# jasonkyuyim/se3_diffusion

Measured on AMD Instinct MI355X. Metric: residues/sec IPA fwd+bwd, higher is better.
Workload: dtype f32

## Files before the change

include/fd_hip.h:

```cpp
#ifndef FD_HIP_H_
#define FD_HIP_H_

#ifdef __cplusplus
extern "C" {
#endif

#define FD_ABI_VERSION 2

const char* fd_last_error(void);
int fd_abi_version(void);
const char* fd_backend(void);
const char* fd_build_flags(void);
long fd_launch_count(void);

typedef struct FdGemmDesc {
  const float* A;
  const float* B;
  float* C;
  int M, N, K;
  long a_rs, a_cs;
  long b_rs, b_cs;
  long ldc;
  int batch, bdiv;
  long a_so, a_si, b_so, b_si, c_so, c_si;
// ... 41 lines not shown
int fd_edge_mlp_pack(const float* W1, const float* W2, const float* Wf, long ld, void* image, void* stream);
int fd_edge_mlp_pack_bwd(const float* Wf, const float* W2, const float* W1, long ld, const float* W40, void* image, void* stream);
typedef struct FdEdgeMlpDesc {
  const float* x;
  const void* img;
  const float* p1;
  const float* q1;
  const float* bias2;
  float* save1;
  float* save2;
  const float* pf;
  const float* qf;
  const float* gamma;
  const float* beta;
  const float* rowscale;
  float* y;
  float* mean;
  float* rstd;
  float* out;
  long rows;
  int nres;
  int backward;
  float eps;
  int blocks;
  long ld_pq;
  long ld_pqf;
  float* zb_out;
  const float* zb_bias;
  unsigned* mask1;
  unsigned* mask2;
  const unsigned* gmask1;
  const unsigned* gmask2;
  const float* ln_y;
  const float* ln_mean;
  const float* ln_rstd;
  const float* ln_gamma;
  const float* ln_rowscale;
  float* dy_out;
  float* ln_dgamma;
  float* ln_dbeta;
  const float* dzb;
  unsigned* sched;
  int shape;
} FdEdgeMlpDesc;
#define FD_EDGE_MLP_W8_MIN_ROWS 65536L
#define FD_EDGE_MLP_PAIR_MAX_ROWS 16384L
int fd_edge_mlp(const FdEdgeMlpDesc* desc, void* stream);

#define FD_EDGE_EMBED_IMAGE_BYTES (24 * 12288)
int fd_edge_embed_pack_zb(const float* W40, void* image, void* stream);
int fd_edge_embed_pack(const float* W0, const float* W2, const float* W4, void* image, void* stream);
typedef struct FdEdgeEmbedDesc {
  const long* seq_idx;
  const float* sc_ca;
  const float* idenom;
  const float* dg_lower;
  const float* dg_upper;
  const void* img;
  const float* p;
  const float* q;
  const float* bias2;
  const float* bias3;
  const float* gamma;
  const float* beta;
  const float* rowscale;
  float* h1;
  float* h2;
  float* h3;
  float* mean;
  float* rstd;
  float* out;
  long rows;
  int nres;
  float eps;
  int blocks;
  float* zb_out;
  const float* zb_bias;
  unsigned* mask1;
  unsigned* mask2;
  long ld_pq;
} FdEdgeEmbedDesc;
int fd_edge_embed(const FdEdgeEmbedDesc* desc, void* stream);

#define FD_EDGE_EMBED_BWD_IMAGE_BYTES (16 * 12288)
int fd_edge_embed_bwd_pack(const float* W2, const float* W4, void* image, void* stream);
typedef struct FdEdgeEmbedBwdDesc {
  const float* dy;
  const float* h3;
  const float* mean;
  const float* rstd;
  const float* gamma;
  const float* rowscale;
  const float* h2;
  const float* h1;
  const void* img;
  float* dh3;
  float* dh2;
  float* dh1;
  float* dgamma;
  float* dbeta;
  long rows;
  int blocks;
  const unsigned* gmask2;
  const unsigned* gmask1;
  unsigned* sched;
} FdEdgeEmbedBwdDesc;
int fd_edge_embed_bwd(const FdEdgeEmbedBwdDesc* desc, void* stream);

typedef struct FdLnGemmDesc {
  const float* x;
  long ldx;
  const float* gamma;
  const float* beta;
  const float* ln_rowscale;
  float* ln_out;
  long ld_ln_out;
  const float* W;
  long ldw;
  const float* bias;
  const float* resid;
  long ld_resid;
  float* out;
  long ldo;
  int M, N, K;
  int relu;
  float eps;
  int ln_cols;
} FdLnGemmDesc;
int fd_ln_gemm(const FdLnGemmDesc* desc, void* stream);

#define FD_PAIR_DW_MAX_ITEMS 8
typedef struct FdPairDwItem {
  const float* A;
  long lda;
  const float* A_add;
  long ld_add;
  const float* B;
  long ldb;
  float* C;
  long ldc;
  float* a_colsum;
  int trans;
  int a_bands;
  int b_cols;
} FdPairDwItem;
typedef struct FdPairDwDesc {
  FdPairDwItem item[FD_PAIR_DW_MAX_ITEMS];
  int nitems;
  long rows;
  int blocks;
} FdPairDwDesc;
int fd_pair_dw(const FdPairDwDesc* desc, void* stream);

#define FD_GROUP_DW_MAX_ITEMS 32
typedef struct FdGroupDwItem {
  const float* A;
  const float* B;
  float* C;
  float* a_colsum;
  int lda, ldb, ldc;
  int n_out, k_in;
} FdGroupDwItem;
typedef struct FdGroupDwDesc {
  FdGroupDwItem item[FD_GROUP_DW_MAX_ITEMS];
  int nitems;
  long rows;
  int blocks;
} FdGroupDwDesc;
int fd_group_dw(const FdGroupDwDesc* desc, void* stream);

int fd_seq_attn_fwd(const float* qkv, const float* key_add, float* out, float* A_out, float scale, int B, int N,
                    void* stream);
int fd_seq_attn_bwd(const float* qkv, const float* A, const float* dout, const float* out, float* dqkv, float scale, int B, int N,
                    void* stream);

int fd_node_feats(const long* seq_idx, const float* tscaled, const float* fixed, const float* tfreq,
                  const float* idenom, float* out , int B, int N, void* stream);
int fd_node_feats_ld(const long* seq_idx, const float* tscaled, const float* fixed, const float* tfreq,
                     const float* idenom, float* out , long ld, int B, int N, void* stream);
int fd_edge_feats(const long* seq_idx, const float* tscaled, const float* fixed, const float* sc_ca,
                  const float* tfreq, const float* idenom, const float* dg_lower, const float* dg_upper,
                  float* out , int B, int N, void* stream);

int fd_ipa_points_fwd(const float* proj, const float* quat, const float* trans, float* qp, float* kp, float* vp,
                      float* kp_soa, int n_res, long R, int nheads, int c_hidden, int n_qk, int n_v, void* stream);
int fd_ipa_points_bwd(const float* proj, const float* quat, const float* dqp, const float* dkp, const float* dvp,
                      float* dproj, float* dframe, long R, int nheads, int c_hidden, int n_qk, int n_v,
                      void* stream);
int fd_ipa_softmax_fwd(float* S, const float* zb, const float* qp, const float* kp, const float* head_w,
                       const float* mask, int B, int N, void* stream);
// ... 296 lines not shown
```

se3_diffusion_amd/csrc/fd_edge_embed.hip:

```cpp
#include "fd_common.h"
#include "../../include/fd_hip.h"

namespace {

#include "fd_chain.h"

constexpr int EE_UNITS = 20;
constexpr int EE_ZB_UNITS = 4;
constexpr int EE_ZB = 40;
constexpr int EE_C = 128;
constexpr float kPi = 3.14159265358979323846f;

__global__ __launch_bounds__(256) void edge_embed_pack_kernel(const float* __restrict__ W0, const float* __restrict__ W2,
                                                              const float* __restrict__ W4, char* __restrict__ img) {
  const int gid = (int)(blockIdx.x * blockDim.x + threadIdx.x);
  if (gid >= EE_UNITS * 4 * 64) return;
  const int lane = gid & 63, i = (gid >> 6) & 3, u = gid >> 8;
  const int m = lane & 15, g = lane >> 4;
  const int layer = u < 4 ? 0 : (u < 12 ? 1 : 2);
  const int r = u - (layer == 0 ? 0 : (layer == 1 ? 4 : 12));
  const int n = 64 * (r & 1) + 16 * i + m, k0 = 32 * (r >> 1);
  float x[8];
#pragma unroll
  for (int e = 0; e < 8; ++e) {
    if (layer == 0) {
      const int k = k0 + 8 * g + e;
      x[e] = k < 54 ? W0[n * 120 + 66 + k] : 0.f;
    } else {
      const int k = k0 + 16 * (e >> 2) + 4 * g + (e & 3);
      x[e] = (layer == 1 ? W2 : W4)[n * EE_C + k];
    }
  }
  uint4 s0, s1, s2;
  fd_split8(x, s0, s1, s2);
  char* dst = img + (long)u * EM_UNIT + (i * 3) * EM_PIECE + lane * 16;
  *reinterpret_cast<uint4*>(dst) = s0;
  *reinterpret_cast<uint4*>(dst + EM_PIECE) = s1;
  *reinterpret_cast<uint4*>(dst + 2 * EM_PIECE) = s2;
}

__global__ __launch_bounds__(256) void edge_embed_pack_zb_kernel(const float* __restrict__ W40, char* __restrict__ img) {
  const int gid = (int)(blockIdx.x * blockDim.x + threadIdx.x);
  if (gid >= EE_ZB_UNITS * 4 * 64) return;
  const int lane = gid & 63, i = (gid >> 6) & 3, ks = gid >> 8;
  const int m = lane & 15, g = lane >> 4;
  const int n = 16 * i + m;
  float x[8];
#pragma unroll
  for (int e = 0; e < 8; ++e) {
    const int k = 32 * ks + 16 * (e >> 2) + 4 * g + (e & 3);
    x[e] = n < EE_ZB ? W40[n * EE_C + k] : 0.f;
  }
  uint4 s0, s1, s2;
  fd_split8(x, s0, s1, s2);
  char* dst = img + (long)(EE_UNITS + ks) * EM_UNIT + (i * 3) * EM_PIECE + lane * 16;
  *reinterpret_cast<uint4*>(dst) = s0;
  *reinterpret_cast<uint4*>(dst + EM_PIECE) = s1;
  *reinterpret_cast<uint4*>(dst + 2 * EM_PIECE) = s2;
}

template <bool ZB>
__global__ __launch_bounds__(64 * EM_WAVES, 2) void edge_embed_kernel(FdEdgeEmbedDesc d) {
  constexpr int EE_NSTAGE = (EE_UNITS + (ZB ? EE_ZB_UNITS : 0)) / EM_UPS;
  __shared__ __attribute__((aligned(16))) char lds[2 * EM_STAGE];
  const int tid = (int)threadIdx.x;
  const int lane = tid & 63, wave = tid >> 6;
  const int m = lane & 15, g = lane >> 4;
  const long rows = d.rows;
  const long ld_pq = d.ld_pq > 0 ? d.ld_pq : EE_C;
  const int ntiles = (int)((rows + EM_ROWS - 1) / EM_ROWS);
  const int G = (int)gridDim.x, first = (int)blockIdx.x;
  if (first >= ntiles) return;
  const int nmine = (ntiles - first + G - 1) / G;
  const int total_stages = nmine * EE_NSTAGE;

  const char* __restrict__ img_lane = static_cast<const char*>(d.img) + wave * (EM_STAGE / EM_WAVES) + lane * 16;
  char* const lds_wave = lds + wave * (EM_STAGE / EM_WAVES);
  int issued = 0, consumed = 0;
  auto issue_stage = [&]() {
    const char* src = img_lane + (long)(issued % EE_NSTAGE) * EM_STAGE;
    char* dst = lds_wave + (issued & 1) * EM_STAGE;
    fd::glds16x4(src, dst);
    fd::glds16x2(src + 4096, dst + 4096);
    ++issued;
  };
  auto stage_begin = [&]() -> const char* {
    fd::wait_vmem();
    __syncthreads();
    const char* cur = lds + (consumed & 1) * EM_STAGE + lane * 16;
    ++consumed;
    return cur;
  };
  auto stage_prefetch = [&]() {
    if (issued < total_stages) issue_stage();
  };
  issue_stage();

  float den[8], lo[8], up[8];
#pragma unroll
  for (int e = 0; e < 8; ++e) {
    den[e] = d.idenom[(8 * g + e) & 15];
    const int kb = 8 * g + e;
    lo[e] = kb < 22 ? d.dg_lower[kb] : 3.0e38f;
    up[e] = kb < 22 ? d.dg_upper[kb] : 0.f;
  }

  for (int ti = 0; ti < nmine; ++ti) {
    const long row = ((long)first + (long)ti * G) * EM_ROWS + wave * 16 + m;
    const bool rok = row < rows;
    const long rc = rok ? row : rows - 1;
    const long qi = rc / d.nres;
    const long qj = (qi / d.nres) * d.nres + (rc - qi * d.nres);

    float x0[8], x1[8];
    {
      const float rel = (float)(d.seq_idx[qi] - d.seq_idx[qj]) * kPi;
      const float dx = d.sc_ca[qi * 3 + 0] - d.sc_ca[qj * 3 + 0], dy = d.sc_ca[qi * 3 + 1] - d.sc_ca[qj * 3 + 1],
                  dz = d.sc_ca[qi * 3 + 2] - d.sc_ca[qj * 3 + 2];
      const float dist = sqrtf(dx * dx + dy * dy + dz * dz);
#pragma unroll
      for (int e = 0; e < 8; ++e) {
        float sn, cs;
        sincosf(rel / den[e], &sn, &cs);
        x0[e] = g < 2 ? sn : cs;
        x1[e] = (dist > lo[e] && dist < up[e]) ? 1.f : 0.f;
      }
    }
    uint4 b[3];
    Em16Half H[2];

    f32x4 acc1[8];
#pragma unroll
    for (int nb = 0; nb < 8; ++nb) {
      const float4 pa = *reinterpret_cast<const float4*>(d.p + qi * ld_pq + 16 * nb + 4 * g);
      const float4 qa = *reinterpret_cast<const float4*>(d.q + qj * ld_pq + 16 * nb + 4 * g);
      acc1[nb][0] = pa.x + qa.x; acc1[nb][1] = pa.y + qa.y; acc1[nb][2] = pa.z + qa.z; acc1[nb][3] = pa.w + qa.w;
    }
#pragma clang loop unroll(full)
    for (int sg = 0; sg < 4 / EM_UPS; ++sg) {
      const char* st = stage_begin();
      em16_read_half(H[0], st);
// ... 203 lines not shown
```

se3_diffusion_amd/csrc/fd_edge_embed_bwd.hip:

```cpp
#include "fd_common.h"
#include "../../include/fd_hip.h"

namespace {

#include "fd_chain.h"

constexpr int EB_UNITS = 16;
constexpr int EB_NSTAGE = EB_UNITS / EM_UPS;
constexpr int EB_C = 128;

__global__ __launch_bounds__(256) void edge_embed_bwd_pack_kernel(const float* __restrict__ W2, const float* __restrict__ W4,
                                                                  char* __restrict__ img) {
  const int gid = (int)(blockIdx.x * blockDim.x + threadIdx.x);
  if (gid >= EB_UNITS * 4 * 64) return;
  const int lane = gid & 63, i = (gid >> 6) & 3, u = gid >> 8;
  const int m = lane & 15, g = lane >> 4;
  const int layer = u >> 3, r = u & 7;
  const int n = 64 * (r & 1) + 16 * i + m, k0 = 32 * (r >> 1);
  const float* __restrict__ W = layer == 0 ? W4 : W2;
  float x[8];
#pragma unroll
  for (int e = 0; e < 8; ++e) {
    const int k = k0 + 16 * (e >> 2) + 4 * g + (e & 3);
    x[e] = W[k * EB_C + n];
  }
  uint4 s0, s1, s2;
  fd_split8(x, s0, s1, s2);
  char* dst = img + (long)u * EM_UNIT + (i * 3) * EM_PIECE + lane * 16;
  *reinterpret_cast<uint4*>(dst) = s0;
  *reinterpret_cast<uint4*>(dst + EM_PIECE) = s1;
  *reinterpret_cast<uint4*>(dst + 2 * EM_PIECE) = s2;
}

__global__ __launch_bounds__(64 * EM_WAVES, 2) void edge_embed_bwd_kernel(FdEdgeEmbedBwdDesc d) {
  __shared__ __attribute__((aligned(16))) char lds[2 * EM_STAGE];
  const int tid = (int)threadIdx.x;
  const int lane = tid & 63, wave = tid >> 6;
  const int m = lane & 15, g = lane >> 4;
  const long rows = d.rows;
  const int ntiles = (int)((rows + EM_ROWS - 1) / EM_ROWS);
  const int G = (int)gridDim.x, first = (int)blockIdx.x;
  if (first >= ntiles) return;
  unsigned* const sched = d.sched;
  const bool dyn = sched != nullptr;
  __shared__ int s_tile;
  const int nmine = (ntiles - first + G - 1) / G;
  const int total_stages = dyn ? 0x7fffffff : nmine * EB_NSTAGE;

  const char* __restrict__ img_lane = static_cast<const char*>(d.img) + wave * (EM_STAGE / EM_WAVES) + lane * 16;
  char* const lds_wave = lds + wave * (EM_STAGE / EM_WAVES);
  int issued = 0, consumed = 0;
  auto issue_stage = [&]() {
    const char* src = img_lane + (long)(issued % EB_NSTAGE) * EM_STAGE;
    char* dst = lds_wave + (issued & 1) * EM_STAGE;
    fd::glds16x4(src, dst);
    fd::glds16x2(src + 4096, dst + 4096);
    ++issued;
  };
  auto stage_begin = [&]() -> const char* {
    fd::wait_vmem();
    __syncthreads();
    const char* cur = lds + (consumed & 1) * EM_STAGE + lane * 16;
    ++consumed;
    return cur;
  };
  auto stage_prefetch = [&]() {
    if (issued < total_stages) issue_stage();
  };
  issue_stage();

  f32x4 dgam[8], dbet[8];
#pragma unroll
  for (int nb = 0; nb < 8; ++nb)
#pragma unroll
    for (int e = 0; e < 4; ++e) dgam[nb][e] = dbet[nb][e] = 0.f;

  int tile = first, nxt = 0;
  for (int ti = 0;;) {
    if (dyn && tid == 0) nxt = G + (int)atomicAdd(&sched[0], 1u);
    const long row = (long)tile * EM_ROWS + wave * 16 + m;
    const bool rok = row < rows;
    const long rc = rok ? row : rows - 1;

    const bool packed = d.gmask2 != nullptr;
    unsigned gm2 = 0u, gm1 = 0u;
    if (packed) {
      gm2 = d.gmask2[rc * 4 + g];
      gm1 = d.gmask1[rc * 4 + g];
    }

    f32x4 d3[8];
    {
      const float rs = (d.rowscale != nullptr ? d.rowscale[rc] : 1.f) * (rok ? 1.f : 0.f);
      const float mean = d.mean[rc], rstd = d.rstd[rc];
      float s1 = 0.f, s2 = 0.f;
#pragma unroll
      for (int nb = 0; nb < 8; ++nb) {
        const int col = 16 * nb + 4 * g;
        const float4 dy = *reinterpret_cast<const float4*>(d.dy + rc * EB_C + col);
        const float4 h = *reinterpret_cast<const float4*>(d.h3 + rc * EB_C + col);
        const float4 gm = *reinterpret_cast<const float4*>(d.gamma + col);
        const float dyv[4] = {dy.x, dy.y, dy.z, dy.w}, hv[4] = {h.x, h.y, h.z, h.w}, gv[4] = {gm.x, gm.y, gm.z, gm.w};
#pragma unroll
        for (int e = 0; e < 4; ++e) {
          const float x = (hv[e] - mean) * rstd;
          const float gy = dyv[e] * rs;
          dgam[nb][e] += gy * x;
          dbet[nb][e] += gy;
          const float t = gy * gv[e];
          d3[nb][e] = t;
          s1 += t;
          s2 += t * x;
        }
      }
      s1 += __shfl_xor(s1, 16);
      s1 += __shfl_xor(s1, 32);
      s2 += __shfl_xor(s2, 16);
      s2 += __shfl_xor(s2, 32);
      const float m1 = s1 * (1.0f / 128.0f), m2 = s2 * (1.0f / 128.0f);
#pragma unroll
      for (int nb = 0; nb < 8; ++nb) {
        const float4 h = *reinterpret_cast<const float4*>(d.h3 + rc * EB_C + 16 * nb + 4 * g);
        const float hv[4] = {h.x, h.y, h.z, h.w};
#pragma unroll
        for (int e = 0; e < 4; ++e) d3[nb][e] = rstd * (d3[nb][e] - m1 - (hv[e] - mean) * rstd * m2);
        if (rok)
          *reinterpret_cast<float4*>(d.dh3 + row * EB_C + 16 * nb + 4 * g) =
              make_float4(d3[nb][0], d3[nb][1], d3[nb][2], d3[nb][3]);
      }
    }
    uint4 b[3];
    Em16Half H[2];

    f32x4 a2[8];
#pragma unroll
    for (int nb = 0; nb < 8; ++nb)
#pragma unroll
      for (int e = 0; e < 4; ++e) a2[nb][e] = 0.f;
#pragma clang loop unroll(full)
    for (int sg = 0; sg < 8 / EM_UPS; ++sg) {
      const char* st = stage_begin();
      em16_read_half(H[0], st);
#pragma clang loop unroll(full)
      for (int hh = 0; hh < 2 * EM_UPS; ++hh) {
        const int r = EM_UPS * sg + (hh >> 1), ks = r >> 1, g2 = r & 1, a = 4 * g2 + 2 * (hh & 1);
        EM_PIN_TOP();
        if (hh + 1 < 2 * EM_UPS) em16_read_half(H[(hh + 1) & 1], st + (hh + 1) * (EM_UNIT / 2));
        EM_PIN_MID();
        if (g2 == 0 && (hh & 1) == 0) em16_split2(d3[2 * ks], d3[2 * ks + 1], b[0], b[1], b[2]);
        em16_mma_half(a2[a], a2[a + 1], H[hh & 1], b);
        EM_GROUPS(hh + 1 < 2 * EM_UPS);
        if (hh == 1) stage_prefetch();
      }
    }
#pragma unroll
    for (int nb = 0; nb < 8; ++nb) {
      if (packed) {
#pragma unroll
        for (int e = 0; e < 4; ++e) a2[nb][e] = ((gm2 >> (4 * nb + e)) & 1u) ? a2[nb][e] : 0.f;
      } else {
        const float4 h = *reinterpret_cast<const float4*>(d.h2 + rc * EB_C + 16 * nb + 4 * g);
        a2[nb][0] = h.x > 0.f ? a2[nb][0] : 0.f;
        a2[nb][1] = h.y > 0.f ? a2[nb][1] : 0.f;
        a2[nb][2] = h.z > 0.f ? a2[nb][2] : 0.f;
        a2[nb][3] = h.w > 0.f ? a2[nb][3] : 0.f;
      }
      if (rok)
        *reinterpret_cast<float4*>(d.dh2 + row * EB_C + 16 * nb + 4 * g) = make_float4(a2[nb][0], a2[nb][1], a2[nb][2], a2[nb][3]);
    }

    f32x4 a1[8];
#pragma unroll
    for (int nb = 0; nb < 8; ++nb)
#pragma unroll
      for (int e = 0; e < 4; ++e) a1[nb][e] = 0.f;
#pragma clang loop unroll(full)
    for (int sg = 0; sg < 8 / EM_UPS; ++sg) {
      const char* st = stage_begin();
      em16_read_half(H[0], st);
#pragma clang loop unroll(full)
      for (int hh = 0; hh < 2 * EM_UPS; ++hh) {
        const int r = EM_UPS * sg + (hh >> 1), ks = r >> 1, g2 = r & 1, a = 4 * g2 + 2 * (hh & 1);
        EM_PIN_TOP();
        if (hh + 1 < 2 * EM_UPS) em16_read_half(H[(hh + 1) & 1], st + (hh + 1) * (EM_UNIT / 2));
        EM_PIN_MID();
        if (g2 == 0 && (hh & 1) == 0) em16_split2(a2[2 * ks], a2[2 * ks + 1], b[0], b[1], b[2]);
        em16_mma_half(a1[a], a1[a + 1], H[hh & 1], b);
        EM_GROUPS(hh + 1 < 2 * EM_UPS);
        if (hh == 1) stage_prefetch();
      }
    }
#pragma unroll
    for (int nb = 0; nb < 8; ++nb) {
      float4 o;
      if (packed) {
        o = make_float4(((gm1 >> (4 * nb)) & 1u) ? a1[nb][0] : 0.f, ((gm1 >> (4 * nb + 1)) & 1u) ? a1[nb][1] : 0.f,
                        ((gm1 >> (4 * nb + 2)) & 1u) ? a1[nb][2] : 0.f, ((gm1 >> (4 * nb + 3)) & 1u) ? a1[nb][3] : 0.f);
      } else {
        const float4 h = *reinterpret_cast<const float4*>(d.h1 + rc * EB_C + 16 * nb + 4 * g);
        o = make_float4(h.x > 0.f ? a1[nb][0] : 0.f, h.y > 0.f ? a1[nb][1] : 0.f, h.z > 0.f ? a1[nb][2] : 0.f,
                        h.w > 0.f ? a1[nb][3] : 0.f);
      }
      if (rok) *reinterpret_cast<float4*>(d.dh1 + row * EB_C + 16 * nb + 4 * g) = o;
    }
    if (!dyn) {
      if (++ti >= nmine) break;
      tile = first + ti * G;
    } else {
      if (tid == 0) s_tile = nxt;
      __syncthreads();
      tile = s_tile;
      __syncthreads();
      if (tile >= ntiles) break;
    }
  }
  if (dyn) fd::wait_vmem();

#pragma unroll
  for (int nb = 0; nb < 8; ++nb)
#pragma unroll
    for (int e = 0; e < 4; ++e) {
      float a = dgam[nb][e], c = dbet[nb][e];
#pragma unroll
      for (int o = 1; o < 16; o <<= 1) {
        a += __shfl_xor(a, o);
        c += __shfl_xor(c, o);
      }
      dgam[nb][e] = a;
      dbet[nb][e] = c;
    }
  __syncthreads();
  float* red = reinterpret_cast<float*>(lds);
  if (m == 0) {
#pragma unroll
    for (int nb = 0; nb < 8; ++nb)
#pragma unroll
      for (int e = 0; e < 4; ++e) {
        red[(wave * 2 + 0) * EB_C + 16 * nb + 4 * g + e] = dgam[nb][e];
        red[(wave * 2 + 1) * EB_C + 16 * nb + 4 * g + e] = dbet[nb][e];
      }
  }
  __syncthreads();
  if (tid < 2 * EB_C) {
    const int which = tid >> 7, col = tid & 127;
    float a = 0.f;
#pragma unroll
    for (int w = 0; w < EM_WAVES; ++w) a += red[(w * 2 + which) * EB_C + col];
    float* dst = which == 0 ? d.dgamma : d.dbeta;
    if (dst != nullptr) atomicAdd(dst + col, a);
  }
}

}

extern "C" int fd_edge_embed_bwd_pack(const float* W2, const float* W4, void* img, void* stream) {
  FD_CHECK_ARG(W2 && W4 && img, "fd_edge_embed_bwd_pack: null operand");
  FD_CHECK_ARG(fd_aligned16(img), "fd_edge_embed_bwd_pack: image must be 16-byte aligned");
  hipLaunchKernelGGL(edge_embed_bwd_pack_kernel, dim3(EB_UNITS * 4 * 64 / 256), dim3(256), 0, (hipStream_t)stream, W2, W4,
                     static_cast<char*>(img));
  FD_CHECK_LAUNCH("fd_edge_embed_bwd_pack");
  return FD_OK;
}

extern "C" int fd_edge_embed_bwd(const FdEdgeEmbedBwdDesc* desc, void* stream) {
  FD_CHECK_ARG(desc != nullptr, "fd_edge_embed_bwd: null descriptor");
  const FdEdgeEmbedBwdDesc& d = *desc;
  FD_CHECK_ARG(d.dy && d.h3 && d.mean && d.rstd && d.gamma && d.img && d.dh3 && d.dh2 && d.dh1,
               "fd_edge_embed_bwd: a required operand is null");
  FD_CHECK_ARG((d.h2 && d.h1) || (d.gmask2 && d.gmask1), "fd_edge_embed_bwd: h2 / h1 or their packed sign masks are required");
  FD_CHECK_ARG(d.rows >= 0, "fd_edge_embed_bwd: negative row count");
  const void* ptrs[] = {d.dy, d.h3, d.gamma, d.h2, d.h1, d.img, d.dh3, d.dh2, d.dh1};
  for (const void* p : ptrs) FD_CHECK_ARG(fd_aligned16(p), "fd_edge_embed_bwd: operands must be 16-byte aligned");
  if (d.rows == 0) return FD_OK;
  const long ntiles = (d.rows + EM_ROWS - 1) / EM_ROWS;
  const int blocks = d.blocks > 0 ? d.blocks : 256 * EM_BLOCKS_PER_CU;
  const long grid = ntiles < blocks ? ntiles : blocks;
  FdEdgeEmbedBwdDesc dd = d;
  if (dd.sched != nullptr && ntiles >= 4 * grid) {
    FD_CHECK_ARG(hipMemsetAsync(dd.sched, 0, sizeof(unsigned), (hipStream_t)stream) == hipSuccess,
                 "fd_edge_embed_bwd: zeroing the tile counter failed");
  } else {
    dd.sched = nullptr;
  }
  hipLaunchKernelGGL(edge_embed_bwd_kernel, dim3((unsigned)grid), dim3(64 * EM_WAVES), 0, (hipStream_t)stream, dd);
  FD_CHECK_LAUNCH("fd_edge_embed_bwd");
  return FD_OK;
}
```

se3_diffusion_amd/csrc/fd_edge_mlp.hip:

```cpp
#if defined(EM_PHASE_TIMING) || defined(EM_ABLATE_PQ) || defined(EM_PLAIN_SAVES)
#include "fd_probe.h"
#endif
#include "fd_common.h"
#include "../../include/fd_hip.h"

#ifdef EM_SHAPE_W8
#define EM_LAUNCH fd_edge_mlp_launch_w8
#else
#define EM_LAUNCH fd_edge_mlp_launch_w4
#endif
int fd_edge_mlp_launch_w4(const FdEdgeMlpDesc& d, hipStream_t st);
int fd_edge_mlp_launch_w8(const FdEdgeMlpDesc& d, hipStream_t st);
int fd_edge_mlp_launch_pair(const FdEdgeMlpDesc& d, hipStream_t st);

namespace {

#include "fd_chain.h"

__device__ __forceinline__ float fd_f4(const float4& v, int e) { return e == 0 ? v.x : e == 1 ? v.y : e == 2 ? v.z : v.w; }

constexpr int EM_UNITS = 120;
constexpr int EM_ZB_UNITS = 4;
constexpr int EM_ZB = 40;
constexpr int EM_RING = 2;
constexpr int EM_H = 384, EM_C = 128;
#ifdef EM_PLAIN_SAVES
#define EM_SAVE4(p, a, b, c, e) (*reinterpret_cast<float4*>(p) = make_float4((a), (b), (c), (e)))
#else
#define EM_SAVE4(p, a, b, c, e) fd::store_nt4((p), (a), (b), (c), (e))
#endif

#ifdef EM_PHASE_TIMING
__device__ unsigned long long em_phase[12];
#define EM_TICK_TO(var)                                                \
  {                                                                    \
    __builtin_amdgcn_sched_barrier(0);                                 \
    const long long t_ = (long long)__builtin_amdgcn_s_memtime();      \
    __builtin_amdgcn_sched_barrier(0);                                 \
    var += t_ - tl_;                                                   \
    tl_ = t_;                                                          \
  }
#define EM_BODY_TO(i) { EM_TICK_TO(tb_); em_add(i, tb_); tb_ = 0; }
#else
#define EM_TICK_TO(var)
#define EM_BODY_TO(i)
#endif

#ifndef EM_SHAPE_W8
struct EmMat {
  const float* p;
  long rs, cs;
};

__global__ __launch_bounds__(256) void edge_mlp_pack16_kernel(EmMat A1, EmMat A2, EmMat A4, char* __restrict__ img, int rot) {
  const int gid = (int)(blockIdx.x * blockDim.x + threadIdx.x);
  if (gid >= EM_UNITS * 4 * 64) return;
  const int lane = gid & 63, i = (gid >> 6) & 3, u = gid >> 8;
  const int m = lane & 15, g = lane >> 4;
  EmMat M;
  int n, k0;
  if (u < 96) {
    const int c = u / 32, r = u % 32, hc = (c + rot) % 3;
    if (r < 8) {
      M = A1; n = 128 * hc + 64 * (r & 1) + 16 * i + m; k0 = 32 * (r >> 1);
    } else {
      const int r2 = r - 8;
      M = A2; n = 64 * (r2 % 6) + 16 * i + m; k0 = 128 * hc + 32 * (r2 / 6);
    }
  } else {
    const int v = u - 96;
    M = A4; n = 64 * (v & 1) + 16 * i + m; k0 = 32 * (v >> 1);
  }
  float x[8];
#pragma unroll
  for (int e = 0; e < 8; ++e) {
    const int k = k0 + 16 * (e >> 2) + 4 * g + (e & 3);
    x[e] = M.p[(long)n * M.rs + (long)k * M.cs];
  }
  uint4 s0, s1, s2;
  fd_split8(x, s0, s1, s2);
  char* dst = img + (long)u * EM_UNIT + (i * 3) * EM_PIECE + lane * 16;
  *reinterpret_cast<uint4*>(dst) = s0;
  *reinterpret_cast<uint4*>(dst + EM_PIECE) = s1;
  *reinterpret_cast<uint4*>(dst + 2 * EM_PIECE) = s2;
}

__global__ __launch_bounds__(256) void edge_mlp_pack_zb_kernel(const float* __restrict__ W40, char* __restrict__ img) {
  const int gid = (int)(blockIdx.x * blockDim.x + threadIdx.x);
  if (gid >= EM_ZB_UNITS * 4 * 64) return;
  const int lane = gid & 63, i = (gid >> 6) & 3, ks = gid >> 8;
  const int m = lane & 15, g = lane >> 4;
  const int n = 16 * i + m;
  float x[8];
#pragma unroll
  for (int e = 0; e < 8; ++e) {
    const int k = 32 * ks + 16 * (e >> 2) + 4 * g + (e & 3);
    x[e] = n < EM_ZB ? W40[n * EM_C + k] : 0.f;
  }
  uint4 s0, s1, s2;
  fd_split8(x, s0, s1, s2);
  char* dst = img + (long)(EM_UNITS + ks) * EM_UNIT + (i * 3) * EM_PIECE + lane * 16;
  *reinterpret_cast<uint4*>(dst) = s0;
  *reinterpret_cast<uint4*>(dst + EM_PIECE) = s1;
  *reinterpret_cast<uint4*>(dst + 2 * EM_PIECE) = s2;
}

__global__ __launch_bounds__(256) void edge_mlp_pack_zbw_kernel(const float* __restrict__ W40, char* __restrict__ img) {
  const int gid = (int)(blockIdx.x * blockDim.x + threadIdx.x);
  if (gid >= EM_ZB_UNITS * 4 * 64) return;
  const int lane = gid & 63, i = (gid >> 6) & 3, u = gid >> 8;
  const int m = lane & 15, g = lane >> 4;
  const int n = 64 * (u & 1) + 16 * i + m, k0 = 32 * (u >> 1);
  float x[8];
#pragma unroll
  for (int e = 0; e < 8; ++e) {
    const int k = k0 + 8 * g + e;
    x[e] = k < EM_ZB ? W40[k * EM_C + n] : 0.f;
  }
  uint4 s0, s1, s2;
  fd_split8(x, s0, s1, s2);
  char* dst = img + (long)u * EM_UNIT + (i * 3) * EM_PIECE + lane * 16;
  *reinterpret_cast<uint4*>(dst) = s0;
  *reinterpret_cast<uint4*>(dst + EM_PIECE) = s1;
  *reinterpret_cast<uint4*>(dst + 2 * EM_PIECE) = s2;
}

#endif

template <bool BWD, bool ZB = false, bool TRAIN = false, bool LNB = false, bool ZBW = false>
__global__ __launch_bounds__(64 * EM_WAVES, 2) void edge_mlp16_kernel(FdEdgeMlpDesc d) {
  static_assert(!BWD || (!ZB && TRAIN), "backward: no zb layer, always with the saves");
  static_assert(BWD || (!LNB && !ZBW), "the fused prologue is a backward option");
  constexpr int EM_NSTAGE = (EM_UNITS + (ZB ? EM_ZB_UNITS : 0) + (ZBW ? EM_ZB_UNITS : 0)) / EM_UPS;
  __shared__ __attribute__((aligned(16))) char lds[EM_RING * EM_STAGE];
  __shared__ float lnacc[LNB ? 2 * EM_C : 1];
  const int tid = (int)threadIdx.x;
  const int lane = tid & 63, wave = tid >> 6;
  const int m = lane & 15, g = lane >> 4;
  const long rows = d.rows;
#ifdef EM_PHASE_TIMING
  long long p0_ = 0, p1_ = 0, p2_ = 0, p3_ = 0, p4_ = 0, p5_ = 0, p6_ = 0, p7_ = 0, p8_ = 0, p9_ = 0;
  long long tb_ = 0, tl_ = (long long)__builtin_amdgcn_s_memtime();
  auto em_add = [&](int i, long long v) {
    switch (i) {
      case 0: p0_ += v; break;
      case 2: p2_ += v; break;
      case 3: p3_ += v; break;
      case 4: p4_ += v; break;
      case 5: p5_ += v; break;
      case 6: p6_ += v; break;
      case 7: p7_ += v; break;
      case 8: p8_ += v; break;
      default: p9_ += v; break;
    }
  };
#endif
  const long ld_pq = d.ld_pq > 0 ? d.ld_pq : EM_H, ld_pqf = d.ld_pqf > 0 ? d.ld_pqf : EM_C;
  const int ntiles = (int)((rows + EM_ROWS - 1) / EM_ROWS);
  const int G = (int)gridDim.x, first = (int)blockIdx.x;
  if (first >= ntiles) return;
  unsigned* const sched = d.sched;
  const bool dyn = sched != nullptr;
  __shared__ int s_tile;
  const int nmine = (ntiles - first + G - 1) / G;
  const int total_stages = dyn ? 0x7fffffff : nmine * EM_NSTAGE;

  const char* __restrict__ img_lane = static_cast<const char*>(d.img) + wave * (EM_STAGE / EM_WAVES) + lane * 16;
  char* const lds_wave = lds + wave * (EM_STAGE / EM_WAVES);
  int issued = 0, consumed = 0;
  auto issue_stage = [&]() __attribute__((always_inline)) {
    const char* src = img_lane + (long)(issued % EM_NSTAGE) * EM_STAGE;
    char* dst = lds_wave + (issued % EM_RING) * EM_STAGE;
    if (EM_PPW == 6) {
      fd::glds16x4(src, dst);
      fd::glds16x2(src + 4096, dst + 4096);
    } else {
      fd::glds16x3(src, dst);
    }
    ++issued;
  };
  auto stage_begin = [&]() __attribute__((always_inline)) -> const char* {
    EM_TICK_TO(tb_);
    fd::wait_vmem();
    __syncthreads();
    EM_TICK_TO(p1_);
    const char* cur = lds + (consumed % EM_RING) * EM_STAGE + lane * 16;
    ++consumed;
    return cur;
  };
  auto stage_prefetch = [&]() __attribute__((always_inline)) {
    if (issued < total_stages) issue_stage();
  };
  issue_stage();
  if (LNB) {
    if (tid < 2 * EM_C) lnacc[tid] = 0.f;
    __syncthreads();
  }

  int tile = first, nxt = 0;
  for (int ti = 0;;) {
    if (dyn && tid == 0) nxt = G + (int)atomicAdd(&sched[0], 1u);
    const long row = (long)tile * EM_ROWS + wave * 16 + m;
    const bool rok = row < rows;
    const long rc = rok ? row : rows - 1;
    const long qi = rc / d.nres;
    const long qj = (qi / d.nres) * d.nres + (rc - qi * d.nres);

    f32x4 X[BWD ? 8 : 1], Xk[2][2];
    auto load_xk = [&](int buf, int ks) __attribute__((always_inline)) {
#pragma unroll
      for (int i = 0; i < 2; ++i) {
        const float4 v = *reinterpret_cast<const float4*>(d.x + rc * EM_C + 16 * (2 * ks + i) + 4 * g);
        Xk[buf][i][0] = v.x; Xk[buf][i][1] = v.y; Xk[buf][i][2] = v.z; Xk[buf][i][3] = v.w;
      }
    };
    if (BWD) {
#pragma unroll
      for (int nb = 0; nb < 8; ++nb) {
        float4 v = make_float4(0.f, 0.f, 0.f, 0.f);
        if (!LNB || d.x != nullptr) v = *reinterpret_cast<const float4*>(d.x + rc * EM_C + 16 * nb + 4 * g);
        X[nb][0] = v.x; X[nb][1] = v.y; X[nb][2] = v.z; X[nb][3] = v.w;
      }
    } else {
      load_xk(0, 0);
    }
    if (LNB) {
      if (ZBW) {
        float kz[2][8];
        {
          const float* zp = d.dzb + rc * EM_ZB + 8 * g;
          const float4 v = *reinterpret_cast<const float4*>(zp);
          const float4 w = *reinterpret_cast<const float4*>(zp + 4);
          kz[0][0] = v.x; kz[0][1] = v.y; kz[0][2] = v.z; kz[0][3] = v.w;
          kz[0][4] = w.x; kz[0][5] = w.y; kz[0][6] = w.z; kz[0][7] = w.w;
          float4 v1 = make_float4(0.f, 0.f, 0.f, 0.f), w1 = v1;
          if (g == 0) {
            v1 = *reinterpret_cast<const float4*>(d.dzb + rc * EM_ZB + 32);
            w1 = *reinterpret_cast<const float4*>(d.dzb + rc * EM_ZB + 36);
          }
          kz[1][0] = v1.x; kz[1][1] = v1.y; kz[1][2] = v1.z; kz[1][3] = v1.w;
          kz[1][4] = w1.x; kz[1][5] = w1.y; kz[1][6] = w1.z; kz[1][7] = w1.w;
        }
        uint4 bz[3];
        Em16Half Hz[2];
#pragma clang loop unroll(full)
        for (int sg = 0; sg < EM_ZB_UNITS / EM_UPS; ++sg) {
          const char* st = stage_begin();
          em16_read_half(Hz[0], st);
#pragma clang loop unroll(full)
          for (int hh = 0; hh < 2 * EM_UPS; ++hh) {
            const int r = EM_UPS * sg + (hh >> 1), g2 = r & 1, a = 4 * g2 + 2 * (hh & 1);
            EM_PIN_TOP();
            if (hh + 1 < 2 * EM_UPS) em16_read_half(Hz[(hh + 1) & 1], st + (hh + 1) * (EM_UNIT / 2));
            if (g2 == 0 && (hh & 1) == 0) fd_split8(kz[r >> 1], bz[0], bz[1], bz[2]);
            em16_mma_half(X[a], X[a + 1], Hz[hh & 1], bz);
            EM_GROUPS(hh + 1 < 2 * EM_UPS);
            if (hh == 1) stage_prefetch();
          }
        }
      }
      {
        const float rs = (d.ln_rowscale != nullptr ? d.ln_rowscale[rc] : 1.f) * (rok ? 1.f : 0.f);
        const float mean = d.ln_mean[rc], rstd = d.ln_rstd[rc];
        float s1 = 0.f, s2 = 0.f;
#pragma unroll
        for (int nb = 0; nb < 8; ++nb) {
          const int col = 16 * nb + 4 * g;
          const float4 yv = *reinterpret_cast<const float4*>(d.ln_y + rc * EM_C + col);
          const float4 gm = *reinterpret_cast<const float4*>(d.ln_gamma + col);
          const float hv[4] = {yv.x, yv.y, yv.z, yv.w}, gv[4] = {gm.x, gm.y, gm.z, gm.w};
          float cg[4], cb[4];
#pragma unroll
          for (int e = 0; e < 4; ++e) {
            const float xh = (hv[e] - mean) * rstd;
            const float gy = X[nb][e] * rs;
            cg[e] = fd::row16_sum(gy * xh);
            cb[e] = fd::row16_sum(gy);
            const float t = gy * gv[e];
            X[nb][e] = t;
            s1 += t;
            s2 += t * xh;
          }
          if (m == 0) {
#pragma unroll
// ... 243 lines not shown
          if (col < EM_ZB && d.zb_bias != nullptr) a = *reinterpret_cast<const float4*>(d.zb_bias + col);
          acc4[nb][0] = a.x; acc4[nb][1] = a.y; acc4[nb][2] = a.z; acc4[nb][3] = a.w;
        }
#pragma clang loop unroll(full)
        for (int sg = 0; sg < EM_ZB_UNITS / EM_UPS; ++sg) {
          const char* st = stage_begin();
          em16_read_half(H[0], st);
#pragma clang loop unroll(full)
          for (int hh = 0; hh < 2 * EM_UPS; ++hh) {
            const int ks = EM_UPS * sg + (hh >> 1), a = 2 * (hh & 1);
            EM_PIN_TOP();
            if (hh + 1 < 2 * EM_UPS) em16_read_half(H[(hh + 1) & 1], st + (hh + 1) * (EM_UNIT / 2));
            if ((hh & 1) == 0) em16_split2(acc3[2 * ks], acc3[2 * ks + 1], b[0], b[1], b[2]);
            em16_mma_half(acc4[a], acc4[a + 1], H[hh & 1], b);
            EM_GROUPS(hh + 1 < 2 * EM_UPS);
            if (hh == 1) stage_prefetch();
          }
        }
#pragma unroll
        for (int nb = 0; nb < 3; ++nb) {
          const int col = 16 * nb + 4 * g;
          if (rok && col < EM_ZB)
            *reinterpret_cast<float4*>(d.zb_out + row * EM_ZB + col) = make_float4(acc4[nb][0], acc4[nb][1], acc4[nb][2], acc4[nb][3]);
        }
      }
    } else {
#pragma unroll
      for (int nb = 0; nb < 8; ++nb)
        if (rok)
          *reinterpret_cast<float4*>(d.out + row * EM_C + 16 * nb + 4 * g) =
              make_float4(acc3[nb][0], acc3[nb][1], acc3[nb][2], acc3[nb][3]);
    }
    EM_BODY_TO(BWD ? 7 : 8);
    if (!dyn) {
      if (++ti >= nmine) break;
      tile = first + ti * G;
    } else {
      if (tid == 0) s_tile = nxt;
      __syncthreads();
      tile = s_tile;
      __syncthreads();
      if (tile >= ntiles) break;
    }
  }
#ifdef EM_PHASE_TIMING
  if (lane == 0) {
    const long long pv[10] = {p0_, p1_, p2_, p3_, p4_, p5_, p6_, p7_, p8_, p9_};
#pragma unroll
    for (int i = 0; i < 10; ++i)
      __hip_atomic_fetch_add(&em_phase[i], (unsigned long long)pv[i], __ATOMIC_RELAXED, __HIP_MEMORY_SCOPE_AGENT);
  }
  if (tid == 0) __hip_atomic_fetch_add(&em_phase[10], 1ull, __ATOMIC_RELAXED, __HIP_MEMORY_SCOPE_AGENT);
#endif
  if (dyn) fd::wait_vmem();
  if (LNB) {
    __syncthreads();
    if (tid < EM_C) {
      if (d.ln_dgamma != nullptr) atomicAdd(d.ln_dgamma + tid, lnacc[tid]);
    } else if (tid < 2 * EM_C) {
      if (d.ln_dbeta != nullptr) atomicAdd(d.ln_dbeta + (tid - EM_C), lnacc[tid]);
    }
  }
}

}

#ifdef EM_PHASE_TIMING
extern "C" int fd_edge_mlp_phases(unsigned long long* host12, int reset) {
  if (host12 != nullptr && hipMemcpyFromSymbol(host12, HIP_SYMBOL(em_phase), sizeof(em_phase)) != hipSuccess) return -1;
  if (reset) {
    unsigned long long z[12] = {0};
    if (hipMemcpyToSymbol(HIP_SYMBOL(em_phase), z, sizeof(z)) != hipSuccess) return -1;
  }
  return 0;
}
#endif

int EM_LAUNCH(const FdEdgeMlpDesc& d, hipStream_t st) {
  const long ntiles = (d.rows + EM_ROWS - 1) / EM_ROWS;
  const int blocks = d.blocks > 0 ? d.blocks : 256 * EM_BLOCKS_PER_CU;
  const int grid = (int)(ntiles < blocks ? ntiles : blocks);
  const dim3 g3(grid), b3(64 * EM_WAVES);
  FdEdgeMlpDesc dd = d;
  if (dd.sched != nullptr && ntiles >= 4L * grid) {
    FD_CHECK_ARG(hipMemsetAsync(dd.sched, 0, sizeof(unsigned), st) == hipSuccess, "fd_edge_mlp: zeroing the tile counter failed");
  } else {
    dd.sched = nullptr;
  }
  const bool zbv = d.zb_out != nullptr, train = d.save1 != nullptr;
#define EM_GO(...) hipLaunchKernelGGL(HIP_KERNEL_NAME(edge_mlp16_kernel<__VA_ARGS__>), g3, b3, 0, st, dd)
  if (d.backward) {
    if (d.ln_y != nullptr && d.dzb != nullptr) EM_GO(true, false, true, true, true);
    else if (d.ln_y != nullptr) EM_GO(true, false, true, true, false);
    else EM_GO(true, false, true, false, false);
  } else if (zbv) {
    if (train) EM_GO(false, true, true); else EM_GO(false, true, false);
  } else {
    if (train) EM_GO(false, false, true); else EM_GO(false, false, false);
  }
#undef EM_GO
  FD_CHECK_LAUNCH("fd_edge_mlp");
  return FD_OK;
}

#ifndef EM_SHAPE_W8
extern "C" int fd_edge_mlp_pack(const float* W1, const float* W2, const float* Wf, long ld, void* img, void* stream) {
  FD_CHECK_ARG(W1 && W2 && Wf && img, "fd_edge_mlp_pack: null operand");
  FD_CHECK_ARG(fd_aligned16(img), "fd_edge_mlp_pack: image must be 16-byte aligned");
  EmMat m1{W1, ld, 1}, m2{W2, ld, 1}, m4{Wf, ld, 1};
  hipLaunchKernelGGL(edge_mlp_pack16_kernel, dim3(EM_UNITS * 4 * 64 / 256), dim3(256), 0, (hipStream_t)stream, m1, m2, m4,
                     static_cast<char*>(img), 0);
  FD_CHECK_LAUNCH("fd_edge_mlp_pack");
  return FD_OK;
}

extern "C" int fd_edge_mlp_pack_bwd(const float* Wf, const float* W2, const float* W1, long ld, const float* W40, void* img,
                                    void* stream) {
  FD_CHECK_ARG(Wf && W2 && W1 && img, "fd_edge_mlp_pack_bwd: null operand");
  FD_CHECK_ARG(fd_aligned16(img), "fd_edge_mlp_pack_bwd: image must be 16-byte aligned");
  char* base = static_cast<char*>(img);
  if (W40 != nullptr) {
    hipLaunchKernelGGL(edge_mlp_pack_zbw_kernel, dim3(EM_ZB_UNITS * 4 * 64 / 256), dim3(256), 0, (hipStream_t)stream, W40, base);
    base += (long)EM_ZB_UNITS * EM_UNIT;
  }
  EmMat m1{Wf, 1, ld}, m2{W2, 1, ld}, m4{W1, 1, ld};
  hipLaunchKernelGGL(edge_mlp_pack16_kernel, dim3(EM_UNITS * 4 * 64 / 256), dim3(256), 0, (hipStream_t)stream, m1, m2, m4, base, 1);
  FD_CHECK_LAUNCH("fd_edge_mlp_pack_bwd");
  return FD_OK;
}

extern "C" int fd_edge_mlp_pack_zb(const float* W40, void* img, void* stream) {
  FD_CHECK_ARG(W40 && img, "fd_edge_mlp_pack_zb: null operand");
  FD_CHECK_ARG(fd_aligned16(img), "fd_edge_mlp_pack_zb: image must be 16-byte aligned");
  hipLaunchKernelGGL(edge_mlp_pack_zb_kernel, dim3(EM_ZB_UNITS * 4 * 64 / 256), dim3(256), 0, (hipStream_t)stream, W40,
                     static_cast<char*>(img));
  FD_CHECK_LAUNCH("fd_edge_mlp_pack_zb");
  return FD_OK;
}

extern "C" int fd_edge_mlp(const FdEdgeMlpDesc* desc, void* stream) {
  FD_CHECK_ARG(desc != nullptr, "fd_edge_mlp: null descriptor");
  const FdEdgeMlpDesc& d = *desc;
  FD_CHECK_ARG(d.img && d.out && (d.x || (d.backward && d.ln_y && d.dzb)), "fd_edge_mlp: x / img / out are required");
  FD_CHECK_ARG(d.ln_y == nullptr || (d.backward && d.ln_mean && d.ln_rstd && d.ln_gamma),
               "fd_edge_mlp: the fused LayerNorm backward (ln_y) is a backward option and needs ln_mean / ln_rstd / ln_gamma");
  FD_CHECK_ARG(d.dzb == nullptr || d.ln_y != nullptr, "fd_edge_mlp: dzb needs the fused LayerNorm-backward prologue (ln_y)");
  FD_CHECK_ARG(d.nres > 0 && d.rows >= 0, "fd_edge_mlp: bad extents");
  if (d.backward) {
    FD_CHECK_ARG(d.gmask1 && d.gmask2 && d.save1 && d.save2,
                 "fd_edge_mlp(backward): the packed sign masks of h2 (gmask1) and h1 (gmask2) and the outputs d2 (save1) / d1 (save2) "
                 "are required");
    FD_CHECK_ARG(!d.mask1 && !d.mask2 && !d.zb_out, "fd_edge_mlp(backward): mask1 / mask2 / zb_out are forward outputs");
  } else {
    FD_CHECK_ARG(d.p1 && d.q1 && d.bias2 && d.pf && d.qf && d.gamma && d.beta,
                 "fd_edge_mlp(forward): p1 / q1 / bias2 / pf / qf / gamma / beta are required");
    const int nsave = (d.save1 != nullptr) + (d.save2 != nullptr) + (d.mask1 != nullptr) + (d.mask2 != nullptr);
    FD_CHECK_ARG(nsave == 0 || nsave == 4,
                 "fd_edge_mlp(forward): the training outputs save1 (h1), save2 (h2 + [z | 0 | 0]), mask1, mask2 come together");
    FD_CHECK_ARG(nsave == 4 || (!d.y && !d.mean && !d.rstd), "fd_edge_mlp(forward): y / mean / rstd are training outputs (with the saves)");
    FD_CHECK_ARG(!d.gmask1 && !d.gmask2, "fd_edge_mlp(forward): gmask1 / gmask2 are backward inputs");
  }
  const void* ptrs[] = {d.x, d.img, d.out, d.p1, d.q1, d.bias2, d.save1, d.save2, d.pf, d.qf,
                        d.gamma, d.beta, d.y, d.ln_y, d.ln_gamma, d.dy_out, d.dzb};
  for (const void* p : ptrs) FD_CHECK_ARG(fd_aligned16(p), "fd_edge_mlp: operands must be 16-byte aligned");
  if (d.rows == 0) return FD_OK;
  FD_CHECK_ARG(d.zb_out == nullptr || (fd_aligned16(d.zb_out) && fd_aligned16(d.zb_bias)),
               "fd_edge_mlp: zb_out / zb_bias must be 16-byte aligned (the image must carry the fd_edge_mlp_pack_zb units)");
  FD_CHECK_ARG(d.shape == 0 || d.shape == 2 || d.shape == 4 || d.shape == 8,
               "fd_edge_mlp: shape is 0 (by size), 2 (two waves per 16 rows: inference forward), 4 or 8 (waves per block)");
  const bool pair_ok = !d.backward && d.save1 == nullptr;
  FD_CHECK_ARG(d.shape != 2 || pair_ok, "fd_edge_mlp: shape 2 is an inference forward (no backward, no training saves)");
// ... 8 lines not shown
```

se3_diffusion_amd/csrc/fd_gemm_w.h:

```cpp
#ifdef GW_RING
#include "fd_probe.h"
#endif
#ifdef GW_ABL
#include "fd_probe.h"
#else
#define GW_ABL 0
#endif
constexpr int W_BK = 16;
typedef fd::u32x4 w_u32x4;
constexpr int W_TR_PST = W_BK * 64 + 64;

template <int BM, int BN, bool B_KC>
struct WCfg {
  static constexpr int TM = BM / 64, TN = BN / 64;
  static constexpr int A_BYTES = BM * 64;
  static constexpr int B_PLANE = B_KC ? BN * 32 : (BN / 32) * W_TR_PST;
  static constexpr int B_BYTES = 3 * B_PLANE;
  static constexpr int STAGE = A_BYTES + B_BYTES;
#ifdef GW_RING
  static constexpr int RING = GW_RING;
#else
  static constexpr int RING = 3;
#endif
  static constexpr int LDS = RING * STAGE;
// ... 78 lines not shown
#pragma unroll
    for (int j = 0; j < TN; ++j)
#pragma unroll
      for (int r = 0; r < 16; ++r) acc[i][j][r] = 0.f;

  const int sa = (l31 >> 2) & 3;
  const int fa_row = (wm * TM * 32 + l31) * 64;
  const int fa_p0 = fa_row + (((2 * h) ^ sa) * 16), fa_p1 = fa_row + (((2 * h + 1) ^ sa) * 16);
  const int fb_off = A_BYTES + (B_KC ? (wn * TN * 32 + l31) * 32 + ((h ^ ((l31 >> 3) & 1)) * 16)
                                     : (wn * TN) * W_TR_PST + (8 * h + ((lane & 15) >> 2)) * 64 + ((lane >> 4) & 1) * 32 + (lane & 3) * 8);
  auto step = [&](const char* st) __attribute__((always_inline)) {
    uint4 fa[TM][3], fb[TN][3];
    float4 xa[TM][2];
    if (!(GW_ABL & 32)) {
#pragma unroll
      for (int i = 0; i < TM; ++i) {
        xa[i][0] = *reinterpret_cast<const float4*>(st + fa_p0 + i * 32 * 64);
        xa[i][1] = *reinterpret_cast<const float4*>(st + fa_p1 + i * 32 * 64);
      }
#pragma unroll
      for (int pl = 0; pl < 3; ++pl)
#pragma unroll
        for (int j = 0; j < TN; ++j) {
          if (B_KC) {
            fb[j][pl] = *reinterpret_cast<const uint4*>(st + fb_off + pl * B_PLANE + j * 32 * 32);
          } else {
            const char* q = st + fb_off + pl * B_PLANE + j * W_TR_PST;
            const uint2 lo = fd::lds_read_tr16(q), hi = fd::lds_read_tr16(q + 256);
            fb[j][pl] = make_uint4(lo.x, lo.y, hi.x, hi.y);
          }
        }
    }
#pragma unroll
    for (int i = 0; i < TM; ++i) {
      uint2 a0, a1, a2, b0, b1, b2;
      if (GW_ABL & 4) {
        a0 = make_uint2(__float_as_uint(xa[i][0].x), __float_as_uint(xa[i][0].y)); a1 = a0; a2 = a0;
        b0 = make_uint2(__float_as_uint(xa[i][1].x), __float_as_uint(xa[i][1].y)); b1 = b0; b2 = b0;
      } else {
        fd_split4(xa[i][0], a0, a1, a2);
        fd_split4(xa[i][1], b0, b1, b2);
      }
      fa[i][0] = make_uint4(a0.x, a0.y, b0.x, b0.y);
      fa[i][1] = make_uint4(a1.x, a1.y, b1.x, b1.y);
      fa[i][2] = make_uint4(a2.x, a2.y, b2.x, b2.y);
    }
    if (GW_ABL & 8) {
      acc[0][0][0] += __uint_as_float(fa[0][0].x ^ fb[0][0].x ^ fa[TM - 1][2].w ^ fb[TN - 1][2].w);
      return;
    }
    fd_mma6<TRANS, TM, TN>(acc, fa, fb);
  };

  constexpr int RING = Cfg::RING;
  int wslot = 0, rslot = 0;
#pragma unroll
  for (int u = 0; u < RING - 1; ++u) {
    copy(lds + wslot * STAGE);
    wslot = wslot + 1 == RING ? 0 : wslot + 1;
  }
  fd::wait_vmem_keep<(RING - 2) * NPW>();
  __syncthreads();
#pragma unroll 1
  for (int s = 0; s < nk; ++s) {
    copy(lds + wslot * STAGE);
    wslot = wslot + 1 == RING ? 0 : wslot + 1;
    step(lds + rslot * STAGE);
    rslot = rslot + 1 == RING ? 0 : rslot + 1;
    fd::wait_vmem_keep<(RING - 2) * NPW>();
    __syncthreads();
  }
  fd::wait_vmem();

  float* __restrict__ C = d.C;
  if ((GW_ABL & 16) && acc[0][0][0] != 12345.678f) return;
  if (TRANS)
    store_tile_t<TM, TN>(d, C, acc, m0 + wm * TM * 32, n0 + wn * TN * 32, h, l31, g.epi_vec != 0);
  else
    store_tile<TM, TN>(d, C, acc, m0 + wm * TM * 32, n0 + wn * TN * 32, h, l31, g.ksplit > 1);
}

__global__ __launch_bounds__(256) void split_planes_kernel(const float* __restrict__ x, long n8, long n,
                                                           unsigned short* __restrict__ planes) {
  for (long i = (long)blockIdx.x * blockDim.x + threadIdx.x; i < n8; i += (long)gridDim.x * blockDim.x) {
    const float4 a = *reinterpret_cast<const float4*>(x + 8 * i), b = *reinterpret_cast<const float4*>(x + 8 * i + 4);
    uint2 a0, a1, a2, b0, b1, b2;
    fd_split4(a, a0, a1, a2);
    fd_split4(b, b0, b1, b2);
    *reinterpret_cast<uint4*>(planes + 8 * i) = make_uint4(a0.x, a0.y, b0.x, b0.y);
    *reinterpret_cast<uint4*>(planes + n + 8 * i) = make_uint4(a1.x, a1.y, b1.x, b1.y);
    *reinterpret_cast<uint4*>(planes + 2 * n + 8 * i) = make_uint4(a2.x, a2.y, b2.x, b2.y);
  }
}

bool w_ok(const FdGemmDesc& d) {
  if (d.b_planes == nullptr || d.a_cs != 1 || (d.K % W_BK) != 0 || d.batch > 1 || d.a_rowsum != nullptr || d.M < 1) return false;
  auto al4 = [](long x) { return (x & 3) == 0; };
  auto al8 = [](long x) { return (x & 7) == 0; };
  if (!(fd_aligned16(d.A) && al4(d.a_rs) && fd_aligned16(d.b_planes) && al8(d.b_plane_stride))) return false;
  if (d.b_rs == 1) return al8(d.b_cs);
  return d.b_cs == 1 && al8(d.b_rs) && al8(d.N) && d.N >= 8;
}

template <int BM, int BN>
int launch_w(const FdGemmDesc& d, hipStream_t stream) {
  GemmArgs g{};
  g.d = d;
  g.nblk_m = fd_cdiv(d.M, BM);
  g.nblk_n = fd_cdiv(d.N, BN);
  g.ksplit = d.ksplit > 1 ? d.ksplit : 1;
  const int nkt_all = d.K / W_BK;
  if (g.ksplit > nkt_all) g.ksplit = nkt_all > 0 ? nkt_all : 1;
  g.mtiles = 1;
  g.epi_vec = epilogue_vectorisable(d, g.ksplit);
  const bool b_kc = (d.b_rs == 1);
  static const int raster_env = getenv("FD_GEMM_W_RASTER") ? atoi(getenv("FD_GEMM_W_RASTER")) : -1;
  g.raster = raster_env >= 0 ? raster_env : ((long)d.N * 6 > (long)d.M * 4 ? 1 : 0);
  dim3 grid(g.nblk_m * g.nblk_n, 1, g.ksplit), block(256, 1, 1);
  if (g.ksplit > 1) {
    if (b_kc) hipLaunchKernelGGL(HIP_KERNEL_NAME(gemm_w_kernel<BM, BN, true, false>), grid, block, 0, stream, g);
    else hipLaunchKernelGGL(HIP_KERNEL_NAME(gemm_w_kernel<BM, BN, false, false>), grid, block, 0, stream, g);
  } else {
    if (b_kc) hipLaunchKernelGGL(HIP_KERNEL_NAME(gemm_w_kernel<BM, BN, true, true>), grid, block, 0, stream, g);
    else hipLaunchKernelGGL(HIP_KERNEL_NAME(gemm_w_kernel<BM, BN, false, true>), grid, block, 0, stream, g);
  }
  FD_CHECK_LAUNCH("fd_gemm(pre-split weights)");
  return FD_OK;
}
```

se3_diffusion_amd/csrc/fd_split.h:

```cpp
#pragma once

__device__ __forceinline__ void fd_split_residual(float& u, float& v, unsigned t) {
  u -= fd::bf16lo_f32(t);
  v -= fd::bf16hi_f32(t);
}

__device__ __forceinline__ void fd_split4(float4 v, uint2& s0, uint2& s1, uint2& s2) {
  const unsigned h0 = fd::pack_bf16(v.x, v.y), h1 = fd::pack_bf16(v.z, v.w);
  fd_split_residual(v.x, v.y, h0);
  fd_split_residual(v.z, v.w, h1);
  const unsigned m0 = fd::pack_bf16(v.x, v.y), m1 = fd::pack_bf16(v.z, v.w);
  fd_split_residual(v.x, v.y, m0);
  fd_split_residual(v.z, v.w, m1);
  s0 = make_uint2(h0, h1);
  s1 = make_uint2(m0, m1);
  s2 = make_uint2(fd::pack_bf16(v.x, v.y), fd::pack_bf16(v.z, v.w));
}

__device__ __forceinline__ void fd_split8(const float (&x)[8], uint4& s0, uint4& s1, uint4& s2) {
  unsigned t0[4], t1[4], t2[4];
#pragma unroll
  for (int j = 0; j < 4; ++j) {
    float u = x[2 * j], v = x[2 * j + 1];
    t0[j] = fd::pack_bf16(u, v);
    fd_split_residual(u, v, t0[j]);
    t1[j] = fd::pack_bf16(u, v);
    fd_split_residual(u, v, t1[j]);
    t2[j] = fd::pack_bf16(u, v);
  }
  s0 = make_uint4(t0[0], t0[1], t0[2], t0[3]);
  s1 = make_uint4(t1[0], t1[1], t1[2], t1[3]);
  s2 = make_uint4(t2[0], t2[1], t2[2], t2[3]);
}

constexpr int FD_PA[6] = {2, 1, 0, 1, 0, 0};
constexpr int FD_PB[6] = {0, 1, 2, 0, 1, 0};

template <bool TRANS, int TM, int TN>
__device__ __forceinline__ void fd_mma6(f32x16 (&acc)[TM][TN], const uint4 (&fa)[TM][3], const uint4 (&fb)[TN][3]) {
#pragma unroll
  for (int p = 0; p < 6; ++p)
#pragma unroll
    for (int i = 0; i < TM; ++i)
#pragma unroll
      for (int j = 0; j < TN; ++j)
        acc[i][j] = TRANS ? fd::mfma_32x32x16_bf16(fb[j][FD_PB[p]], fa[i][FD_PA[p]], acc[i][j])
                          : fd::mfma_32x32x16_bf16(fa[i][FD_PA[p]], fb[j][FD_PB[p]], acc[i][j]);
}
```

se3_diffusion_amd/hip.py:

```python
from __future__ import annotations

import ctypes
import os
from ctypes import POINTER, Structure, c_char_p, c_double, c_float, c_int, c_long, c_void_p

import torch

_HERE = os.path.dirname(os.path.abspath(__file__))
LIB_PATH = os.path.join(_HERE, "lib", "libfd_hip.so")


_RAW_STREAM = getattr(torch._C, "_cuda_getCurrentRawStream", None)


class FdError(RuntimeError):
    pass


class FdGemmDesc(Structure):
    _fields_ = [
        ("A", c_void_p), ("B", c_void_p), ("C", c_void_p),
        ("M", c_int), ("N", c_int), ("K", c_int),
        ("a_rs", c_long), ("a_cs", c_long),
        ("b_rs", c_long), ("b_cs", c_long),
# ... 4 lines not shown
        ("alpha", c_float), ("beta", c_int),
        ("bias", c_void_p),
        ("pair_p", c_void_p), ("pair_q", c_void_p), ("ld_pair", c_long), ("nres", c_int),
        ("resid", c_void_p), ("ld_resid", c_long),
        ("gate", c_void_p), ("ld_gate", c_long),
        ("rowscale", c_void_p),
        ("relu", c_int), ("tile", c_int), ("ksplit", c_int), ("mtiles", c_int),
        ("a_rowsum", c_void_p),
        ("b_planes", c_void_p), ("b_plane_stride", c_long),
    ]


class FdHeadConst(Structure):
    _fields_ = [
        ("atoms", c_float * 15), ("Rd", c_float * 9), ("td", c_float * 3),
        ("coord_scale", c_float),
        ("exp_max_sigma", c_double), ("exp_min_sigma", c_double),
        ("min_b", c_float), ("max_b", c_float),
        ("L", c_int),
        ("score_norms", c_void_p), ("omega_grid", c_void_p), ("n_omega", c_int),
    ]


class FdLossDesc(Structure):
    _fields_ = [
        ("B", c_int), ("N", c_int),
        ("res_mask", c_void_p), ("fixed_mask", c_void_p), ("t", c_void_p),
        ("gt_trans_score", c_void_p), ("gt_rot_score", c_void_p),
        ("trans_score_scaling", c_void_p), ("rot_score_scaling", c_void_p),
        ("gt_rigids", c_void_p), ("gt_atom37", c_void_p),
        ("rot_score", c_void_p), ("trans_score", c_void_p), ("rigids", c_void_p), ("atom37", c_void_p),
        ("coordinate_scaling", c_float), ("trans_x0_threshold", c_float), ("trans_loss_weight", c_float),
        ("rot_loss_weight", c_float), ("rot_loss_t_threshold", c_float),
        ("bb_atom_loss_weight", c_float), ("bb_atom_loss_t_filter", c_float), ("aux_loss_weight", c_float),
        ("dist_mat_loss_weight", c_float), ("dist_mat_loss_t_filter", c_float),
        ("d_rot_score", c_void_p), ("d_trans_score", c_void_p), ("d_rigids", c_void_p), ("d_atom37", c_void_p),
        ("terms", c_void_p), ("loss", c_void_p), ("scratch", c_void_p),
        ("joint_rot_loss", c_int),
    ]


class FdEdgeMlpDesc(Structure):
    __slots__ = ()
    _fields_ = [
        ("x", c_void_p), ("img", c_void_p), ("p1", c_void_p), ("q1", c_void_p), ("bias2", c_void_p),
        ("save1", c_void_p), ("save2", c_void_p),
        ("pf", c_void_p), ("qf", c_void_p), ("gamma", c_void_p), ("beta", c_void_p), ("rowscale", c_void_p),
        ("y", c_void_p), ("mean", c_void_p), ("rstd", c_void_p), ("out", c_void_p),
        ("rows", c_long), ("nres", c_int), ("backward", c_int), ("eps", c_float), ("blocks", c_int),
        ("ld_pq", c_long), ("ld_pqf", c_long), ("zb_out", c_void_p), ("zb_bias", c_void_p),
        ("mask1", c_void_p), ("mask2", c_void_p), ("gmask1", c_void_p), ("gmask2", c_void_p),
        ("ln_y", c_void_p), ("ln_mean", c_void_p), ("ln_rstd", c_void_p), ("ln_gamma", c_void_p), ("ln_rowscale", c_void_p),
        ("dy_out", c_void_p), ("ln_dgamma", c_void_p), ("ln_dbeta", c_void_p), ("dzb", c_void_p), ("sched", c_void_p),
        ("shape", c_int),
    ]


EDGE_MLP_W8_MIN_ROWS = 65536
EDGE_MLP_PAIR_MAX_ROWS = 16384
EDGE_MLP_IMAGE_BYTES = 124 * 12288


class FdEdgeEmbedDesc(Structure):
    __slots__ = ()
    _fields_ = [
        ("seq_idx", c_void_p), ("sc_ca", c_void_p), ("idenom", c_void_p), ("dg_lower", c_void_p), ("dg_upper", c_void_p),
        ("img", c_void_p), ("p", c_void_p), ("q", c_void_p), ("bias2", c_void_p), ("bias3", c_void_p),
        ("gamma", c_void_p), ("beta", c_void_p), ("rowscale", c_void_p),
        ("h1", c_void_p), ("h2", c_void_p), ("h3", c_void_p), ("mean", c_void_p), ("rstd", c_void_p), ("out", c_void_p),
        ("rows", c_long), ("nres", c_int), ("eps", c_float), ("blocks", c_int), ("zb_out", c_void_p), ("zb_bias", c_void_p),
        ("mask1", c_void_p), ("mask2", c_void_p), ("ld_pq", c_long),
    ]


EDGE_EMBED_IMAGE_BYTES = 24 * 12288


class FdEdgeEmbedBwdDesc(Structure):
    __slots__ = ()
    _fields_ = [
        ("dy", c_void_p), ("h3", c_void_p), ("mean", c_void_p), ("rstd", c_void_p), ("gamma", c_void_p), ("rowscale", c_void_p),
        ("h2", c_void_p), ("h1", c_void_p), ("img", c_void_p), ("dh3", c_void_p), ("dh2", c_void_p), ("dh1", c_void_p),
        ("dgamma", c_void_p), ("dbeta", c_void_p), ("rows", c_long), ("blocks", c_int), ("gmask2", c_void_p), ("gmask1", c_void_p),
        ("sched", c_void_p),
    ]


EDGE_EMBED_BWD_IMAGE_BYTES = 16 * 12288

class FdLnGemmDesc(Structure):
    __slots__ = ()
    _fields_ = [
        ("x", c_void_p), ("ldx", c_long), ("gamma", c_void_p), ("beta", c_void_p), ("ln_rowscale", c_void_p),
        ("ln_out", c_void_p), ("ld_ln_out", c_long), ("W", c_void_p), ("ldw", c_long), ("bias", c_void_p),
        ("resid", c_void_p), ("ld_resid", c_long), ("out", c_void_p), ("ldo", c_long),
        ("M", c_int), ("N", c_int), ("K", c_int), ("relu", c_int), ("eps", c_float), ("ln_cols", c_int),
    ]


PAIR_DW_MAX_ITEMS = 8


class FdPairDwItem(Structure):
    __slots__ = ()
    _fields_ = [
        ("A", c_void_p), ("lda", c_long), ("A_add", c_void_p), ("ld_add", c_long), ("B", c_void_p), ("ldb", c_long),
        ("C", c_void_p), ("ldc", c_long), ("a_colsum", c_void_p), ("trans", c_int), ("a_bands", c_int), ("b_cols", c_int),
    ]


class FdPairDwDesc(Structure):
    _fields_ = [("item", FdPairDwItem * PAIR_DW_MAX_ITEMS), ("nitems", c_int), ("rows", c_long), ("blocks", c_int)]


GROUP_DW_MAX_ITEMS = 32


class FdGroupDwItem(Structure):
    __slots__ = ()
    _fields_ = [("A", c_void_p), ("B", c_void_p), ("C", c_void_p), ("a_colsum", c_void_p),
                ("lda", c_int), ("ldb", c_int), ("ldc", c_int), ("n_out", c_int), ("k_in", c_int)]


class FdGroupDwDesc(Structure):
    _fields_ = [("item", FdGroupDwItem * GROUP_DW_MAX_ITEMS), ("nitems", c_int), ("rows", c_long), ("blocks", c_int)]


OPT_WS_DOUBLES = 3 * 4096
OPT_STATE_BYTES = 72


class FdOptState(Structure):
    __slots__ = ()
    _fields_ = [
        ("step", c_long), ("skipped", c_long), ("clipped", c_long), ("nonfinite", c_long),
        ("grad_norm", c_double), ("clip_coef", c_double), ("max_abs", c_double),
        ("bc1", c_float), ("rsqrt_bc2", c_float), ("coef", c_float), ("apply", c_int),
    ]


assert ctypes.sizeof(FdOptState) == OPT_STATE_BYTES


ABI_VERSION = 2


def _ptr(t, off=0):
    if t is None:
        return None
    if isinstance(t, tuple):
        t, off = t
    return t.data_ptr() + t.element_size() * int(off)


def fill_ptrs(desc, **fields):
    tens = []
    for name, t in fields.items():
        if t is None:
            continue
        if type(t) is tuple:
            off = t[1]
            t = t[0]
            setattr(desc, name, t.data_ptr() + t.element_size() * int(off))
        else:
            setattr(desc, name, t.data_ptr())
        tens.append(t)
    return tens


_SIGS = {
    "fd_gemm": "Ss",
    "fd_gemm_plan": "S",
    "fd_split_planes": "plps",
    "fd_gemm_set_exact_f32": "i",
    "fd_gemm_set_persistent_blocks": "i",
    "fd_edge_mlp_pack": "ppplps",
    "fd_edge_mlp": "Ss",
    "fd_edge_mlp_pack_zb": "pps",
    "fd_edge_mlp_pack_bwd": "ppplpps",
    "fd_edge_embed_pack": "pppps",
    "fd_edge_embed": "Ss",
    "fd_edge_embed_pack_zb": "pps",
    "fd_edge_embed_bwd_pack": "ppps",
    "fd_edge_embed_bwd": "Ss",
    "fd_ln_gemm": "Ss",
    "fd_pair_dw": "Ss",
    "fd_group_dw": "Ss",
    "fd_layernorm_fwd": "plpppplpplifs",
    "fd_layernorm_bwd": "plplpppppl" + "ipplis",
    "fd_colsum_acc": "pllips",
    "fd_pair_reduce_acc": "piiippls",
    "fd_axpby": "ppffls",
    "fd_rowscale": "plppllis",
    "fd_add2d": "plpllifs",
    "fd_node_feats": "ppppppiis",
    "fd_node_feats_ld": "ppppppliis",
    "fd_edge_feats": "pppppppppiis",
    "fd_ipa_points_fwd": "pppppppiliiiis",
    "fd_ipa_points_bwd": "pppppppliiiis",
    "fd_ipa_softmax_fwd": "ppppppiis",
    "fd_ipa_attn_fwd": "ppppppppiis",
    "fd_ipa_flash_fwd": "ppppppppppp" + "iiis",
    "fd_ipa_flash_fwd_split": "ppppppppppp" + "iiii" + "ps",
    "fd_ipa_flash_bwd": "pppppppppppp" + "pppppp" + "iis",
    "fd_ipa_flash_bwd_keys": "pppppppp" + "ppp" + "iiis",
    "fd_ipa_opt_bwd_dot": "ppppppp" + "ls",
    "fd_seq_attn_fwd": "ppppfiis",
    "fd_seq_attn_bwd": "pppppfiis",
    "fd_ipa_attn_bwd": "pppppppppppppiis",
    "fd_ipa_softmax_bwd": "ppppppppppiis",
    "fd_ipa_kpts_bwd": "pppppiis",
    "fd_ipa_dz_acc": "ppplis",
    "fd_ipa_opt_fwd": "ppppls",
    "fd_ipa_opt_bwd": "pppppls",
    "fd_ipa_opair_fwd": "pppiis",
    "fd_ipa_opair_bwd": "pppppiis",
    "fd_row_softmax_fwd": "pplii" + "s",
    "fd_row_softmax_bwd": "pplis",
    "fd_split_rigids": "pfpfppplis",
    "fd_bb_update_fwd": "plipppppppp" + "ls",
    "fd_bb_update_bwd": "pppppppppp" + "ls",
    "fd_heads_fwd": "pppp" + "pl" + "ppp" + "pi" + "S" + "ppppppp" + "iis",
    "fd_heads_bwd": "ppppp" + "ppp" + "pi" + "S" + "ppppp" + "ppp" + "iis",
    "fd_backbone_atoms": "ppSppls",
    "fd_igso3_tables": "ppiiippps",
    "fd_sample_ref": "pppppidpls",
    "fd_forward_marginal": "ppppppipdddipppp" + "ls",
    "fd_forward_marginal_batch": "ppppppippdipppp" + "iis",
    "fd_se3_reverse_step": "ppppppiiddpdddiiips",
    "fd_se3_reverse_step_f32": "ppppppiiddpdddiiips",
    "fd_se3_reverse_step_net": "ppppppiiddpdddiiips",
    "fd_sample_advance": "ppppilpipps",
    "fd_sample_record": "ppppp" + "S" + "piili" + "pppp" + "s",
    "fd_dsm_loss": "Ss",
    "fd_adam_step": "pppplffffffs",
    "fd_adam_step_ema": "ppppplfffffffs",
    "fd_grad_stats": "plpps",
    "fd_adam_step_guarded": "pppplddddd" + "i" + "pp" + "s",
    "fd_adam_step_guarded_ema": "ppppplddddd" + "i" + "pp" + "di" + "s",
    "fd_backbone_metrics": "plpiips",
    "fd_aligned_rmsd": "plplpppiipps",
    "fd_tm_search": "plplppp" + "iiiii" + "ppp" + "s",
    "fd_tm_align": "pliplipppp" + "iiii" + "pppp" + "s",
    "fd_dssp_hbonds": "plppiipps",
    "fd_dssp_assign": "plipppiipps",
    "fd_violations": "plppiippppps",
    "fd_cluster_linkage": "pllp" + "iiii" + "ppps",
    "fd_cluster_cut": "pppllp" + "iii" + "d" + "ppps",
    "fd_chain_windows": "pppips",
    "fd_chain_batch": "pppppp" + "ii" + "S" + "ppppp" + "s",
    "fd_mpnn_graph": "pppp" + "li" + "ppp" + "s",
    "fd_mpnn_encoder": "ppp" + "li" + "pp" + "ppppp" + "s",
    "fd_mpnn_decode": "pp" + "ilii" + "pppp" + "pppppp" + "fi" + "pppp" + "s",
    "fd_pdb_count": "plpp" + "ii" + "pp" + "s",
    "fd_pdb_format": "plppp" + "iil" + "pl" + "s",
    "fd_pdb_read_summary": "plpi" + "i" + "p" + "s",
    "fd_pdb_read_count": "plpi" + "ii" + "ppp" + "s",
    "fd_pdb_read_fill": "plpi" + "ii" + "ppp" + "ll" + "pppppp" + "pppp" + "s",
    "fd_cif_read_lines": "plpi" + "p" + "s",
    "fd_cif_read_marks": "plpi" + "pp" + "s",
    "fd_cif_read_header": "plpi" + "ii" + "pppp" + "s",
    "fd_cif_read_summary": "plpi" + "i" + "ppp" + "s",
    "fd_cif_read_count": "plpi" + "ii" + "ppp" + "s",
    "fd_cif_read_fill": "plpi" + "ii" + "ppp" + "ll" + "pppppp" + "pppp" + "s",
    "fd_seq_align": "ppi" + "pipi" + "p" + "iii" + "p" + "s",
    "fd_seq_greedy": "pli" + "p" + "pppp" + "s",
}
# ... 149 lines not shown
```

se3_diffusion_amd/network.py:

```python
from __future__ import annotations

import math

import torch

from . import hip, ops
from .ops import empty, zeros, mv, lib
from .options import opts

H, C, PQ, PV, CZ4 = 8, 256, 8, 12, 32
CS, CZ = 256, 128
LDP = 6816
LDF = 2688
ZB = 40
TD, TH, THD = 320, 4, 80


def check_conf(conf):
    ipa = conf.ipa
    want = dict(c_s=256, c_z=128, c_hidden=256, c_skip=64, no_heads=8, no_qk_points=8, no_v_points=12,
                seq_tfmr_num_heads=4)
    for k, v in want.items():
        if getattr(ipa, k) != v:
            raise NotImplementedError(
# ... 60 lines not shown
    seq = feats["seq_idx"]
    R, Pn = B * N, B * N * N
    pre = "embedding_layer.edge_embedder"
    padded = cache is not None and not save and opts.embed_first_padded and fused_embed()
    NFL = 72 if padded else 65
    nf = empty((R, NFL), dev)
    if padded:
        lib().call("fd_node_feats_ld", seq, tscaled, fixed, tfreq, idenom, nf, NFL, B, N)
        if "embed_first" not in cache:
            Wn, W0e = P["embedding_layer.node_embedder.0.weight"], P[f"{pre}.0.weight"]
            Wn72 = torch.zeros((CS, NFL), device=Wn.device); Wn72[:, :65] = Wn
            Wpq = torch.zeros((2 * CZ, NFL), device=Wn.device); Wpq[:CZ, :33] = W0e[:, :33]; Wpq[CZ:, :33] = W0e[:, 33:66]
            bpq = torch.cat([P[f"{pre}.0.bias"], torch.zeros_like(P[f"{pre}.0.bias"])]).contiguous()
            cache["embed_first"] = (Wn72, Wpq, bpq)
        Wn72, Wpq, bpq = cache["embed_first"]
        node, sv_n = mlp3_ln_fwd(P, "embedding_layer.node_embedder", mv(nf), R, NFL, CS, mask, W0=Wn72)
    else:
        lib().call("fd_node_feats", seq, tscaled, fixed, tfreq, idenom, nf, B, N)
        node, sv_n = mlp3_ln_fwd(P, "embedding_layer.node_embedder", mv(nf), R, 65, CS, mask)
    emask = pair_mask(mask, B, N) if cache is None else cache.setdefault("emask", None)
    if emask is None:
        emask = cache["emask"] = pair_mask(mask, B, N)
    if not fused_embed():
        ef = empty((Pn, 120), dev)
        lib().call("fd_edge_feats", seq, tscaled, fixed, feats["sc_ca_t"], tfreq, idenom, lower, upper, ef, B, N)
        edge, sv_e = mlp3_ln_fwd(P, pre, mv(ef), Pn, 120, CZ, emask)
        return node, edge, dict(node=sv_n, edge=sv_e, emask=emask), None
    W0 = P[f"{pre}.0.weight"]
    ld_pq = 0
    if padded:
        pq = empty((R, 2 * CZ), dev)
        ops.linear(mv(nf), mv(Wpq), bpq, mv(pq), R, 2 * CZ, NFL)
        p_, q_, ld_pq = pq, pq[:, CZ:], 2 * CZ
    else:
        p_ = empty((R, CZ), dev); q_ = empty((R, CZ), dev)
        ops.linear((nf, 0, 65), (W0, 0, 120), P[f"{pre}.0.bias"], mv(p_), R, CZ, 33)
        ops.linear((nf, 0, 65), (W0, 33, 120), None, mv(q_), R, CZ, 33)
    use_zb = (opts.zb_from_edge and zb_next is not None and zb_next[0].is_contiguous() and zb_next[0].data_ptr() % 16 == 0
              and zb_next[1].data_ptr() % 16 == 0)
    key = ("ee_img", pre, use_zb)
    if cache is not None and key in cache:
        img = cache[key]
    else:
        img = ops.edge_embed_pack(W0, P[f"{pre}.2.weight"], P[f"{pre}.4.weight"], W40=zb_next[0] if use_zb else None)
        if cache is not None:
            cache[key] = img
    edge = empty((Pn, CZ), dev)
    kw = {}
    zb = None
    if use_zb:
        zb = empty((Pn, ZB), dev)
        kw.update(zb_out=zb, zb_bias=zb_next[1])
    if save:
        h1 = empty((Pn, CZ), dev); h2 = empty((Pn, CZ), dev); h3 = empty((Pn, CZ), dev)
        mean = empty((Pn,), dev); rstd = empty((Pn,), dev)
        kw.update(h1=h1, h2=h2, h3=h3, mean=mean, rstd=rstd)
        if opts.packed_gates:
            mh1 = empty((Pn, 4), dev, torch.int32); mh2 = empty((Pn, 4), dev, torch.int32)
            kw.update(mask1=mh1, mask2=mh2)
    ops.edge_embed(seq, feats["sc_ca_t"], idenom, lower, upper, img, p_, q_, P[f"{pre}.2.bias"], P[f"{pre}.4.bias"],
                   P[f"{pre}.5.weight"], P[f"{pre}.5.bias"], edge, Pn, N, rowscale=emask, ld_pq=ld_pq, **kw)
    sv_e = None
    if save:
        sv_e = dict(x=None, h1=h1, h2=h2, h3=h3, mean=mean, rstd=rstd, rowscale=emask, M=Pn, K0=120, C=CZ,
                    mh1=kw.get("mask1"), mh2=kw.get("mask2"),
                    regen=(seq, tscaled, fixed, feats["sc_ca_t"], B, N))
    return node, edge, dict(node=sv_n, edge=sv_e, emask=emask), zb


def embed_regen_early(sv, G):
    se = sv["edge"]
    if G is None or se is None or se.get("x") is not None or "regen" not in se:
        return
    seq, tscaled, fixed, sc, B, N = se["regen"]
    Pn = B * N * N
    if not ops.side_active(sc, Pn):
        return
    tfreq, idenom, lower, upper = ops.feature_tables(sc.device)
    ef = empty((Pn, 120), sc)
    ops.side(lambda: lib().call("fd_edge_feats", seq, tscaled, fixed, sc, tfreq, idenom, lower, upper, ef, B, N), (ef,), Pn)
    se["x_early"] = ef


def embed_bwd(P, G, sv, dnode, dedge):
    mlp3_ln_bwd(P, G, "embedding_layer.node_embedder", sv["node"], dnode)
    se = sv["edge"]
    if se.get("x_early") is not None:
        se = dict(se, x=mv(se.pop("x_early")))
    if se.get("x") is None:
        seq, tscaled, fixed, sc, B, N = se["regen"]
        tfreq, idenom, lower, upper = ops.feature_tables(dedge.device)
        ef = empty((B * N * N, 120), dedge)
        lib().call("fd_edge_feats", seq, tscaled, fixed, sc, tfreq, idenom, lower, upper, ef, B, N)
        se = dict(se, x=mv(ef))
    pre = "embedding_layer.edge_embedder"
    if (opts.fused_embed_bwd and fused_embed() and G is not None and se.get("regen") is not None
            and all(f"{pre}.{l}.{t}" in G for l in (0, 2, 4) for t in ("weight", "bias"))):
        M = se["M"]
        dh3 = empty((M, CZ), dedge); dh2 = empty((M, CZ), dedge); dh1 = empty((M, CZ), dedge)
        img = ops.edge_embed_bwd_pack(P[f"{pre}.2.weight"], P[f"{pre}.4.weight"])
        ops.edge_embed_bwd(dedge, se["h3"], se["mean"], se["rstd"], P[f"{pre}.5.weight"], se["rowscale"], se["h2"], se["h1"], img,
                           dh3, dh2, dh1, G[f"{pre}.5.weight"], G[f"{pre}.5.bias"], M, gmask2=se.get("mh2"), gmask1=se.get("mh1"))
        x = se["x"]
        items = [(mv(dh3), mv(se["h2"]), mv(G[f"{pre}.4.weight"]), G[f"{pre}.4.bias"], CZ, CZ),
                 (mv(dh2), mv(se["h1"]), mv(G[f"{pre}.2.weight"]), G[f"{pre}.2.bias"], CZ, CZ),
                 (mv(dh1), x, mv(G[f"{pre}.0.weight"]), G[f"{pre}.0.bias"], CZ, se["K0"])]
        ops.side(lambda: ops.group_dw(items, M), (dh3, dh2, dh1, se["h2"], se["h1"], x[0]), M)
        return
    mlp3_ln_bwd(P, G, pre, se, dedge)


def pair_mask(mask, B, N):
    em = empty((B * N * N,), mask)
    src = mask.reshape(B, 1, N).expand(B, N, N).contiguous()
    lib().call("fd_rowscale", src, N, mask.reshape(-1), em, N, B * N, N)
    return em


def _adjacent_view(a, b, shape, *more):
    ts = (a, b) + more
    for x, y in zip(ts[:-1], ts[1:]):
        if not (x.is_contiguous() and y.is_contiguous() and x.dtype == y.dtype and x.device == y.device
                and x.untyped_storage().data_ptr() == y.untyped_storage().data_ptr()
                and x.storage_offset() + x.numel() == y.storage_offset()):
            return None
    if a.data_ptr() % 16 != 0:
        return None
    strides, st = [], 1
    for d in reversed(shape):
        strides.append(st)
        st *= d
    return a.detach().as_strided(shape, tuple(reversed(strides)))


_PROJ = ("linear_q", "linear_kv", "linear_q_points", "linear_kv_points")


def _proj_views(P, pre):
    if not opts.proj_merge:
        return None
    try:
        W = _adjacent_view(*(P[f"{pre}.{n}.weight"] for n in _PROJ[:2]), (LDP, CS), *(P[f"{pre}.{n}.weight"] for n in _PROJ[2:]))
        b = _adjacent_view(*(P[f"{pre}.{n}.bias"] for n in _PROJ[:2]), (LDP,), *(P[f"{pre}.{n}.bias"] for n in _PROJ[2:]))
    except KeyError:
        return None
    return None if W is None or b is None else (W, b)


def _joined(a, b, shape):
    v = _adjacent_view(a, b, shape)
    return v if v is not None else torch.cat([a, b], 0).contiguous()


def ipa_w40(P, pre, cache=None):
    if cache is not None and ("W40", pre) in cache:
        return cache[("W40", pre)]
    W40 = _joined(P[f"{pre}.linear_b.weight"], P[f"{pre}.down_z.weight"], (ZB, CZ))
    b40 = _joined(P[f"{pre}.linear_b.bias"], P[f"{pre}.down_z.bias"], (ZB,))
    if cache is not None:
        cache[("W40", pre)] = (W40, b40)
    return W40, b40


def ipa_fwd(P, pre, s, z, quat, trans, mask, B, N, cache=None, zb=None, out_view=None, save=True):
    dev = z
    R, Pn = B * N, B * N * N
    proj = empty((R, LDP), dev)
    if cache is not None:
        if ("Wproj", pre) not in cache:
            cache[("Wproj", pre)] = (torch.cat([P[f"{pre}.{n}.weight"] for n in _PROJ], 0).contiguous(),
                                     torch.cat([P[f"{pre}.{n}.bias"] for n in _PROJ], 0).contiguous())
        Wp, bp = cache[("Wproj", pre)]
        ops.linear(s, mv(Wp), bp, mv(proj), R, LDP, CS)
    elif _proj_views(P, pre) is not None:
        Wp, bp = _proj_views(P, pre)
        ops.linear(s, mv(Wp), bp, mv(proj), R, LDP, CS)
    else:
        ops.linear(s, mv(P[f"{pre}.linear_q.weight"]), P[f"{pre}.linear_q.bias"], (proj, 0, LDP), R, H * C, CS)
        ops.linear(s, mv(P[f"{pre}.linear_kv.weight"]), P[f"{pre}.linear_kv.bias"], (proj, 2048, LDP), R, 2 * H * C, CS)
        ops.linear(s, mv(P[f"{pre}.linear_q_points.weight"]), P[f"{pre}.linear_q_points.bias"], (proj, 6144, LDP), R, 192, CS)
        ops.linear(s, mv(P[f"{pre}.linear_kv_points.weight"]), P[f"{pre}.linear_kv_points.bias"], (proj, 6336, LDP), R, 480, CS)
    qp = empty((R, H, PQ * 3), dev); kp = empty((R, H, PQ * 3), dev); vp = empty((R, H, PV * 3), dev)
    train = bool(save)
    flash = (opts.flash_ipa and B * ((N + 15) // 16) >= opts.flash_ipa_min_tiles and N <= 1024
             and (lib().is_device or opts.flash_ipa_min_tiles <= 0))
# ... 291 lines not shown
```

se3_diffusion_amd/ops.py:

```python
from __future__ import annotations

import math
import threading

import torch

from . import hip
from .options import opts

F32 = torch.float32


def lib():
    return hip.get_lib()


def empty(shape, like, dtype=F32):
    return torch.empty(shape, device=like.device, dtype=dtype)


def zeros(shape, like, dtype=F32):
    a = _ARENA["buf"]
    if a is not None and dtype == F32 and a.device == like.device:
        n = 1
        for d in shape:
            n *= int(d)
        lo = _ARENA["used"]
        hi = lo + (n + 63) // 64 * 64
        if hi <= a.numel():
            _ARENA["used"] = hi
            return a[lo:lo + n].view(shape)
    return torch.zeros(shape, device=like.device, dtype=dtype)


_ARENA = {"buf": None, "used": 0}


class zero_arena:
    def __init__(self, numel, like):
        self.numel, self.like = int(numel), like

    def __enter__(self):
        self.prev = dict(_ARENA)
        _ARENA["buf"] = torch.zeros(self.numel, device=self.like.device, dtype=F32) if self.numel > 0 else None
        _ARENA["used"] = 0
        return self

    def __exit__(self, *exc):
        _ARENA.update(self.prev)
        return False


def mv(t, off=0, ld=None):
    return (t, off, ld if ld is not None else t.shape[-1])


_PLANES = None


def weight_planes(P):
    global _PLANES
    _PLANES = None
    if not opts.weight_planes or lib().exact_f32:
        return None
    ts = list(P.values())
    st = ts[0].untyped_storage()
    base, nbytes = st.data_ptr(), st.nbytes()
    if base % 16 or nbytes % 32 or any(t.dtype != F32 or t.untyped_storage().data_ptr() != base for t in ts):
        return None
    n = nbytes // 4
    flat = torch.empty(0, dtype=F32, device=ts[0].device).set_(st, 0, (n,), (1,))
    planes = torch.empty((3, n), dtype=torch.int16, device=ts[0].device)
    lib().call("fd_split_planes", flat, n, planes)
    _PLANES = (base, nbytes, planes)
    return _PLANES


def set_weight_planes(ps):
    global _PLANES
    was, _PLANES = _PLANES, ps
    return was


def _planes_of(wt, wo):
    ps = _PLANES
    if ps is None:
        return None
    a = wt.data_ptr() + 4 * wo
    if not (ps[0] <= a < ps[0] + ps[1]):
        return None
    return (ps[2].data_ptr() + (a - ps[0]) // 2, ps[1] // 4)


def linear(x, W, b, out, M, N, K, *, relu=False, resid=None, rowscale=None, pair=None, beta=False,
           gate=None, alpha=1.0, tile=0):
    xt, xo, xl = x
    wt, wo, wl = W
    ot, oo, ol = out
    kw = {}
    bp = _planes_of(wt, wo)
    if bp is not None:
        kw["b_planes"] = bp
    if resid is not None:
        kw.update(resid=(resid[0], resid[1]), ld_resid=resid[2])
    if gate is not None:
        kw.update(gate=(gate[0], gate[1]), ld_gate=gate[2])
    lib().gemm(xt, wt, ot, M, N, K, (xl, 1), (1, wl), ol, a_off=xo, b_off=wo, c_off=oo, bias=b,
               relu=relu, rowscale=rowscale, pair=pair, beta=beta, alpha=alpha, tile=tile, **kw)


def linear_dx(dy, W, dx, M, N, K, *, beta=False, gate=None, rowscale=None, alpha=1.0, resid=None):
    dt, do, dl = dy
    wt, wo, wl = W
    xt, xo, xl = dx
    kw = {}
    if gate is not None:
        kw.update(gate=(gate[0], gate[1]), ld_gate=gate[2])
    if resid is not None:
        kw.update(resid=(resid[0], resid[1]), ld_resid=resid[2])
    bp = _planes_of(wt, wo)
    if beta and not kw and rowscale is None and N >= 1024 and opts.dx_splitk and not lib().exact_f32:
        lib().gemm(dt, wt, xt, M, K, N, (dl, 1), (wl, 1), xl, a_off=do, b_off=wo, c_off=xo, alpha=alpha,
                   ksplit=min(8, N // 512), b_planes=bp)
        return
    lib().gemm(dt, wt, xt, M, K, N, (dl, 1), (wl, 1), xl, a_off=do, b_off=wo, c_off=xo, beta=beta,
               rowscale=rowscale, alpha=alpha, b_planes=bp, **kw)


_SIDE = {"streams": {}, "pending": [], "used": False}


def _new_side_stream(device):
    return torch.cuda.Stream(device=device, priority=int(opts.side_stream_priority))


def side(fn, tensors, rows):
    t = tensors[0]
    if not (opts.grad_stream and t.is_cuda and rows <= opts.grad_stream_max_rows):
        fn()
        return
    key = t.device.index
    st = _SIDE["streams"].get(key)
    if st is None:
        st = _SIDE["streams"][key] = _new_side_stream(t.device)
    st.wait_stream(torch.cuda.current_stream())
    with torch.cuda.stream(st):
        fn()
    _SIDE["pending"].extend(tensors)
    _SIDE["used"] = True


def side_active(t, rows):
    return bool(opts.grad_stream and t.is_cuda and rows <= opts.grad_stream_max_rows)


def grad_stream(device):
    if not (opts.grad_stream and device.type == "cuda"):
        return None
    st = _SIDE["streams"].get(device.index)
    if st is None:
        st = _SIDE["streams"][device.index] = _new_side_stream(device)
    st.wait_stream(torch.cuda.current_stream())
# ... 77 lines not shown
    q["items"], q["tensors"], q["rows"] = [], [], None


def queue_dw_ok(dy, x, dW, M, N, K):
    if not opts.grouped_node_dw or M > GROUP_DW_MAX_ROWS or M < 1 or lib().exact_f32:
        return False
    dt, do, dl = dy
    xt, xo, xl = x
    wt, wo, wl = dW
    if (N % 4) or (K % 4) or (dl % 4) or (xl % 4) or (dt.data_ptr() + 4 * do) % 16 or (xt.data_ptr() + 4 * xo) % 16:
        return False
    return not (wl < K or dl < N or xl < K)


def flush_dw(blocks=0):
    q = _DWQ
    if not q["items"]:
        return
    items, tens, rows = q["items"], q["tensors"], q["rows"]
    q["items"], q["tensors"], q["rows"] = [], [], None
    side(lambda: group_dw(items, rows, blocks), tens, rows)


def add_view(dst, src, rows, cols, alpha=1.0):
    dt, do, dl = dst
    st, so, sl = src
    lib().call("fd_add2d", (dt, do), dl, (st, so), sl, rows, cols, alpha)


def bias_grad(dy, db, M, N):
    dt, do, dl = dy
    lib().call("fd_colsum_acc", (dt, do), dl, M, N, db)


def layernorm(x, gamma, beta, y, rows, C, *, rowscale=None, save=None):
    xt, xo, xl = x
    yt, yo, yl = y
    mean, rstd = save if save is not None else (None, None)
    lib().call("fd_layernorm_fwd", (xt, xo), xl, gamma, beta, rowscale, (yt, yo), yl, mean, rstd, rows, C, 1e-5)


def layernorm_bwd(dy, x, gamma, mean, rstd, dx, rows, C, *, rowscale=None, dgamma=None, dbeta=None, accum=False):
    dt, do, dl = dy
    xt, xo, xl = x
    gt, go, gl = dx
    lib().call("fd_layernorm_bwd", (dt, do), dl, (xt, xo), xl, gamma, rowscale, mean, rstd, (gt, go), gl,
               int(accum), dgamma, dbeta, rows, C)


def ln_linear_ok(x, W, M, N, K):
    return bool(opts.ln_fold and M <= 1024 and K % 8 == 0 and K <= 320 and x[1] % 4 == 0 and W[1] == 0 and x[2] % 4 == 0
                and W[2] % 4 == 0)


def ln_linear(x, gamma, beta, W, b, out, M, N, K, *, relu=False, resid=None, ln_rowscale=None, ln_out=None, ln_cols=0):
    d = hip.FdLnGemmDesc()
    tens = hip.fill_ptrs(d, x=x, gamma=gamma, beta=beta, ln_rowscale=ln_rowscale, ln_out=ln_out, W=W, bias=b, resid=resid, out=out)
    d.ldx, d.ldw, d.ldo = x[2], W[2], out[2]
    if ln_out is not None:
        d.ld_ln_out = ln_out[2]
    if resid is not None:
        d.ld_resid = resid[2]
    d.M, d.N, d.K, d.relu, d.eps, d.ln_cols = int(M), int(N), int(K), int(bool(relu)), 1e-5, int(ln_cols)
    lib().launch("fd_ln_gemm", d, tens)


_TABLES = {}


def feature_tables(device, index_embed_size=32, num_bins=22, min_bin=1e-5, max_bin=20.0):
    key = (str(device), index_embed_size, num_bins, min_bin, max_bin)
    if key not in _TABLES:
        half = index_embed_size // 2
        tfreq = torch.exp(torch.arange(half, dtype=torch.float32) * -(math.log(10000) / (half - 1)))
        k = torch.arange(half)
        idenom = (2056 ** (2 * k[None] / index_embed_size))[0].to(torch.float32)
        lower = torch.linspace(min_bin, max_bin, num_bins)
        upper = torch.cat([lower[1:], lower.new_tensor([1e8])])
        _TABLES[key] = tuple(t.contiguous().to(device) for t in (tfreq, idenom, lower, upper))
    return _TABLES[key]


def edge_mlp_pack(W1, W2, Wf, backward=False, out=None, W40=None):
    img = out if out is not None else torch.empty(hip.EDGE_MLP_IMAGE_BYTES, dtype=torch.uint8, device=W1.device)
    assert W40 is None or (W40.is_contiguous() and tuple(W40.shape) == (40, 128))
    assert W1.stride(-1) == 1 and W2.stride(-1) == 1 and Wf.stride(-1) == 1 and W1.stride(0) == W2.stride(0) == Wf.stride(0)
    ld = W1.stride(0)
    if not backward:
        lib().call("fd_edge_mlp_pack", W1, W2, Wf, ld, img)
        if W40 is not None:
            lib().call("fd_edge_mlp_pack_zb", W40, img)
    else:
        lib().call("fd_edge_mlp_pack_bwd", Wf, W2, W1, ld, W40, img)
    return img


def edge_mlp_pack_bwd(Wf, W2, W1, W40=None, out=None):
    return edge_mlp_pack(W1, W2, Wf, backward=True, out=out, W40=W40)


_SCHED = {}
_SCHED_LOCK = threading.Lock()
STATS = {"edge_dynamic_launches": 0, "ipa_flash_fwd": 0, "ipa_sequence_fwd": 0, "ipa_flash_bwd": 0, "ipa_sequence_bwd": 0,
         "ipa_flash_bwd_keys": 0, "ipa_keys_gemms": 0}


_SCHED_WORDS = 256


def edge_sched_init(device):
    with _SCHED_LOCK:
        pool = _SCHED.get(("pool", device))
        if pool is None:
            if device.type == "cuda" and torch.cuda.is_current_stream_capturing():
                raise RuntimeError("ops.edge_sched_init must run before hipGraph capture starts (sampler.sample calls it)")
            pool = _SCHED[("pool", device)] = (torch.zeros(_SCHED_WORDS, dtype=torch.int32, device=device), {})
    return pool


def _edge_sched(like, stream):
    buf, slots = edge_sched_init(like.device)
    with _SCHED_LOCK:
        key = int(stream or 0)
        slot = slots.get(key)
        if slot is None:
            if len(slots) >= _SCHED_WORDS // 4:
                raise RuntimeError(f"ops._edge_sched: more than {_SCHED_WORDS // 4} streams have used the dynamic tile hand-out on "
                                   f"{like.device}; raise ops._SCHED_WORDS")
            slot = slots[key] = len(slots)
        STATS["edge_dynamic_launches"] += 1
    return buf.data_ptr() + 16 * slot


EDGE_MLP_MACS_PER_ROW = 128 * 384 + 384 * 384 + 384 * 128


def edge_mlp(x, img, out, rows, nres, *, backward=False, blocks=0, ld_pq=0, ld_pqf=0, **ptrs):
    d = hip.FdEdgeMlpDesc()
    tens = hip.fill_ptrs(d, x=x, img=img, out=out, **ptrs)
    d.rows, d.nres, d.backward, d.eps, d.blocks = int(rows), int(nres), int(bool(backward)), 1e-5, int(blocks or opts.edge_blocks)
    d.ld_pq, d.ld_pqf = int(ld_pq), int(ld_pqf)
    d.shape = int(opts.edge_shape)
    infer_fwd = not backward and ptrs.get("save1") is None
    if d.shape == 2 and not infer_fwd:
        d.shape = 0
    if d.shape == 0 and infer_fwd and not opts.edge_pair and rows <= hip.EDGE_MLP_PAIR_MAX_ROWS:
        d.shape = 4
    L = lib()
    w8 = d.shape == 8 or (d.shape == 0 and rows >= hip.EDGE_MLP_W8_MIN_ROWS)
    if opts.edge_dynamic_tiles and rows >= 4 * (128 if w8 else 64) * (d.blocks or (256 if w8 else 512)):
        d.sched = _edge_sched(out, L._stream(tens))
    L.launch("fd_edge_mlp", d, tens,
             (7, True, True, 2.0 * int(rows) * (EDGE_MLP_MACS_PER_ROW + (5120 if ptrs.get("zb_out") is not None else 0)),
              (int(rows), 128, 384, 1, int(bool(backward)), 0, 0, 1)) if L.profiling else None)


def edge_embed_pack(W0, W2, W4, out=None, W40=None):
    img = out if out is not None else torch.empty(hip.EDGE_EMBED_IMAGE_BYTES, dtype=torch.uint8, device=W0.device)
    lib().call("fd_edge_embed_pack", W0, W2, W4, img)
    if W40 is not None:
        assert W40.is_contiguous() and tuple(W40.shape) == (40, 128)
        lib().call("fd_edge_embed_pack_zb", W40, img)
    return img


def edge_embed(seq_idx, sc_ca, idenom, dg_lower, dg_upper, img, p, q, bias2, bias3, gamma, beta, out, rows, nres, *,
               blocks=0, ld_pq=0, **ptrs):
    d = hip.FdEdgeEmbedDesc()
    tens = hip.fill_ptrs(d, seq_idx=seq_idx, sc_ca=sc_ca, idenom=idenom, dg_lower=dg_lower, dg_upper=dg_upper, img=img, p=p, q=q,
                         bias2=bias2, bias3=bias3, gamma=gamma, beta=beta, out=out, **ptrs)
    d.rows, d.nres, d.eps, d.blocks = int(rows), int(nres), 1e-5, int(blocks)
    d.ld_pq = int(ld_pq)
    L = lib()
    L.launch("fd_edge_embed", d, tens,
             (8, True, True, 2.0 * int(rows) * 310 * 128, (int(rows), 128, 128, 1, 0, 0, 0, 1)) if L.profiling else None)


def edge_embed_bwd_pack(W2, W4, out=None):
    img = out if out is not None else torch.empty(hip.EDGE_EMBED_BWD_IMAGE_BYTES, dtype=torch.uint8, device=W2.device)
    lib().call("fd_edge_embed_bwd_pack", W2, W4, img)
    return img


def edge_embed_bwd(dy, h3, mean, rstd, gamma, rowscale, h2, h1, img, dh3, dh2, dh1, dgamma, dbeta, rows, blocks=0, gmask2=None,
                   gmask1=None):
    d = hip.FdEdgeEmbedBwdDesc()
    tens = hip.fill_ptrs(d, dy=dy, h3=h3, mean=mean, rstd=rstd, gamma=gamma, rowscale=rowscale, h2=h2, h1=h1, img=img, dh3=dh3, dh2=dh2,
                         dh1=dh1, dgamma=dgamma, dbeta=dbeta, gmask2=gmask2, gmask1=gmask1)
    d.rows, d.blocks = int(rows), int(blocks)
    L = lib()
    if opts.edge_dynamic_tiles and rows >= 4 * 64 * (d.blocks or 512):
        d.sched = _edge_sched(dh3, L._stream(tens))
    L.launch("fd_edge_embed_bwd", d, tens)


def pair_dw(items, rows, blocks=0):
    d = hip.FdPairDwDesc()
    tens = []
    assert 1 <= len(items) <= hip.PAIR_DW_MAX_ITEMS
    for t, it in enumerate(items):
        e = d.item[t]
        add = it.get("A_add")
        tens += hip.fill_ptrs(e, A=it["A"], B=it["B"], C=it["C"], A_add=add, a_colsum=it.get("colsum"))
        e.lda, e.ldb, e.ldc, e.ld_add = int(it["A"][2]), int(it["B"][2]), int(it["C"][2]), 0 if add is None else int(add[2])
        e.trans = int(bool(it.get("trans", False)))
        e.a_bands = int(it.get("a_bands", 3))
        e.b_cols = int(it.get("b_cols", 0))
    d.nitems, d.rows, d.blocks = len(items), int(rows), int(blocks)
    L = lib()
    profile = None
    if L.profiling:
        flops = sum(2.0 * int(rows) * 128 * int(it.get("a_bands", 3)) * (int(it.get("b_cols", 0)) or 128) for it in items)
        profile = (9, False, False, flops, (384, 128 * len(items), int(rows), 1, 0, 0, 0, 1))
    L.launch("fd_pair_dw", d, tens, profile)
```

se3_diffusion_amd/optim.py:

```python
from __future__ import annotations

import contextlib

import torch
import torch.distributed as dist

from . import hip

_ALIGN = 64


class FlatAdam:
    def __init__(self, params, lr=1e-4, betas=(0.9, 0.999), eps=1e-8, adjacent=None, max_grad_norm=None,
                 skip_nonfinite=False, ema_decay=None, ema_warmup=True):
        self.params = [p for p in params if p.requires_grad]
        assert self.params, "no trainable parameters"
        assert all(p.dtype == torch.float32 for p in self.params), "fp32 parameters only"
        self.lr, self.betas, self.eps = float(lr), (float(betas[0]), float(betas[1])), float(eps)
        dev = self.params[0].device
        group_of = {}
        for grp in (adjacent or ()):
            grp = [p for p in grp if p.requires_grad]
            assert all(p.numel() % 4 == 0 for p in grp[:-1]), "grouped parameters must keep their successors 16-byte aligned"
            for p in grp:
                group_of[id(p)] = grp
        placed, off = {}, 0
        for p in self.params:
            if id(p) in placed:
                continue
            for q in group_of.get(id(p), [p]):
                if id(q) in placed:
                    continue
                placed[id(q)] = off
                off += q.numel()
            off = (off + _ALIGN - 1) // _ALIGN * _ALIGN
        self.offsets = [placed[id(p)] for p in self.params]
        self.numel = off
        self.flat_p = torch.zeros(off, device=dev)
        self.flat_g = torch.zeros(off, device=dev)
        self.exp_avg = torch.zeros(off, device=dev)
        self.exp_avg_sq = torch.zeros(off, device=dev)
        for p, o in zip(self.params, self.offsets):
            view = self.flat_p[o:o + p.numel()].view_as(p)
            view.copy_(p.data)
            p.data = view
            p.grad = self.flat_g[o:o + p.numel()].view_as(p)
        self.max_grad_norm = None if max_grad_norm is None else float(max_grad_norm)
        self.skip_nonfinite = bool(skip_nonfinite)
        self.guarded = self.max_grad_norm is not None or self.skip_nonfinite
        self._max_norm_arg()
        self._t = 0
        self._ws = self._opt_state = self._stats = None
        if self.guarded:
            self._ws = torch.empty(hip.OPT_WS_DOUBLES, dtype=torch.float64, device=dev)
            self._opt_state = torch.zeros(hip.OPT_STATE_BYTES // 8, dtype=torch.int64, device=dev)
        self._dirty = False
        self.ema_decay = None if ema_decay is None else float(ema_decay)
        self.ema_warmup = bool(ema_warmup)
        self.ema = None
        self._ema_live = False
        if self.ema_decay is not None:
            self._ema_decay_arg()
            self.ema = self.flat_p.clone()

    @property
    def t(self):
        if self.guarded:
            raise AttributeError("a guarded FlatAdam counts its steps on the device: applied_steps() / set_applied_steps()")
        return self._t

    @t.setter
    def t(self, value):
        if self.guarded:
            raise AttributeError("a guarded FlatAdam counts its steps on the device: applied_steps() / set_applied_steps()")
        self._t = int(value)

    def _max_norm_arg(self):
        if self.max_grad_norm is None:
            return 0.0
        if not self.max_grad_norm > 0.0:
            raise ValueError(f"max_grad_norm must be positive or None (no clipping), not {self.max_grad_norm!r}")
        return self.max_grad_norm

    def _ema_decay_arg(self):
        if not 0.0 < self.ema_decay < 1.0:
            raise ValueError(f"ema_decay must lie strictly between 0 and 1 (or be None: no average), not {self.ema_decay!r}")
        return self.ema_decay

    def rebind(self):
        bp, bg = self.flat_p.data_ptr(), self.flat_g.data_ptr()
        for p, o in zip(self.params, self.offsets):
            g = p.grad
            if p.data_ptr() == bp + 4 * o and g is not None and g.data_ptr() == bg + 4 * o:
                continue
            n = p.numel()
            if p.data.data_ptr() != self.flat_p.data_ptr() + 4 * o:
                view = self.flat_p[o:o + n].view_as(p)
                view.copy_(p.data)
                p.data = view
            if p.grad is None:
                view = self.flat_g[o:o + n].view_as(p)
                if self._dirty:
                    view.zero_()
                p.grad = view
            elif p.grad.data_ptr() != self.flat_g.data_ptr() + 4 * o:
                view = self.flat_g[o:o + n].view_as(p)
                if self._dirty:
                    view.copy_(p.grad.to(view.dtype))
                else:
                    view.add_(p.grad.to(view.dtype))
                p.grad = view

    def zero_grad(self, set_to_none=False):
        self.flat_g.zero_()
        for p in self.params:
            if p.grad is not None and not (self.flat_g.data_ptr() <= p.grad.data_ptr() < self.flat_g.data_ptr() + 4 * self.numel):
                p.grad = None
        self._dirty = False
        self.rebind()

    zero = zero_grad

    def all_reduce_mean(self):
        self.rebind()
        if dist.is_initialized() and dist.get_world_size() > 1:
            dist.all_reduce(self.flat_g, op=dist.ReduceOp.SUM)
            self.flat_g.div_(dist.get_world_size())
        self._dirty = True

    def step(self):
        if self._ema_live:
            raise RuntimeError("step() inside ema_weights(): the parameters are the average there, not the training weights")
        self.rebind()
        b1, b2 = self.betas
        if self.guarded:
            if self.ema is None:
                hip.get_lib().call("fd_adam_step_guarded", self.flat_p, self.flat_g, self.exp_avg, self.exp_avg_sq, self.numel,
                                   self.lr, b1, b2, self.eps, self._max_norm_arg(), int(self.skip_nonfinite), self._ws,
                                   self._opt_state)
            else:
                hip.get_lib().call("fd_adam_step_guarded_ema", self.flat_p, self.flat_g, self.exp_avg, self.exp_avg_sq, self.ema,
                                   self.numel, self.lr, b1, b2, self.eps, self._max_norm_arg(), int(self.skip_nonfinite),
                                   self._ws, self._opt_state, self._ema_decay_arg(), int(self.ema_warmup))
            self._dirty = True
            return
        if self.ema is None:
            self._t += 1
            hip.get_lib().call("fd_adam_step", self.flat_p, self.flat_g, self.exp_avg, self.exp_avg_sq, self.numel,
                               self.lr, b1, b2, self.eps, 1.0 - b1 ** self._t, 1.0 - b2 ** self._t)
        else:
            d = self._ema_decay_arg()
            self._t += 1
            if self.ema_warmup:
                d = min(d, (1.0 + self._t) / (10.0 + self._t))
            hip.get_lib().call("fd_adam_step_ema", self.flat_p, self.flat_g, self.exp_avg, self.exp_avg_sq, self.ema, self.numel,
                               self.lr, b1, b2, self.eps, 1.0 - b1 ** self._t, 1.0 - b2 ** self._t, 1.0 - d)
        self._dirty = True

    def _need_ema(self):
        if self.ema is None:
            raise RuntimeError("this FlatAdam keeps no moving average (ema_decay=None)")

    def _exchange_ema(self):
        tmp = self.flat_p.clone()
        self.flat_p.copy_(self.ema)
        self.ema.copy_(tmp)

    def reset_ema(self):
        self._need_ema()
        if self._ema_live:
            raise RuntimeError("reset_ema() inside ema_weights()")
        self.rebind()
        self.ema.copy_(self.flat_p)

    @contextlib.contextmanager
    def ema_weights(self):
        self._need_ema()
        if self._ema_live:
            raise RuntimeError("ema_weights() does not nest")
        self.rebind()
        self._exchange_ema()
        self._ema_live = True
        try:
            yield self
        finally:
            self._exchange_ema()
            self._ema_live = False

    def _ema_slices(self, model):
        self.rebind()
        at = {self.flat_p.data_ptr() + 4 * o: (o, p.numel()) for p, o in zip(self.params, self.offsets)}
        out = []
        for k, t in model.state_dict().items():
            hit = at.get(t.data_ptr()) if t.dtype == torch.float32 and t.device == self.flat_p.device else None
            if hit is not None and hit[1] == t.numel():
                out.append((k, self.ema[hit[0]:hit[0] + hit[1]].view(t.shape)))
        return out

    def ema_state_dict(self, model):
        self._need_ema()
        if self._ema_live:
            raise RuntimeError("ema_state_dict() inside ema_weights(): model.state_dict() is the average there")
        sd = model.state_dict()
        for k, view in self._ema_slices(model):
            sd[k] = view.clone()
        return sd

    def load_ema_state_dict(self, model, sd):
        self._need_ema()
        if self._ema_live:
            raise RuntimeError("load_ema_state_dict() inside ema_weights()")
        slices = self._ema_slices(model)
        for k, view in slices:
            if k not in sd:
                raise KeyError(f"load_ema_state_dict: missing key {k!r}")
            if tuple(sd[k].shape) != tuple(view.shape):
# ... 60 lines not shown
```

se3_diffusion_amd/options.py:

```python
from __future__ import annotations

import contextlib
import dataclasses
import os


def _flag(name, default):
    return os.environ.get(name, "1" if default else "0") not in ("", "0")


def _int(name, default):
    return int(os.environ.get(name, str(default)))


def _opt(env, default):
    return dataclasses.field(default=default, metadata={"env": env})


@dataclasses.dataclass
class Options:
    grad_stream: bool = _opt("FD_GRAD_STREAM", True)
    grad_stream_max_rows: int = _opt("FD_GRAD_STREAM_ROWS", 1 << 40)
    side_stream_priority: int = _opt("FD_SIDE_PRIORITY", 0)
    fused_edge: bool = _opt("FD_EDGE_FUSED", True)
    fused_embed: bool = _opt("FD_EMBED_FUSED", True)
    fused_embed_bwd: bool = _opt("FD_EMBED_BWD_FUSED", True)
    grouped_pair_dw: bool = _opt("FD_PAIR_DW", True)
    pair_dw_blocks: int = _opt("FD_PAIR_DW_BLOCKS", 160)
    edge_blocks: int = _opt("FD_EDGE_BLOCKS", 0)
    edge_shape: int = _opt("FD_EDGE_SHAPE", 0)
    edge_pair: bool = _opt("FD_EDGE_PAIR", True)
    edge_dynamic_tiles: bool = _opt("FD_EDGE_DYN_TILES", True)
    packed_gates: bool = _opt("FD_PACKED_GATES", True)
    fused_ln_bwd: bool = _opt("FD_EDGE_LN_BWD", True)
    zb_from_edge: bool = _opt("FD_ZB_FUSED", True)
    fold_node_terms: bool = _opt("FD_FOLD_NODE_TERMS", True)
    fused_ipa_attn: bool = _opt("FD_IPA_ATTN_FUSED", True)
    flash_ipa: bool = _opt("FD_IPA_FLASH", True)
    flash_ipa_min_tiles: int = _opt("FD_IPA_FLASH_MIN_TILES", 80)
    flash_ipa_bwd: bool = _opt("FD_IPA_FLASH_BWD", True)
    flash_ipa_keys: bool = _opt("FD_IPA_FLASH_KEYS", True)
    flash_ipa_keys_max_n: int = _opt("FD_IPA_FLASH_KEYS_MAX_N", 384)
    flash_ipa_bwd_min_tiles: int = _opt("FD_IPA_FLASH_BWD_MIN_TILES", 128)
    flash_ipa_split_min_n: int = _opt("FD_IPA_FLASH_SPLIT_MIN_N", 384)
    flash_ipa_splits: int = _opt("FD_IPA_FLASH_SPLITS", 4)
    flash_ipa_hpb: int = _opt("FD_IPA_FLASH_HPB", 0)
    proj_merge: bool = _opt("FD_PROJ_MERGE", True)
    fused_seq_attn: bool = _opt("FD_SEQ_ATTN_FUSED", True)
    seq_attn_min_rows: int = _opt("FD_SEQ_ATTN_MIN_ROWS", 1024)
    fused_seq_attn_bwd: bool = _opt("FD_SEQ_ATTN_BWD_FUSED", True)
    grouped_node_dw: bool = _opt("FD_NODE_DW", True)
    defer_node_dw: bool = _opt("FD_DEFER_NODE_DW", True)
    node_dw_blocks: int = _opt("FD_NODE_DW_BLOCKS", 0)
    weight_planes: bool = _opt("FD_WEIGHT_PLANES", True)
    ln_fold: bool = _opt("FD_LN_FOLD", True)
    sampler_device_steps: bool = _opt("FD_SAMPLER_DEVICE_STEPS", True)
    embed_first_padded: bool = _opt("FD_EMBED_FIRST_PADDED", True)
    merge_skip_embed: bool = _opt("FD_MERGE_SKIP", True)
    zero_arena: bool = _opt("FD_ZERO_ARENA", True)
    dx_splitk: bool = _opt("FD_DX_SPLITK", True)

    @classmethod
    def from_env(cls):
        return cls(**{f.name: (_flag if isinstance(f.default, bool) else _int)(f.metadata["env"], f.default)
                      for f in dataclasses.fields(cls)})


opts = Options.from_env()


@contextlib.contextmanager
def override(**kw):
    was = {}
    for k, v in kw.items():
        if not hasattr(opts, k):
            raise AttributeError(f"unknown option {k!r}")
        was[k] = getattr(opts, k)
        setattr(opts, k, v)
    try:
        yield opts
    finally:
        for k, v in was.items():
            setattr(opts, k, v)
```

se3_diffusion_amd/trunk.py:

```python
from __future__ import annotations

import math

import numpy as np
import torch

from . import hip, ops
from .trace import rng
from . import network as nw
from .network import CS, CZ, TD, H, _lin_grads
from .ops import empty, zeros, mv, lib
from .options import opts

EH = 384
CE = 128


def bb_update_fwd(P, b, n3, dmask, quat, trans, R):
    pre = f"score_model.trunk.bb_update_{b}.linear"
    dev = n3
    upd = empty((R, 6), dev); q2 = empty((R, 4), dev); t2 = empty((R, 3), dev)
    lib().call("fd_bb_update_fwd", n3, CS, CS, dmask, P[f"{pre}.weight"], P[f"{pre}.bias"], quat, trans, upd, q2, t2, R)
    return q2, t2, dict(n3=n3, dmask=dmask, quat=quat, upd=upd, R=R)

# ... 278 lines not shown


def sigma_grid(device, min_sigma=0.1, max_sigma=1.5, num_sigma=1000):
    key = (str(device), min_sigma, max_sigma, num_sigma)
    if key not in _SG:
        t = np.linspace(0.0, 1.0, num_sigma)
        g = np.log(t * np.exp(max_sigma) + (1 - t) * np.exp(min_sigma))
        _SG[key] = torch.tensor(g, dtype=torch.float64, device=device)
    return _SG[key]


def heads_fwd(P, node, quat, trans, feats, B, N, dconf, sc_ca_out=None):
    tp = "score_model.torsion_pred"
    dev = node
    R = B * N
    h1 = empty((R, CS), dev); h2 = empty((R, CS), dev); u = empty((R, 2), dev)
    ops.linear(mv(node), mv(P[f"{tp}.linear_1.weight"]), P[f"{tp}.linear_1.bias"], mv(h1), R, CS, CS, relu=True)
    ops.linear(mv(h1), mv(P[f"{tp}.linear_2.weight"]), P[f"{tp}.linear_2.bias"], mv(h2), R, CS, CS, resid=mv(node))
    ops.linear(mv(h2), mv(P[f"{tp}.linear_final.weight"]), P[f"{tp}.linear_final.bias"], mv(u), R, 2, CS)
    hc, sg = head_tables(dconf, dev.device)
    rot = empty((B, N, 3), dev, torch.float64); ts = empty((B, N, 3), dev); rig = empty((B, N, 7), dev)
    psi = empty((B, N, 2), dev); a37 = empty((B, N, 37, 3), dev); a14 = empty((B, N, 14, 3), dev)
    gt = feats["torsion_angles_sin_cos"]
    tt = feats["t"].float().contiguous()
    lib().call("fd_heads_fwd", feats["rigids_t"], quat, trans, u, (gt, 4), 14, feats["fixed_mask"], feats["res_mask"],
               tt, sg, sg.numel(), hc, rot, ts, rig, psi, a37, a14, sc_ca_out, B, N)
    out = dict(psi=psi, rot_score=rot, trans_score=ts, rigids=rig, atom37=a37, atom14=a14)
    return out, dict(node=node, h1=h1, h2=h2, u=u, quat=quat, trans=trans, psi=psi, t=tt, hc=hc, sg=sg, B=B, N=N)


def heads_bwd(P, G, sv, feats, d_out, dnode):
    tp = "score_model.torsion_pred"
    B, N = sv["B"], sv["N"]
    R = B * N
    dev = sv["node"]
    dq = empty((R, 4), dev); dt = empty((R, 3), dev); du = empty((R, 2), dev)

    def g(k, dtype=torch.float32):
        v = d_out.get(k)
        return None if v is None else v.to(dtype).contiguous()

    lib().call("fd_heads_bwd", feats["rigids_t"], sv["quat"], sv["trans"], sv["u"], sv["psi"], feats["fixed_mask"],
               feats["res_mask"], sv["t"], sv["sg"], sv["sg"].numel(), sv["hc"], g("rot_score", torch.float64),
               g("trans_score"), g("rigids"), g("psi"), g("atom37"), dq, dt, du, B, N)
    _lin_grads(G, f"{tp}.linear_final.weight", f"{tp}.linear_final.bias", mv(du), mv(sv["h2"]), R, 2, CS)
    dh2 = empty((R, CS), dev)
    ops.linear_dx(mv(du), mv(P[f"{tp}.linear_final.weight"]), mv(dh2), R, 2, CS)
    ops.add_view(mv(dnode), mv(dh2), R, CS)
    _lin_grads(G, f"{tp}.linear_2.weight", f"{tp}.linear_2.bias", mv(dh2), mv(sv["h1"]), R, CS, CS)
    dh1 = empty((R, CS), dev)
    ops.linear_dx(mv(dh2), mv(P[f"{tp}.linear_2.weight"]), mv(dh1), R, CS, CS, gate=mv(sv["h1"]))
    _lin_grads(G, f"{tp}.linear_1.weight", f"{tp}.linear_1.bias", mv(dh1), mv(sv["node"]), R, CS, CS)
    ops.linear_dx(mv(dh1), mv(P[f"{tp}.linear_1.weight"]), mv(dnode), R, CS, CS, beta=True)
    return dq, dt


def _prep_feats(feats):
    f = {}
    f["res_mask"] = feats["res_mask"].to(torch.float32).contiguous()
    f["fixed_mask"] = feats["fixed_mask"].to(torch.float32).contiguous()
    f["seq_idx"] = feats["seq_idx"].to(torch.int64).contiguous()
    f["t"] = feats["t"].contiguous()
    f["sc_ca_t"] = feats["sc_ca_t"].to(torch.float32).contiguous()
    f["rigids_t"] = feats["rigids_t"].to(torch.float32).contiguous()
    f["torsion_angles_sin_cos"] = feats["torsion_angles_sin_cos"].to(torch.float32).contiguous()
    return f


def _cached(cache, key, fn):
    if cache is None:
        return fn()
    if key not in cache:
        cache[key] = fn()
    return cache[key]


def _tfmr_layers(P, b):
    n = 0
    while f"score_model.trunk.seq_tfmr_{b}.layers.{n}.linear1.weight" in P:
        n += 1
    return n


def forward(P, feats, num_blocks, dconf=(0.1, 0.1, 20.0, 0.1, 1.5, 1000), tfmr_bool_mask=False, save=True, cache=None,
            sc_ca_out=None):
    if save:
        cache = None
    planes = ops.weight_planes(P) if save else None
    if not save:
        ops.set_weight_planes(None)
    f = _prep_feats(feats)
    B, N = f["res_mask"].shape
    R = B * N
    L = lib()
    mask = f["res_mask"]
    dev = mask
    if not (mask.is_cuda and torch.cuda.is_current_stream_capturing()):
        ops.edge_sched_init(mask.device)
    if cache is not None:
        sig = (B, N, mask.data_ptr(), f["fixed_mask"].data_ptr(), bool(tfmr_bool_mask))
        if cache.get("_sig") != sig:
            cache.clear()
            cache["_sig"] = sig
    rig = f["rigids_t"]
    quat = empty((R, 4), dev); trans = empty((R, 3), dev)
    t32 = f["t"].dtype == torch.float32
    tsc = empty((B,), dev) if t32 else None
    L.call("fd_split_rigids", rig, float(dconf[0]), f["t"] if t32 else None, 10000.0, quat, trans, tsc, R, B)
    f["tscaled"] = tsc if t32 else (f["t"] * 10000).float().contiguous()
    with rng("embed.fwd"):
        node0, z, sv_embed, zb = nw.embed_fwd(P, f, B, N, cache, save=save,
                                              zb_next=nw.ipa_w40(P, "score_model.trunk.ipa_0", cache) if num_blocks > 0 else None)
    emask = sv_embed["emask"]

    def _dmask():
        dm = empty((B, N), dev)
        L.call("fd_rowscale", (1 - f["fixed_mask"]).contiguous(), 1, mask.reshape(-1), dm, 1, R, 1)
        return dm
    dmask = _cached(cache, "dmask", _dmask)
    init_node = node0
    node = node0
    if tfmr_bool_mask:
        key_add = _cached(cache, "key_add", lambda: torch.where(mask > 0, torch.zeros_like(mask),
                                                                 torch.full_like(mask, float("-inf"))))
    else:
        key_add = (1 - mask).contiguous()
    stages = []
    cat_all = None
    if (cache is not None and not save and num_blocks > 1 and opts.merge_skip_embed
            and all(_tfmr_layers(P, b) >= 1 for b in range(num_blocks))
            and ops.ln_linear_ok((node, 0, TD), (node, 0, TD), R, 3 * TD, TD)):
        tp = "score_model.trunk"
        if "skip_all" not in cache:
            Wp = torch.zeros((num_blocks * TD, CS), device=mask.device)
            bp = torch.zeros((num_blocks * TD,), device=mask.device)
            for b in range(num_blocks):
                Wp[b * TD + CS:(b + 1) * TD] = P[f"{tp}.skip_embed_{b}.weight"]
                bp[b * TD + CS:(b + 1) * TD] = P[f"{tp}.skip_embed_{b}.bias"]
            cache["skip_all"] = (Wp, bp)
        Wp, bp = cache["skip_all"]
        cat_all = empty((R, num_blocks * TD), dev)
        ops.linear(mv(init_node), mv(Wp), bp, mv(cat_all), R, num_blocks * TD, CS)
    for b in range(num_blocks):
        pre = f"score_model.trunk.ipa_{b}"
        nl = _tfmr_layers(P, b)
        fold1 = (not save) and nl >= 1 and node.is_cuda == z.is_cuda and ops.ln_linear_ok((node, 0, TD), (node, 0, TD), R, 3 * TD, TD)
        fold6 = fold1 and b < num_blocks - 1 and et_folds_node_terms(cache, save)
        cat = ((cat_all, b * TD, num_blocks * TD) if cat_all is not None else (empty((R, TD), dev), 0, TD)) if fold1 else None
        if fold1 and cat_all is None:
            tp = "score_model.trunk"
            ops.linear(mv(init_node), mv(P[f"{tp}.skip_embed_{b}.weight"]), P[f"{tp}.skip_embed_{b}.bias"],
                       (cat[0], cat[1] + CS, cat[2]), R, 64, CS)
        with rng(f"ipa_{b}.fwd"):
            x1, sv_ipa = nw.ipa_fwd(P, pre, mv(node), z, quat, trans, mask.view(-1), B, N, cache, zb=zb,
                                    out_view=cat if fold1 else None, save=save)
        with rng(f"seq_tfmr_{b}.fwd"):
            pend_ln = None
            if fold1:
                tp = "score_model.trunk"
                u = u0 = empty((R, TD), dev)
                pend_ln = (cat, P[f"{tp}.ipa_ln_{b}.weight"], P[f"{tp}.ipa_ln_{b}.bias"], None, CS, u0)
                sv_ln = None
            else:
                u, sv_ln = nw.ln_skip_fwd(P, b, x1, init_node, R)
                u0 = u
            sv_t = []
            for l in range(nl):
                u, s_, pend_ln = nw.tfmr_layer_fwd(P, f"score_model.trunk.seq_tfmr_{b}.layers.{l}", u, key_add, B, N, save=save,
                                                   out_rowscale=mask.view(-1) if (tfmr_bool_mask and l == nl - 1) else None,
                                                   x_ln=pend_ln, defer_out_ln=not save)
                sv_t.append(s_)
# ... 9 lines not shown
                with rng(f"node_transition_{b}.fwd"):
                    q2, t2, sv_bb = bb_update_fwd(P, b, n3, dmask.view(-1), quat, trans, R)
                z, sv_et, zb = edge_transition_pair(P, b, terms, n3, z, emask, B, N, save=save, cache=cache,
                                                    zb_next=nw.ipa_w40(P, f"score_model.trunk.ipa_{b + 1}", cache))
        else:
            with rng(f"node_transition_{b}.fwd"):
                q2, t2, sv_bb = bb_update_fwd(P, b, n3, dmask.view(-1), quat, trans, R)
            if b < num_blocks - 1:
                with rng(f"edge_transition_{b}.fwd"):
                    z, sv_et, zb = edge_transition_fwd(P, b, n3, z, emask, B, N, save=save, cache=cache,
                                                       zb_next=nw.ipa_w40(P, f"score_model.trunk.ipa_{b + 1}", cache))
        stages.append(dict(ipa=sv_ipa, ln=sv_ln, tfmr=sv_t, pn=sv_pn, bb=sv_bb, et=sv_et))
        node, quat, trans = n3, q2, t2
        if not save:
            stages[-1] = None
    with rng("heads.fwd"):
        sc_out = sc_ca_out if not save else None
        assert sc_out is None or (sc_out.is_contiguous() and sc_out.dtype == torch.float32 and tuple(sc_out.shape) == (B, N, 3))
        out, sv_h = heads_fwd(P, node, quat, trans, f, B, N, dconf, sc_ca_out=sc_out)
    if not save:
        return out, None
    return out, dict(feats=f, embed=sv_embed, stages=stages, heads=sv_h, B=B, N=N, num_blocks=num_blocks,
                     bool_mask=tfmr_bool_mask, mask=mask, dmask=dmask, planes=planes)


def backward(P, G, sv, d_out, on_done=None):
    notify = on_done if on_done is not None else (lambda tag: None)
    hooked = on_done is not None
    B, N, nb = sv["B"], sv["N"], sv["num_blocks"]
    R, Pn = B * N, B * N * N
    f = sv["feats"]
    dev = sv["mask"]
    if sv["bool_mask"]:
        raise NotImplementedError("backward is defined for the training-mode (additive) transformer mask")
    ops.reset_dw_queue()
    ops.set_weight_planes(sv.get("planes"))
    try:
        with ops.zero_arena(R * (nb * 2048 + 1024) + 65536 if opts.zero_arena else 0, dev):
            _backward(P, G, sv, d_out, notify, hooked)
    except BaseException:
        ops.reset_dw_queue()
        raise
    finally:
        ops.set_weight_planes(None)


def _backward(P, G, sv, d_out, notify, hooked=False):
    B, N, nb = sv["B"], sv["N"], sv["num_blocks"]
    R, Pn = B * N, B * N * N
    f = sv["feats"]
    dev = sv["mask"]
    dnode = zeros((R, CS), dev)
    nw.embed_regen_early(sv["embed"], G)
    with rng("heads.bwd"):
        dq, dt = heads_bwd(P, G, sv["heads"], f, d_out, dnode)
    ops.flush_dw()
    notify("heads")
    dinit = zeros((R, CS), dev)
    dz = None
    defer_dw = bool(opts.defer_node_dw and not hooked)
    pend = None
    for b in reversed(range(nb)):
        st = sv["stages"][b]
        dn3 = dnode
        dz_in = None
        if st["et"] is not None:
            dz_in = empty((Pn, CZ), dev)
            with rng(f"edge_transition_{b}.bwd"):
                edge_transition_bwd(P, G, b, st["et"], dz, dz_in, dn3, dzb_next=pend, flush_behind_launch=defer_dw)
            pend = None
        dframe = zeros((R, 12), dev)
        with rng(f"node_transition_{b}.bwd"):
            dq_in, dt_in = bb_update_bwd(P, G, b, st["bb"], dq, dt, None, dn3)
            du0 = zeros((R, TD), dev)
            du2 = nw.post_node_bwd(P, G, b, st["pn"], dn3, du0)
        with rng(f"seq_tfmr_{b}.bwd"):
            du = du2
            for l in reversed(range(len(st["tfmr"]))):
                du = nw.tfmr_layer_bwd(P, G, f"score_model.trunk.seq_tfmr_{b}.layers.{l}", st["tfmr"][l], du)
            ops.add_view(mv(du0), mv(du), R, TD)
            dx1 = empty((R, CS), dev)
            nw.ln_skip_bwd(P, G, b, st["ln"], du0, dx1, dinit)
        ds = zeros((R, CS), dev)
        defer = b > 0 and fused_edge() and opts.fused_ln_bwd and sv["stages"][b - 1]["et"] is not None
        dz_acc = dz_in is not None
        if dz_in is None and not defer:
            dz_in = empty((Pn, CZ), dev)
        with rng(f"ipa_{b}.bwd"):
            pend = nw.ipa_bwd(P, G, f"score_model.trunk.ipa_{b}", st["ipa"], dx1, mv(ds), dz_in, dframe, dz_accumulate=dz_acc,
                              defer_dz=defer)
        _frame_grad_fold(st["bb"]["quat"], dframe, dq_in, dt_in, R)
        dq, dt, dnode, dz = dq_in, dt_in, ds, dz_in
        if not (defer_dw and b > 0 and sv["stages"][b - 1]["et"] is not None):
            ops.flush_dw()
        notify(b)
    ops.add_view(mv(dnode), mv(dinit), R, CS)
    with rng("embed.bwd"):
        nw.embed_bwd(P, G, sv["embed"], dnode, dz)
    ops.flush_dw()
    notify("embed")
    ops.join_grad_stream()


def _frame_grad_fold(quat, dframe, dq, dt, R):
    dev = quat
    z4 = zeros((R, 4), dev); z3 = zeros((R, 3), dev); z6 = zeros((R, 6), dev); zm = zeros((R,), dev)
    dq2 = empty((R, 4), dev); dt2 = empty((R, 3), dev); j1 = empty((R, 6), dev); j2 = empty((R, 6), dev)
    lib().call("fd_bb_update_bwd", z4, z3, dframe, zm, z6, quat, dq2, dt2, j1, j2, R)
    ops.add_view(mv(dq), mv(dq2), R, 4)
    ops.add_view(mv(dt), mv(dt2), R, 3)
```

Baseline: 180,900.

## Fuse first IPA pair-bias backward into edge-embed backward and cache packed weight images

Extends the edge-embed backward kernel with a ZBW variant that streams W40^T units and folds the block-0 IPA pair-bias gradient (dzb) into the dy accumulator through extra MFMA stages. This removes a separate dz GEMM and its round trip through memory. Weight-packing kernels move into a shared header, and a batched fd_weight_images path caches the packed images in an arena, invalidated when the optimizer changes the weights. The dynamic tile counter now resets itself atomically, which removes the per-launch memset.

```diff
diff --git a/include/fd_hip.h b/include/fd_hip.h
--- a/include/fd_hip.h
+++ b/include/fd_hip.h
@@ -147,8 +147,9 @@
 } FdEdgeEmbedDesc;
 int fd_edge_embed(const FdEdgeEmbedDesc* desc, void* stream);
 
-#define FD_EDGE_EMBED_BWD_IMAGE_BYTES (16 * 12288)
+#define FD_EDGE_EMBED_BWD_IMAGE_BYTES (20 * 12288)
 int fd_edge_embed_bwd_pack(const float* W2, const float* W4, void* image, void* stream);
+int fd_edge_embed_bwd_pack_zbw(const float* W40, void* image, void* stream);
 typedef struct FdEdgeEmbedBwdDesc {
   const float* dy;
   const float* h3;
@@ -169,8 +170,29 @@
   const unsigned* gmask2;
   const unsigned* gmask1;
   unsigned* sched;
+  const float* dzb;
+  const void* img_zbw;
 } FdEdgeEmbedBwdDesc;
 int fd_edge_embed_bwd(const FdEdgeEmbedBwdDesc* desc, void* stream);
+
+#define FD_WEIGHT_IMAGES_MAX_ITEMS 32
+enum {
+  FD_WI_PLANES = 0, FD_WI_EDGE_MLP_FWD = 1, FD_WI_EDGE_MLP_BWD = 2, FD_WI_ZB = 3, FD_WI_ZBW = 4, FD_WI_EDGE_EMBED = 5,
+  FD_WI_EDGE_EMBED_BWD = 6
+};
+typedef struct FdWeightImageItem {
+  int kind;
+  const float* w0;
+  const float* w1;
+  const float* w2;
+  void* dst;
+  long n;
+} FdWeightImageItem;
+typedef struct FdWeightImagesDesc {
+  FdWeightImageItem item[FD_WEIGHT_IMAGES_MAX_ITEMS];
+  int nitems;
+} FdWeightImagesDesc;
+int fd_weight_images(const FdWeightImagesDesc* desc, void* stream);
 
 typedef struct FdLnGemmDesc {
   const float* x;
diff --git a/se3_diffusion_amd/csrc/fd_edge_embed.hip b/se3_diffusion_amd/csrc/fd_edge_embed.hip
--- a/se3_diffusion_amd/csrc/fd_edge_embed.hip
+++ b/se3_diffusion_amd/csrc/fd_edge_embed.hip
@@ -11,52 +11,17 @@
 constexpr int EE_C = 128;
 constexpr float kPi = 3.14159265358979323846f;
 
+#include "fd_pack.h"
+
 __global__ __launch_bounds__(256) void edge_embed_pack_kernel(const float* __restrict__ W0, const float* __restrict__ W2,
                                                               const float* __restrict__ W4, char* __restrict__ img) {
   const int gid = (int)(blockIdx.x * blockDim.x + threadIdx.x);
-  if (gid >= EE_UNITS * 4 * 64) return;
-  const int lane = gid & 63, i = (gid >> 6) & 3, u = gid >> 8;
-  const int m = lane & 15, g = lane >> 4;
-  const int layer = u < 4 ? 0 : (u < 12 ? 1 : 2);
-  const int r = u - (layer == 0 ? 0 : (layer == 1 ? 4 : 12));
-  const int n = 64 * (r & 1) + 16 * i + m, k0 = 32 * (r >> 1);
-  float x[8];
-#pragma unroll
-  for (int e = 0; e < 8; ++e) {
-    if (layer == 0) {
-      const int k = k0 + 8 * g + e;
-      x[e] = k < 54 ? W0[n * 120 + 66 + k] : 0.f;
-    } else {
-      const int k = k0 + 16 * (e >> 2) + 4 * g + (e & 3);
-      x[e] = (layer == 1 ? W2 : W4)[n * EE_C + k];
-    }
-  }
-  uint4 s0, s1, s2;
-  fd_split8(x, s0, s1, s2);
-  char* dst = img + (long)u * EM_UNIT + (i * 3) * EM_PIECE + lane * 16;
-  *reinterpret_cast<uint4*>(dst) = s0;
-  *reinterpret_cast<uint4*>(dst + EM_PIECE) = s1;
-  *reinterpret_cast<uint4*>(dst + 2 * EM_PIECE) = s2;
+  if (gid < EE_UNITS * PK_FRAGS) pk_edge_embed(gid, W0, W2, W4, img);
 }
 
 __global__ __launch_bounds__(256) void edge_embed_pack_zb_kernel(const float* __restrict__ W40, char* __restrict__ img) {
   const int gid = (int)(blockIdx.x * blockDim.x + threadIdx.x);
-  if (gid >= EE_ZB_UNITS * 4 * 64) return;
-  const int lane = gid & 63, i = (gid >> 6) & 3, ks = gid >> 8;
-  const int m = lane & 15, g = lane >> 4;
-  const int n = 16 * i + m;
-  float x[8];
-#pragma unroll
-  for (int e = 0; e < 8; ++e) {
-    const int k = 32 * ks + 16 * (e >> 2) + 4 * g + (e & 3);
-    x[e] = n < EE_ZB ? W40[n * EE_C + k] : 0.f;
-  }
-  uint4 s0, s1, s2;
-  fd_split8(x, s0, s1, s2);
-  char* dst = img + (long)(EE_UNITS + ks) * EM_UNIT + (i * 3) * EM_PIECE + lane * 16;
-  *reinterpret_cast<uint4*>(dst) = s0;
-  *reinterpret_cast<uint4*>(dst + EM_PIECE) = s1;
-  *reinterpret_cast<uint4*>(dst + 2 * EM_PIECE) = s2;
+  if (gid < EE_ZB_UNITS * PK_FRAGS) pk_zb(gid, W40, img + (long)EE_UNITS * EM_UNIT);
 }
 
 template <bool ZB>
diff --git a/se3_diffusion_amd/csrc/fd_edge_embed_bwd.hip b/se3_diffusion_amd/csrc/fd_edge_embed_bwd.hip
--- a/se3_diffusion_amd/csrc/fd_edge_embed_bwd.hip
+++ b/se3_diffusion_amd/csrc/fd_edge_embed_bwd.hip
@@ -5,34 +5,27 @@
 
 #include "fd_chain.h"
 
+#include "fd_pack.h"
+
 constexpr int EB_UNITS = 16;
-constexpr int EB_NSTAGE = EB_UNITS / EM_UPS;
-constexpr int EB_C = 128;
+constexpr int EB_ZBW_UNITS = 4;
+constexpr int EB_C = 128, EB_ZB = 40;
+static_assert(EB_UNITS == PK_EB_UNITS && EB_ZBW_UNITS == PK_ZB_UNITS && EB_ZB == PK_ZB, "fd_pack.h packs what this kernel streams");
 
 __global__ __launch_bounds__(256) void edge_embed_bwd_pack_kernel(const float* __restrict__ W2, const float* __restrict__ W4,
                                                                   char* __restrict__ img) {
   const int gid = (int)(blockIdx.x * blockDim.x + threadIdx.x);
-  if (gid >= EB_UNITS * 4 * 64) return;
-  const int lane = gid & 63, i = (gid >> 6) & 3, u = gid >> 8;
-  const int m = lane & 15, g = lane >> 4;
-  const int layer = u >> 3, r = u & 7;
-  const int n = 64 * (r & 1) + 16 * i + m, k0 = 32 * (r >> 1);
-  const float* __restrict__ W = layer == 0 ? W4 : W2;
-  float x[8];
-#pragma unroll
-  for (int e = 0; e < 8; ++e) {
-    const int k = k0 + 16 * (e >> 2) + 4 * g + (e & 3);
-    x[e] = W[k * EB_C + n];
-  }
-  uint4 s0, s1, s2;
-  fd_split8(x, s0, s1, s2);
-  char* dst = img + (long)u * EM_UNIT + (i * 3) * EM_PIECE + lane * 16;
-  *reinterpret_cast<uint4*>(dst) = s0;
-  *reinterpret_cast<uint4*>(dst + EM_PIECE) = s1;
-  *reinterpret_cast<uint4*>(dst + 2 * EM_PIECE) = s2;
-}
-
+  if (gid < EB_UNITS * PK_FRAGS) pk_edge_embed_bwd(gid, W2, W4, img);
+}
+
+__global__ __launch_bounds__(256) void edge_embed_bwd_pack_zbw_kernel(const float* __restrict__ W40, char* __restrict__ img) {
+  const int gid = (int)(blockIdx.x * blockDim.x + threadIdx.x);
+  if (gid < EB_ZBW_UNITS * PK_FRAGS) pk_zbw(gid, W40, img + (long)EB_UNITS * EM_UNIT);
+}
+
+template <bool ZBW>
 __global__ __launch_bounds__(64 * EM_WAVES, 2) void edge_embed_bwd_kernel(FdEdgeEmbedBwdDesc d) {
+  constexpr int EB_ZSTAGE = ZBW ? EB_ZBW_UNITS / EM_UPS : 0, EB_NSTAGE = EB_UNITS / EM_UPS + EB_ZSTAGE;
   __shared__ __attribute__((aligned(16))) char lds[2 * EM_STAGE];
   const int tid = (int)threadIdx.x;
   const int lane = tid & 63, wave = tid >> 6;
@@ -48,10 +41,12 @@
   const int total_stages = dyn ? 0x7fffffff : nmine * EB_NSTAGE;
 
   const char* __restrict__ img_lane = static_cast<const char*>(d.img) + wave * (EM_STAGE / EM_WAVES) + lane * 16;
+  const char* __restrict__ zbw_lane = static_cast<const char*>(d.img_zbw) + wave * (EM_STAGE / EM_WAVES) + lane * 16;
   char* const lds_wave = lds + wave * (EM_STAGE / EM_WAVES);
   int issued = 0, consumed = 0;
   auto issue_stage = [&]() {
-    const char* src = img_lane + (long)(issued % EB_NSTAGE) * EM_STAGE;
+    const int s = issued % EB_NSTAGE;
+    const char* src = ZBW && s < EB_ZSTAGE ? zbw_lane + (long)s * EM_STAGE : img_lane + (long)(s - EB_ZSTAGE) * EM_STAGE;
     char* dst = lds_wave + (issued & 1) * EM_STAGE;
     fd::glds16x4(src, dst);
     fd::glds16x2(src + 4096, dst + 4096);
@@ -77,7 +72,11 @@
 
   int tile = first, nxt = 0;
   for (int ti = 0;;) {
-    if (dyn && tid == 0) nxt = G + (int)atomicAdd(&sched[0], 1u);
+    if (dyn && tid == 0) {
+      const unsigned ticket = atomicAdd(&sched[0], 1u);
+      if (ticket + 1u == (unsigned)ntiles) atomicAdd(&sched[0], 0u - (unsigned)ntiles);
+      nxt = G + (int)ticket;
+    }
     const long row = (long)tile * EM_ROWS + wave * 16 + m;
     const bool rok = row < rows;
     const long rc = rok ? row : rows - 1;
@@ -90,6 +89,46 @@
     }
 
     f32x4 d3[8];
+#pragma unroll
+    for (int nb = 0; nb < 8; ++nb) {
+      float4 v = make_float4(0.f, 0.f, 0.f, 0.f);
+      if (!ZBW || d.dy != nullptr) v = *reinterpret_cast<const float4*>(d.dy + rc * EB_C + 16 * nb + 4 * g);
+      d3[nb][0] = v.x; d3[nb][1] = v.y; d3[nb][2] = v.z; d3[nb][3] = v.w;
+    }
+    if (ZBW) {
+      float kz[2][8];
+      {
+        const float* zp = d.dzb + rc * EB_ZB + 8 * g;
+        const float4 v = *reinterpret_cast<const float4*>(zp);
+        const float4 w = *reinterpret_cast<const float4*>(zp + 4);
+        kz[0][0] = v.x; kz[0][1] = v.y; kz[0][2] = v.z; kz[0][3] = v.w;
+        kz[0][4] = w.x; kz[0][5] = w.y; kz[0][6] = w.z; kz[0][7] = w.w;
+        float4 v1 = make_float4(0.f, 0.f, 0.f, 0.f), w1 = v1;
+        if (g == 0) {
+          v1 = *reinterpret_cast<const float4*>(d.dzb + rc * EB_ZB + 32);
+          w1 = *reinterpret_cast<const float4*>(d.dzb + rc * EB_ZB + 36);
+        }
+        kz[1][0] = v1.x; kz[1][1] = v1.y; kz[1][2] = v1.z; kz[1][3] = v1.w;
+        kz[1][4] = w1.x; kz[1][5] = w1.y; kz[1][6] = w1.z; kz[1][7] = w1.w;
+      }
+      uint4 bz[3];
+      Em16Half Hz[2];
+#pragma clang loop unroll(full)
+      for (int sg = 0; sg < EB_ZBW_UNITS / EM_UPS; ++sg) {
+        const char* st = stage_begin();
+        em16_read_half(Hz[0], st);
+#pragma clang loop unroll(full)
+        for (int hh = 0; hh < 2 * EM_UPS; ++hh) {
+          const int r = EM_UPS * sg + (hh >> 1), g2 = r & 1, a = 4 * g2 + 2 * (hh & 1);
+          EM_PIN_TOP();
+          if (hh + 1 < 2 * EM_UPS) em16_read_half(Hz[(hh + 1) & 1], st + (hh + 1) * (EM_UNIT / 2));
+          if (g2 == 0 && (hh & 1) == 0) fd_split8(kz[r >> 1], bz[0], bz[1], bz[2]);
+          em16_mma_half(d3[a], d3[a + 1], Hz[hh & 1], bz);
+          EM_GROUPS(hh + 1 < 2 * EM_UPS);
+          if (hh == 1) stage_prefetch();
+        }
+      }
+    }
     {
       const float rs = (d.rowscale != nullptr ? d.rowscale[rc] : 1.f) * (rok ? 1.f : 0.f);
       const float mean = d.mean[rc], rstd = d.rstd[rc];
@@ -97,14 +136,13 @@
 #pragma unroll
       for (int nb = 0; nb < 8; ++nb) {
         const int col = 16 * nb + 4 * g;
-        const float4 dy = *reinterpret_cast<const float4*>(d.dy + rc * EB_C + col);
         const float4 h = *reinterpret_cast<const float4*>(d.h3 + rc * EB_C + col);
         const float4 gm = *reinterpret_cast<const float4*>(d.gamma + col);
-        const float dyv[4] = {dy.x, dy.y, dy.z, dy.w}, hv[4] = {h.x, h.y, h.z, h.w}, gv[4] = {gm.x, gm.y, gm.z, gm.w};
+        const float hv[4] = {h.x, h.y, h.z, h.w}, gv[4] = {gm.x, gm.y, gm.z, gm.w};
 #pragma unroll
         for (int e = 0; e < 4; ++e) {
           const float x = (hv[e] - mean) * rstd;
-          const float gy = dyv[e] * rs;
+          const float gy = d3[nb][e] * rs;
           dgam[nb][e] += gy * x;
           dbet[nb][e] += gy;
           const float t = gy * gv[e];
@@ -262,27 +300,36 @@
   return FD_OK;
 }
 
+extern "C" int fd_edge_embed_bwd_pack_zbw(const float* W40, void* img, void* stream) {
+  FD_CHECK_ARG(W40 && img, "fd_edge_embed_bwd_pack_zbw: null operand");
+  FD_CHECK_ARG(fd_aligned16(img), "fd_edge_embed_bwd_pack_zbw: image must be 16-byte aligned");
+  hipLaunchKernelGGL(edge_embed_bwd_pack_zbw_kernel, dim3(EB_ZBW_UNITS * 4 * 64 / 256), dim3(256), 0, (hipStream_t)stream, W40,
+                     static_cast<char*>(img));
+  FD_CHECK_LAUNCH("fd_edge_embed_bwd_pack_zbw");
+  return FD_OK;
+}
+
 extern "C" int fd_edge_embed_bwd(const FdEdgeEmbedBwdDesc* desc, void* stream) {
   FD_CHECK_ARG(desc != nullptr, "fd_edge_embed_bwd: null descriptor");
   const FdEdgeEmbedBwdDesc& d = *desc;
-  FD_CHECK_ARG(d.dy && d.h3 && d.mean && d.rstd && d.gamma && d.img && d.dh3 && d.dh2 && d.dh1,
+  FD_CHECK_ARG((d.dy || d.dzb) && d.h3 && d.mean && d.rstd && d.gamma && d.img && d.dh3 && d.dh2 && d.dh1,
                "fd_edge_embed_bwd: a required operand is null");
+  FD_CHECK_ARG((d.dzb != nullptr) == (d.img_zbw != nullptr),
+               "fd_edge_embed_bwd: dzb and img_zbw (the W40^T units of fd_edge_embed_bwd_pack_zbw) come together");
   FD_CHECK_ARG((d.h2 && d.h1) || (d.gmask2 && d.gmask1), "fd_edge_embed_bwd: h2 / h1 or their packed sign masks are required");
   FD_CHECK_ARG(d.rows >= 0, "fd_edge_embed_bwd: negative row count");
-  const void* ptrs[] = {d.dy, d.h3, d.gamma, d.h2, d.h1, d.img, d.dh3, d.dh2, d.dh1};
+  const void* ptrs[] = {d.dy, d.h3, d.gamma, d.h2, d.h1, d.img, d.dh3, d.dh2, d.dh1, d.dzb, d.img_zbw};
   for (const void* p : ptrs) FD_CHECK_ARG(fd_aligned16(p), "fd_edge_embed_bwd: operands must be 16-byte aligned");
   if (d.rows == 0) return FD_OK;
   const long ntiles = (d.rows + EM_ROWS - 1) / EM_ROWS;
   const int blocks = d.blocks > 0 ? d.blocks : 256 * EM_BLOCKS_PER_CU;
   const long grid = ntiles < blocks ? ntiles : blocks;
   FdEdgeEmbedBwdDesc dd = d;
-  if (dd.sched != nullptr && ntiles >= 4 * grid) {
-    FD_CHECK_ARG(hipMemsetAsync(dd.sched, 0, sizeof(unsigned), (hipStream_t)stream) == hipSuccess,
-                 "fd_edge_embed_bwd: zeroing the tile counter failed");
-  } else {
-    dd.sched = nullptr;
-  }
-  hipLaunchKernelGGL(edge_embed_bwd_kernel, dim3((unsigned)grid), dim3(64 * EM_WAVES), 0, (hipStream_t)stream, dd);
+  if (!(dd.sched != nullptr && ntiles >= 4 * grid)) dd.sched = nullptr;
+  if (dd.dzb != nullptr)
+    hipLaunchKernelGGL(edge_embed_bwd_kernel<true>, dim3((unsigned)grid), dim3(64 * EM_WAVES), 0, (hipStream_t)stream, dd);
+  else
+    hipLaunchKernelGGL(edge_embed_bwd_kernel<false>, dim3((unsigned)grid), dim3(64 * EM_WAVES), 0, (hipStream_t)stream, dd);
   FD_CHECK_LAUNCH("fd_edge_embed_bwd");
   return FD_OK;
 }
diff --git a/se3_diffusion_amd/csrc/fd_edge_mlp.hip b/se3_diffusion_amd/csrc/fd_edge_mlp.hip
--- a/se3_diffusion_amd/csrc/fd_edge_mlp.hip
+++ b/se3_diffusion_amd/csrc/fd_edge_mlp.hip
@@ -47,82 +47,21 @@
 #endif
 
 #ifndef EM_SHAPE_W8
-struct EmMat {
-  const float* p;
-  long rs, cs;
-};
+#include "fd_pack.h"
 
 __global__ __launch_bounds__(256) void edge_mlp_pack16_kernel(EmMat A1, EmMat A2, EmMat A4, char* __restrict__ img, int rot) {
   const int gid = (int)(blockIdx.x * blockDim.x + threadIdx.x);
-  if (gid >= EM_UNITS * 4 * 64) return;
-  const int lane = gid & 63, i = (gid >> 6) & 3, u = gid >> 8;
-  const int m = lane & 15, g = lane >> 4;
-  EmMat M;
-  int n, k0;
-  if (u < 96) {
-    const int c = u / 32, r = u % 32, hc = (c + rot) % 3;
-    if (r < 8) {
-      M = A1; n = 128 * hc + 64 * (r & 1) + 16 * i + m; k0 = 32 * (r >> 1);
-    } else {
-      const int r2 = r - 8;
-      M = A2; n = 64 * (r2 % 6) + 16 * i + m; k0 = 128 * hc + 32 * (r2 / 6);
-    }
-  } else {
-    const int v = u - 96;
-    M = A4; n = 64 * (v & 1) + 16 * i + m; k0 = 32 * (v >> 1);
-  }
-  float x[8];
-#pragma unroll
-  for (int e = 0; e < 8; ++e) {
-    const int k = k0 + 16 * (e >> 2) + 4 * g + (e & 3);
-    x[e] = M.p[(long)n * M.rs + (long)k * M.cs];
-  }
-  uint4 s0, s1, s2;
-  fd_split8(x, s0, s1, s2);
-  char* dst = img + (long)u * EM_UNIT + (i * 3) * EM_PIECE + lane * 16;
-  *reinterpret_cast<uint4*>(dst) = s0;
-  *reinterpret_cast<uint4*>(dst + EM_PIECE) = s1;
-  *reinterpret_cast<uint4*>(dst + 2 * EM_PIECE) = s2;
+  if (gid < EM_UNITS * PK_FRAGS) pk_edge_mlp(gid, A1, A2, A4, img, rot);
 }
 
 __global__ __launch_bounds__(256) void edge_mlp_pack_zb_kernel(const float* __restrict__ W40, char* __restrict__ img) {
   const int gid = (int)(blockIdx.x * blockDim.x + threadIdx.x);
-  if (gid >= EM_ZB_UNITS * 4 * 64) return;
-  const int lane = gid & 63, i = (gid >> 6) & 3, ks = gid >> 8;
-  const int m = lane & 15, g = lane >> 4;
-  const int n = 16 * i + m;
-  float x[8];
-#pragma unroll
-  for (int e = 0; e < 8; ++e) {
-    const int k = 32 * ks + 16 * (e >> 2) + 4 * g + (e & 3);
-    x[e] = n < EM_ZB ? W40[n * EM_C + k] : 0.f;
-  }
-  uint4 s0, s1, s2;
-  fd_split8(x, s0, s1, s2);
-  char* dst = img + (long)(EM_UNITS + ks) * EM_UNIT + (i * 3) * EM_PIECE + lane * 16;
-  *reinterpret_cast<uint4*>(dst) = s0;
-  *reinterpret_cast<uint4*>(dst + EM_PIECE) = s1;
-  *reinterpret_cast<uint4*>(dst + 2 * EM_PIECE) = s2;
+  if (gid < EM_ZB_UNITS * PK_FRAGS) pk_zb(gid, W40, img + (long)EM_UNITS * EM_UNIT);
 }
 
 __global__ __launch_bounds__(256) void edge_mlp_pack_zbw_kernel(const float* __restrict__ W40, char* __restrict__ img) {
   const int gid = (int)(blockIdx.x * blockDim.x + threadIdx.x);
-  if (gid >= EM_ZB_UNITS * 4 * 64) return;
-  const int lane = gid & 63, i = (gid >> 6) & 3, u = gid >> 8;
-  const int m = lane & 15, g = lane >> 4;
-  const int n = 64 * (u & 1) + 16 * i + m, k0 = 32 * (u >> 1);
-  float x[8];
-#pragma unroll
-  for (int e = 0; e < 8; ++e) {
-    const int k = k0 + 8 * g + e;
-    x[e] = k < EM_ZB ? W40[k * EM_C + n] : 0.f;
-  }
-  uint4 s0, s1, s2;
-  fd_split8(x, s0, s1, s2);
-  char* dst = img + (long)u * EM_UNIT + (i * 3) * EM_PIECE + lane * 16;
-  *reinterpret_cast<uint4*>(dst) = s0;
-  *reinterpret_cast<uint4*>(dst + EM_PIECE) = s1;
-  *reinterpret_cast<uint4*>(dst + 2 * EM_PIECE) = s2;
+  if (gid < EM_ZB_UNITS * PK_FRAGS) pk_zbw(gid, W40, img);
 }
 
 #endif
@@ -199,7 +138,11 @@
 
   int tile = first, nxt = 0;
   for (int ti = 0;;) {
-    if (dyn && tid == 0) nxt = G + (int)atomicAdd(&sched[0], 1u);
+    if (dyn && tid == 0) {
+      const unsigned ticket = atomicAdd(&sched[0], 1u);
+      if (ticket + 1u == (unsigned)ntiles) atomicAdd(&sched[0], 0u - (unsigned)ntiles);
+      nxt = G + (int)ticket;
+    }
     const long row = (long)tile * EM_ROWS + wave * 16 + m;
     const bool rok = row < rows;
     const long rc = rok ? row : rows - 1;
@@ -609,11 +552,7 @@
   const int grid = (int)(ntiles < blocks ? ntiles : blocks);
   const dim3 g3(grid), b3(64 * EM_WAVES);
   FdEdgeMlpDesc dd = d;
-  if (dd.sched != nullptr && ntiles >= 4L * grid) {
-    FD_CHECK_ARG(hipMemsetAsync(dd.sched, 0, sizeof(unsigned), st) == hipSuccess, "fd_edge_mlp: zeroing the tile counter failed");
-  } else {
-    dd.sched = nullptr;
-  }
+  if (!(dd.sched != nullptr && ntiles >= 4L * grid)) dd.sched = nullptr;
   const bool zbv = d.zb_out != nullptr, train = d.save1 != nullptr;
 #define EM_GO(...) hipLaunchKernelGGL(HIP_KERNEL_NAME(edge_mlp16_kernel<__VA_ARGS__>), g3, b3, 0, st, dd)
   if (d.backward) {
diff --git a/se3_diffusion_amd/csrc/fd_gemm_w.h b/se3_diffusion_amd/csrc/fd_gemm_w.h
--- a/se3_diffusion_amd/csrc/fd_gemm_w.h
+++ b/se3_diffusion_amd/csrc/fd_gemm_w.h
@@ -184,15 +184,8 @@
 
 __global__ __launch_bounds__(256) void split_planes_kernel(const float* __restrict__ x, long n8, long n,
                                                            unsigned short* __restrict__ planes) {
-  for (long i = (long)blockIdx.x * blockDim.x + threadIdx.x; i < n8; i += (long)gridDim.x * blockDim.x) {
-    const float4 a = *reinterpret_cast<const float4*>(x + 8 * i), b = *reinterpret_cast<const float4*>(x + 8 * i + 4);
-    uint2 a0, a1, a2, b0, b1, b2;
-    fd_split4(a, a0, a1, a2);
-    fd_split4(b, b0, b1, b2);
-    *reinterpret_cast<uint4*>(planes + 8 * i) = make_uint4(a0.x, a0.y, b0.x, b0.y);
-    *reinterpret_cast<uint4*>(planes + n + 8 * i) = make_uint4(a1.x, a1.y, b1.x, b1.y);
-    *reinterpret_cast<uint4*>(planes + 2 * n + 8 * i) = make_uint4(a2.x, a2.y, b2.x, b2.y);
-  }
+  for (long i = (long)blockIdx.x * blockDim.x + threadIdx.x; i < n8; i += (long)gridDim.x * blockDim.x)
+    fd_split_planes8(x, n, planes, i);
 }
 
 bool w_ok(const FdGemmDesc& d) {
diff --git a/se3_diffusion_amd/csrc/fd_pack.h b/se3_diffusion_amd/csrc/fd_pack.h
--- /dev/null
+++ b/se3_diffusion_amd/csrc/fd_pack.h
@@ -0,0 +1,112 @@
+#pragma once
+
+constexpr int PK_C = 128;
+constexpr int PK_ZB = 40;
+constexpr int PK_ZB_UNITS = 4;
+constexpr int PK_FRAGS = 4 * 64;
+
+struct EmMat {
+  const float* p;
+  long rs, cs;
+};
+
+__device__ __forceinline__ void pk_store(const float (&x)[8], char* __restrict__ units, int u, int i, int lane) {
+  uint4 s0, s1, s2;
+  fd_split8(x, s0, s1, s2);
+  char* dst = units + (long)u * EM_UNIT + (i * 3) * EM_PIECE + lane * 16;
+  *reinterpret_cast<uint4*>(dst) = s0;
+  *reinterpret_cast<uint4*>(dst + EM_PIECE) = s1;
+  *reinterpret_cast<uint4*>(dst + 2 * EM_PIECE) = s2;
+}
+
+constexpr int PK_EM_UNITS = 120;
+__device__ __forceinline__ void pk_edge_mlp(int gid, EmMat A1, EmMat A2, EmMat A4, char* __restrict__ img, int rot) {
+  const int lane = gid & 63, i = (gid >> 6) & 3, u = gid >> 8;
+  const int m = lane & 15, g = lane >> 4;
+  EmMat M;
+  int n, k0;
+  if (u < 96) {
+    const int c = u / 32, r = u % 32, hc = (c + rot) % 3;
+    if (r < 8) {
+      M = A1; n = 128 * hc + 64 * (r & 1) + 16 * i + m; k0 = 32 * (r >> 1);
+    } else {
+      const int r2 = r - 8;
+      M = A2; n = 64 * (r2 % 6) + 16 * i + m; k0 = 128 * hc + 32 * (r2 / 6);
+    }
+  } else {
+    const int v = u - 96;
+    M = A4; n = 64 * (v & 1) + 16 * i + m; k0 = 32 * (v >> 1);
+  }
+  float x[8];
+#pragma unroll
+  for (int e = 0; e < 8; ++e) {
+    const int k = k0 + 16 * (e >> 2) + 4 * g + (e & 3);
+    x[e] = M.p[(long)n * M.rs + (long)k * M.cs];
+  }
+  pk_store(x, img, u, i, lane);
+}
+
+__device__ __forceinline__ void pk_zb(int gid, const float* __restrict__ W40, char* __restrict__ units) {
+  const int lane = gid & 63, i = (gid >> 6) & 3, ks = gid >> 8;
+  const int m = lane & 15, g = lane >> 4;
+  const int n = 16 * i + m;
+  float x[8];
+#pragma unroll
+  for (int e = 0; e < 8; ++e) {
+    const int k = 32 * ks + 16 * (e >> 2) + 4 * g + (e & 3);
+    x[e] = n < PK_ZB ? W40[n * PK_C + k] : 0.f;
+  }
+  pk_store(x, units, ks, i, lane);
+}
+
+__device__ __forceinline__ void pk_zbw(int gid, const float* __restrict__ W40, char* __restrict__ units) {
+  const int lane = gid & 63, i = (gid >> 6) & 3, u = gid >> 8;
+  const int m = lane & 15, g = lane >> 4;
+  const int n = 64 * (u & 1) + 16 * i + m, k0 = 32 * (u >> 1);
+  float x[8];
+#pragma unroll
+  for (int e = 0; e < 8; ++e) {
+    const int k = k0 + 8 * g + e;
+    x[e] = k < PK_ZB ? W40[k * PK_C + n] : 0.f;
+  }
+  pk_store(x, units, u, i, lane);
+}
+
+constexpr int PK_EE_UNITS = 20;
+__device__ __forceinline__ void pk_edge_embed(int gid, const float* __restrict__ W0, const float* __restrict__ W2,
+                                              const float* __restrict__ W4, char* __restrict__ img) {
+  const int lane = gid & 63, i = (gid >> 6) & 3, u = gid >> 8;
+  const int m = lane & 15, g = lane >> 4;
+  const int layer = u < 4 ? 0 : (u < 12 ? 1 : 2);
+  const int r = u - (layer == 0 ? 0 : (layer == 1 ? 4 : 12));
+  const int n = 64 * (r & 1) + 16 * i + m, k0 = 32 * (r >> 1);
+  float x[8];
+#pragma unroll
+  for (int e = 0; e < 8; ++e) {
+    if (layer == 0) {
+      const int k = k0 + 8 * g + e;
+      x[e] = k < 54 ? W0[n * 120 + 66 + k] : 0.f;
+    } else {
+      const int k = k0 + 16 * (e >> 2) + 4 * g + (e & 3);
+      x[e] = (layer == 1 ? W2 : W4)[n * PK_C + k];
+    }
+  }
+  pk_store(x, img, u, i, lane);
+}
+
+constexpr int PK_EB_UNITS = 16;
+__device__ __forceinline__ void pk_edge_embed_bwd(int gid, const float* __restrict__ W2, const float* __restrict__ W4,
+                                                  char* __restrict__ img) {
+  const int lane = gid & 63, i = (gid >> 6) & 3, u = gid >> 8;
+  const int m = lane & 15, g = lane >> 4;
+  const int layer = u >> 3, r = u & 7;
+  const int n = 64 * (r & 1) + 16 * i + m, k0 = 32 * (r >> 1);
+  const float* __restrict__ W = layer == 0 ? W4 : W2;
+  float x[8];
+#pragma unroll
+  for (int e = 0; e < 8; ++e) {
+    const int k = k0 + 16 * (e >> 2) + 4 * g + (e & 3);
+    x[e] = W[k * PK_C + n];
+  }
+  pk_store(x, img, u, i, lane);
+}
diff --git a/se3_diffusion_amd/csrc/fd_split.h b/se3_diffusion_amd/csrc/fd_split.h
--- a/se3_diffusion_amd/csrc/fd_split.h
+++ b/se3_diffusion_amd/csrc/fd_split.h
@@ -33,6 +33,16 @@
   s2 = make_uint4(t2[0], t2[1], t2[2], t2[3]);
 }
 
+__device__ __forceinline__ void fd_split_planes8(const float* __restrict__ x, long n, unsigned short* __restrict__ planes, long i) {
+  const float4 a = *reinterpret_cast<const float4*>(x + 8 * i), b = *reinterpret_cast<const float4*>(x + 8 * i + 4);
+  uint2 a0, a1, a2, b0, b1, b2;
+  fd_split4(a, a0, a1, a2);
+  fd_split4(b, b0, b1, b2);
+  *reinterpret_cast<uint4*>(planes + 8 * i) = make_uint4(a0.x, a0.y, b0.x, b0.y);
+  *reinterpret_cast<uint4*>(planes + n + 8 * i) = make_uint4(a1.x, a1.y, b1.x, b1.y);
+  *reinterpret_cast<uint4*>(planes + 2 * n + 8 * i) = make_uint4(a2.x, a2.y, b2.x, b2.y);
+}
+
 constexpr int FD_PA[6] = {2, 1, 0, 1, 0, 0};
 constexpr int FD_PB[6] = {0, 1, 2, 0, 1, 0};
 
diff --git a/se3_diffusion_amd/csrc/fd_weight_images.hip b/se3_diffusion_amd/csrc/fd_weight_images.hip
--- /dev/null
+++ b/se3_diffusion_amd/csrc/fd_weight_images.hip
@@ -0,0 +1,89 @@
+#include "fd_common.h"
+#include "../../include/fd_hip.h"
+
+namespace {
+
+#include "fd_chain.h"
+#include "fd_pack.h"
+
+struct WiArgs {
+  FdWeightImageItem item[FD_WEIGHT_IMAGES_MAX_ITEMS];
+  int first[FD_WEIGHT_IMAGES_MAX_ITEMS + 1];
+  int nitems;
+};
+
+int wi_blocks(const FdWeightImageItem& it) {
+  switch (it.kind) {
+    case FD_WI_PLANES: {
+      const long nb = (it.n / 8 + 255) / 256;
+      return (int)(nb < 2048 ? nb : 2048);
+    }
+    case FD_WI_EDGE_MLP_FWD:
+    case FD_WI_EDGE_MLP_BWD: return PK_EM_UNITS;
+    case FD_WI_ZB:
+    case FD_WI_ZBW: return PK_ZB_UNITS;
+    case FD_WI_EDGE_EMBED: return PK_EE_UNITS;
+    case FD_WI_EDGE_EMBED_BWD: return PK_EB_UNITS;
+    default: return -1;
+  }
+}
+
+__global__ __launch_bounds__(256) void weight_images_kernel(WiArgs a) {
+  const int b = (int)blockIdx.x;
+  int t = 0;
+  while (t + 1 < a.nitems && b >= a.first[t + 1]) ++t;
+  const FdWeightImageItem it = a.item[t];
+  const int lb = b - a.first[t], nb = a.first[t + 1] - a.first[t];
+  const int gid = lb * 256 + (int)threadIdx.x;
+  char* const dst = static_cast<char*>(it.dst);
+  switch (it.kind) {
+    case FD_WI_PLANES: {
+      const long n8 = it.n / 8;
+      for (long i = gid; i < n8; i += (long)nb * 256) fd_split_planes8(it.w0, it.n, reinterpret_cast<unsigned short*>(dst), i);
+      break;
+    }
+    case FD_WI_EDGE_MLP_FWD:
+      pk_edge_mlp(gid, EmMat{it.w0, it.n, 1}, EmMat{it.w1, it.n, 1}, EmMat{it.w2, it.n, 1}, dst, 0);
+      break;
+    case FD_WI_EDGE_MLP_BWD:
+      pk_edge_mlp(gid, EmMat{it.w2, 1, it.n}, EmMat{it.w1, 1, it.n}, EmMat{it.w0, 1, it.n}, dst, 1);
+      break;
+    case FD_WI_ZB: pk_zb(gid, it.w0, dst); break;
+    case FD_WI_ZBW: pk_zbw(gid, it.w0, dst); break;
+    case FD_WI_EDGE_EMBED: pk_edge_embed(gid, it.w0, it.w1, it.w2, dst); break;
+    case FD_WI_EDGE_EMBED_BWD: pk_edge_embed_bwd(gid, it.w0, it.w1, dst); break;
+    default: break;
+  }
+}
+
+}
+
+extern "C" int fd_weight_images(const FdWeightImagesDesc* desc, void* stream) {
+  FD_CHECK_ARG(desc != nullptr, "fd_weight_images: null descriptor");
+  FD_CHECK_ARG(desc->nitems >= 0 && desc->nitems <= FD_WEIGHT_IMAGES_MAX_ITEMS, "fd_weight_images: nitems out of range");
+  if (desc->nitems == 0) return FD_OK;
+  WiArgs a;
+  a.nitems = desc->nitems;
+  int grid = 0;
+  for (int t = 0; t < desc->nitems; ++t) {
+    const FdWeightImageItem& it = desc->item[t];
+    const int nb = wi_blocks(it);
+    FD_CHECK_ARG(nb >= 0, "fd_weight_images: unknown item kind");
+    FD_CHECK_ARG(it.w0 != nullptr && it.dst != nullptr && fd_aligned16(it.dst), "fd_weight_images: an item needs w0 and a 16-byte aligned dst");
+    const bool three = it.kind == FD_WI_EDGE_MLP_FWD || it.kind == FD_WI_EDGE_MLP_BWD || it.kind == FD_WI_EDGE_EMBED;
+    FD_CHECK_ARG(!three || (it.w1 && it.w2), "fd_weight_images: a chain image needs its three weights");
+    FD_CHECK_ARG(it.kind != FD_WI_EDGE_EMBED_BWD || it.w1, "fd_weight_images: the embedder's backward image needs W2 and W4");
+    FD_CHECK_ARG(it.kind != FD_WI_PLANES || (it.n >= 0 && it.n % 8 == 0 && fd_aligned16(it.w0)),
+                 "fd_weight_images: planes need n %% 8 == 0 and a 16-byte aligned buffer");
+    FD_CHECK_ARG((it.kind != FD_WI_EDGE_MLP_FWD && it.kind != FD_WI_EDGE_MLP_BWD) || it.n >= 384,
+                 "fd_weight_images: an edge-transition item carries the weights' row stride in n");
+    a.item[t] = it;
+    a.first[t] = grid;
+    grid += nb;
+  }
+  for (int t = desc->nitems; t <= FD_WEIGHT_IMAGES_MAX_ITEMS; ++t) a.first[t] = grid;
+  if (grid == 0) return FD_OK;
+  hipLaunchKernelGGL(weight_images_kernel, dim3((unsigned)grid), dim3(256), 0, (hipStream_t)stream, a);
+  FD_CHECK_LAUNCH("fd_weight_images");
+  return FD_OK;
+}
diff --git a/se3_diffusion_amd/hip.py b/se3_diffusion_amd/hip.py
--- a/se3_diffusion_amd/hip.py
+++ b/se3_diffusion_amd/hip.py
@@ -110,11 +110,27 @@
         ("dy", c_void_p), ("h3", c_void_p), ("mean", c_void_p), ("rstd", c_void_p), ("gamma", c_void_p), ("rowscale", c_void_p),
         ("h2", c_void_p), ("h1", c_void_p), ("img", c_void_p), ("dh3", c_void_p), ("dh2", c_void_p), ("dh1", c_void_p),
         ("dgamma", c_void_p), ("dbeta", c_void_p), ("rows", c_long), ("blocks", c_int), ("gmask2", c_void_p), ("gmask1", c_void_p),
-        ("sched", c_void_p),
-    ]
-
-
-EDGE_EMBED_BWD_IMAGE_BYTES = 16 * 12288
+        ("sched", c_void_p), ("dzb", c_void_p), ("img_zbw", c_void_p),
+    ]
+
+
+EDGE_EMBED_BWD_IMAGE_BYTES = 20 * 12288
+EDGE_EMBED_BWD_ZBW_OFFSET = 16 * 12288
+
+
+WEIGHT_IMAGES_MAX_ITEMS = 32
+WI_PLANES, WI_EDGE_MLP_FWD, WI_EDGE_MLP_BWD, WI_ZB, WI_ZBW, WI_EDGE_EMBED, WI_EDGE_EMBED_BWD = range(7)
+IMAGE_UNIT_BYTES = 12288
+
+
+class FdWeightImageItem(Structure):
+    __slots__ = ()
+    _fields_ = [("kind", c_int), ("w0", c_void_p), ("w1", c_void_p), ("w2", c_void_p), ("dst", c_void_p), ("n", c_long)]
+
+
+class FdWeightImagesDesc(Structure):
+    _fields_ = [("item", FdWeightImageItem * WEIGHT_IMAGES_MAX_ITEMS), ("nitems", c_int)]
+
 
 class FdLnGemmDesc(Structure):
     __slots__ = ()
@@ -210,7 +226,9 @@
     "fd_edge_embed": "Ss",
     "fd_edge_embed_pack_zb": "pps",
     "fd_edge_embed_bwd_pack": "ppps",
+    "fd_edge_embed_bwd_pack_zbw": "pps",
     "fd_edge_embed_bwd": "Ss",
+    "fd_weight_images": "Ss",
     "fd_ln_gemm": "Ss",
     "fd_pair_dw": "Ss",
     "fd_group_dw": "Ss",
diff --git a/se3_diffusion_amd/network.py b/se3_diffusion_amd/network.py
--- a/se3_diffusion_amd/network.py
+++ b/se3_diffusion_amd/network.py
@@ -166,25 +166,41 @@
     se["x_early"] = ef
 
 
-def embed_bwd(P, G, sv, dnode, dedge):
+_EE = "embedding_layer.edge_embedder"
+
+
+def embed_bwd_fused(G, sv):
+    se = sv["edge"]
+    return bool(opts.fused_embed_bwd and fused_embed() and G is not None and se is not None and se.get("regen") is not None
+                and all(f"{_EE}.{l}.{t}" in G for l in (0, 2, 4) for t in ("weight", "bias")))
+
+
+def embed_bwd(P, G, sv, dnode, dedge, dzb_first=None):
     mlp3_ln_bwd(P, G, "embedding_layer.node_embedder", sv["node"], dnode)
     se = sv["edge"]
+    fused = embed_bwd_fused(G, sv)
+    if dzb_first is not None and not fused:
+        acc = dedge is not None
+        dedge = dedge if acc else empty((se["M"], CZ), dzb_first[0])
+        lib().call("fd_ipa_dz_acc", dzb_first[0], dzb_first[1].contiguous(), dedge, se["M"], int(acc))
+        dzb_first = None
     if se.get("x_early") is not None:
         se = dict(se, x=mv(se.pop("x_early")))
     if se.get("x") is None:
         seq, tscaled, fixed, sc, B, N = se["regen"]
-        tfreq, idenom, lower, upper = ops.feature_tables(dedge.device)
-        ef = empty((B * N * N, 120), dedge)
+        tfreq, idenom, lower, upper = ops.feature_tables(sc.device)
+        ef = empty((B * N * N, 120), sc)
         lib().call("fd_edge_feats", seq, tscaled, fixed, sc, tfreq, idenom, lower, upper, ef, B, N)
         se = dict(se, x=mv(ef))
-    pre = "embedding_layer.edge_embedder"
-    if (opts.fused_embed_bwd and fused_embed() and G is not None and se.get("regen") is not None
-            and all(f"{pre}.{l}.{t}" in G for l in (0, 2, 4) for t in ("weight", "bias"))):
+    pre = _EE
+    if fused:
         M = se["M"]
-        dh3 = empty((M, CZ), dedge); dh2 = empty((M, CZ), dedge); dh1 = empty((M, CZ), dedge)
-        img = ops.edge_embed_bwd_pack(P[f"{pre}.2.weight"], P[f"{pre}.4.weight"])
-        ops.edge_embed_bwd(dedge, se["h3"], se["mean"], se["rstd"], P[f"{pre}.5.weight"], se["rowscale"], se["h2"], se["h1"], img,
-                           dh3, dh2, dh1, G[f"{pre}.5.weight"], G[f"{pre}.5.bias"], M, gmask2=se.get("mh2"), gmask1=se.get("mh1"))
+        h3 = se["h3"]
+        dh3 = empty((M, CZ), h3); dh2 = empty((M, CZ), h3); dh1 = empty((M, CZ), h3)
+        img = ops.edge_embed_bwd_pack(P[f"{pre}.2.weight"], P[f"{pre}.4.weight"], W40=dzb_first[1] if dzb_first is not None else None)
+        ops.edge_embed_bwd(dedge, h3, se["mean"], se["rstd"], P[f"{pre}.5.weight"], se["rowscale"], se["h2"], se["h1"], img,
+                           dh3, dh2, dh1, G[f"{pre}.5.weight"], G[f"{pre}.5.bias"], M, gmask2=se.get("mh2"), gmask1=se.get("mh1"),
+                           dzb=dzb_first[0] if dzb_first is not None else None)
         x = se["x"]
         items = [(mv(dh3), mv(se["h2"]), mv(G[f"{pre}.4.weight"]), G[f"{pre}.4.bias"], CZ, CZ),
                  (mv(dh2), mv(se["h1"]), mv(G[f"{pre}.2.weight"]), G[f"{pre}.2.bias"], CZ, CZ),
diff --git a/se3_diffusion_amd/ops.py b/se3_diffusion_amd/ops.py
--- a/se3_diffusion_amd/ops.py
+++ b/se3_diffusion_amd/ops.py
@@ -2,6 +2,7 @@
 
 import math
 import threading
+import weakref
 
 import torch
 
@@ -56,6 +57,32 @@
 
 
 _PLANES = None
+_WEIGHT_EPOCH = 0
+_FLAT = {}
+_IMAGE_PLANS = {}
+
+
+def weights_changed(flat=None):
+    global _WEIGHT_EPOCH
+    _WEIGHT_EPOCH += 1
+    if flat is not None:
+        _FLAT[flat.untyped_storage().data_ptr()] = weakref.ref(flat)
+
+
+def _weights_stamp(base):
+    ref = _FLAT.get(base)
+    flat = ref() if ref is not None else None
+    return (flat._version if flat is not None else -1, _WEIGHT_EPOCH)
+
+
+def _flat_of(P):
+    ts = list(P.values())
+    st = ts[0].untyped_storage()
+    base, nbytes = st.data_ptr(), st.nbytes()
+    if base % 16 or nbytes % 32 or any(t.dtype != F32 or t.untyped_storage().data_ptr() != base for t in ts):
+        return None
+    n = nbytes // 4
+    return base, nbytes, torch.empty(0, dtype=F32, device=ts[0].device).set_(st, 0, (n,), (1,))
 
 
 def weight_planes(P):
@@ -63,21 +90,78 @@
     _PLANES = None
     if not opts.weight_planes or lib().exact_f32:
         return None
-    ts = list(P.values())
-    st = ts[0].untyped_storage()
-    base, nbytes = st.data_ptr(), st.nbytes()
-    if base % 16 or nbytes % 32 or any(t.dtype != F32 or t.untyped_storage().data_ptr() != base for t in ts):
-        return None
+    fl = _flat_of(P)
+    if fl is None:
+        return None
+    base, nbytes, flat = fl
     n = nbytes // 4
-    flat = torch.empty(0, dtype=F32, device=ts[0].device).set_(st, 0, (n,), (1,))
-    planes = torch.empty((3, n), dtype=torch.int16, device=ts[0].device)
+    planes = torch.empty((3, n), dtype=torch.int16, device=flat.device)
     lib().call("fd_split_planes", flat, n, planes)
-    _PLANES = (base, nbytes, planes)
+    _PLANES = (base, nbytes, planes, {}, _weights_stamp(base))
+    return _PLANES
+
+
+def _image_key(kind, ws, W40=None):
+    return (kind,) + tuple((w.data_ptr(), w.numel(), w.stride(0)) for w in ws) + ((W40.data_ptr(), W40.numel()) if W40 is not None else (0, 0))
+
+
+def _image_of(key):
+    ps = _PLANES
+    return ps[3].get(key) if ps is not None else None
+
+
+def weight_images(P, specs):
+    global _PLANES
+    _PLANES = None
+    if not opts.weight_planes or lib().exact_f32:
+        return None
+    if not opts.weight_images or not specs:
+        return weight_planes(P)
+    fl = _flat_of(P)
+    if fl is None:
+        return None
+    base, nbytes, flat = fl
+    n = nbytes // 4
+    sig = tuple(key for key, _, _ in specs)
+    plan = _IMAGE_PLANS.get((base, nbytes))
+    if plan is None or plan[0] != sig:
+        d = hip.FdWeightImagesDesc()
+        it = d.item[0]
+        it.kind, it.w0, it.n = hip.WI_PLANES, base, n
+        fills, off, k = [], 0, 1
+        for key, units, parts in specs:
+            for kind, ws, ld, unit0 in parts:
+                assert k < hip.WEIGHT_IMAGES_MAX_ITEMS, "weight_images: too many items for one descriptor"
+                it = d.item[k]
+                it.kind, it.n = kind, int(ld)
+                for name, w in zip(("w0", "w1", "w2"), ws):
+                    assert base <= w.data_ptr() < base + nbytes, "weight_images: a weight outside the flat parameter buffer"
+                    setattr(it, name, w.data_ptr())
+                fills.append((k, off + unit0 * hip.IMAGE_UNIT_BYTES))
+                k += 1
+            off += units * hip.IMAGE_UNIT_BYTES
+        d.nitems = k
+        plan = _IMAGE_PLANS[(base, nbytes)] = (sig, d, fills, off, [(key, units) for key, units, _ in specs])
+    _, d, fills, total, layout = plan
+    planes = torch.empty((3, n), dtype=torch.int16, device=flat.device)
+    arena = torch.empty(total, dtype=torch.uint8, device=flat.device)
+    a0 = arena.data_ptr()
+    d.item[0].dst = planes.data_ptr()
+    for k, off in fills:
+        d.item[k].dst = a0 + off
+    lib().launch("fd_weight_images", d, (flat, planes, arena))
+    images, off = {}, 0
+    for key, units in layout:
+        images[key] = arena[off:off + units * hip.IMAGE_UNIT_BYTES]
+        off += units * hip.IMAGE_UNIT_BYTES
+    _PLANES = (base, nbytes, planes, images, _weights_stamp(base))
     return _PLANES
 
 
 def set_weight_planes(ps):
     global _PLANES
+    if ps is not None and ps[4] != _weights_stamp(ps[0]):
+        ps = None
     was, _PLANES = _PLANES, ps
     return was
 
@@ -321,6 +405,10 @@
 
 
 def edge_mlp_pack(W1, W2, Wf, backward=False, out=None, W40=None):
+    if out is None:
+        img = _image_of(_image_key("em_bwd" if backward else "em_fwd", (W1, W2, Wf), W40))
+        if img is not None:
+            return img
     img = out if out is not None else torch.empty(hip.EDGE_MLP_IMAGE_BYTES, dtype=torch.uint8, device=W1.device)
     assert W40 is None or (W40.is_contiguous() and tuple(W40.shape) == (40, 128))
     assert W1.stride(-1) == 1 and W2.stride(-1) == 1 and Wf.stride(-1) == 1 and W1.stride(0) == W2.stride(0) == Wf.stride(0)
@@ -395,6 +483,10 @@
 
 
 def edge_embed_pack(W0, W2, W4, out=None, W40=None):
+    if out is None:
+        img = _image_of(_image_key("ee_fwd", (W0, W2, W4), W40))
+        if img is not None:
+            return img
     img = out if out is not None else torch.empty(hip.EDGE_EMBED_IMAGE_BYTES, dtype=torch.uint8, device=W0.device)
     lib().call("fd_edge_embed_pack", W0, W2, W4, img)
     if W40 is not None:
@@ -415,17 +507,26 @@
              (8, True, True, 2.0 * int(rows) * 310 * 128, (int(rows), 128, 128, 1, 0, 0, 0, 1)) if L.profiling else None)
 
 
-def edge_embed_bwd_pack(W2, W4, out=None):
+def edge_embed_bwd_pack(W2, W4, out=None, W40=None):
+    if out is None:
+        img = _image_of(_image_key("ee_bwd", (W2, W4), W40))
+        if img is not None:
+            return img
     img = out if out is not None else torch.empty(hip.EDGE_EMBED_BWD_IMAGE_BYTES, dtype=torch.uint8, device=W2.device)
     lib().call("fd_edge_embed_bwd_pack", W2, W4, img)
+    if W40 is not None:
+        assert W40.is_contiguous() and tuple(W40.shape) == (40, 128)
+        lib().call("fd_edge_embed_bwd_pack_zbw", W40, img)
     return img
 
 
 def edge_embed_bwd(dy, h3, mean, rstd, gamma, rowscale, h2, h1, img, dh3, dh2, dh1, dgamma, dbeta, rows, blocks=0, gmask2=None,
-                   gmask1=None):
+                   gmask1=None, dzb=None):
     d = hip.FdEdgeEmbedBwdDesc()
     tens = hip.fill_ptrs(d, dy=dy, h3=h3, mean=mean, rstd=rstd, gamma=gamma, rowscale=rowscale, h2=h2, h1=h1, img=img, dh3=dh3, dh2=dh2,
-                         dh1=dh1, dgamma=dgamma, dbeta=dbeta, gmask2=gmask2, gmask1=gmask1)
+                         dh1=dh1, dgamma=dgamma, dbeta=dbeta, gmask2=gmask2, gmask1=gmask1, dzb=dzb)
+    if dzb is not None:
+        d.img_zbw = img.data_ptr() + hip.EDGE_EMBED_BWD_ZBW_OFFSET
     d.rows, d.blocks = int(rows), int(blocks)
     L = lib()
     if opts.edge_dynamic_tiles and rows >= 4 * 64 * (d.blocks or 512):
diff --git a/se3_diffusion_amd/optim.py b/se3_diffusion_amd/optim.py
--- a/se3_diffusion_amd/optim.py
+++ b/se3_diffusion_amd/optim.py
@@ -5,7 +5,7 @@
 import torch
 import torch.distributed as dist
 
-from . import hip
+from . import hip, ops
 
 _ALIGN = 64
 
@@ -45,6 +45,7 @@
             view.copy_(p.data)
             p.data = view
             p.grad = self.flat_g[o:o + p.numel()].view_as(p)
+        ops.weights_changed(self.flat_p)
         self.max_grad_norm = None if max_grad_norm is None else float(max_grad_norm)
         self.skip_nonfinite = bool(skip_nonfinite)
         self.guarded = self.max_grad_norm is not None or self.skip_nonfinite
@@ -98,6 +99,7 @@
                 view = self.flat_p[o:o + n].view_as(p)
                 view.copy_(p.data)
                 p.data = view
+                ops.weights_changed()
             if p.grad is None:
                 view = self.flat_g[o:o + n].view_as(p)
                 if self._dirty:
@@ -132,6 +134,7 @@
         if self._ema_live:
             raise RuntimeError("step() inside ema_weights(): the parameters are the average there, not the training weights")
         self.rebind()
+        ops.weights_changed()
         b1, b2 = self.betas
         if self.guarded:
             if self.ema is None:
diff --git a/se3_diffusion_amd/options.py b/se3_diffusion_amd/options.py
--- a/se3_diffusion_amd/options.py
+++ b/se3_diffusion_amd/options.py
@@ -53,6 +53,7 @@
     defer_node_dw: bool = _opt("FD_DEFER_NODE_DW", True)
     node_dw_blocks: int = _opt("FD_NODE_DW_BLOCKS", 0)
     weight_planes: bool = _opt("FD_WEIGHT_PLANES", True)
+    weight_images: bool = _opt("FD_WEIGHT_IMAGES", True)
     ln_fold: bool = _opt("FD_LN_FOLD", True)
     sampler_device_steps: bool = _opt("FD_SAMPLER_DEVICE_STEPS", True)
     embed_first_padded: bool = _opt("FD_EMBED_FIRST_PADDED", True)
diff --git a/se3_diffusion_amd/trunk.py b/se3_diffusion_amd/trunk.py
--- a/se3_diffusion_amd/trunk.py
+++ b/se3_diffusion_amd/trunk.py
@@ -384,11 +384,50 @@
     return n
 
 
+def _image_specs(P, num_blocks):
+    U = hip.IMAGE_UNIT_BYTES
+    specs = []
+    if num_blocks < 1:
+        return specs
+
+    def w40(b):
+        pre = f"score_model.trunk.ipa_{b}"
+        W = nw.ipa_w40(P, pre)[0]
+        view = W.untyped_storage().data_ptr() == P[f"{pre}.linear_b.weight"].untyped_storage().data_ptr()
+        return W if view and W.is_contiguous() and W.data_ptr() % 16 == 0 else None
+
+    if nw.fused_embed():
+        pre = "embedding_layer.edge_embedder"
+        W0, W2, W4 = P[f"{pre}.0.weight"], P[f"{pre}.2.weight"], P[f"{pre}.4.weight"]
+        zb = w40(0) if opts.zb_from_edge else None
+        parts = [(hip.WI_EDGE_EMBED, (W0, W2, W4), 0, 0)] + ([(hip.WI_ZB, (zb,), 0, 20)] if zb is not None else [])
+        specs.append((ops._image_key("ee_fwd", (W0, W2, W4), zb), hip.EDGE_EMBED_IMAGE_BYTES // U, parts))
+        if opts.fused_embed_bwd:
+            zbw = w40(0)
+            parts = [(hip.WI_EDGE_EMBED_BWD, (W2, W4), 0, 0)] + ([(hip.WI_ZBW, (zbw,), 0, 16)] if zbw is not None else [])
+            specs.append((ops._image_key("ee_bwd", (W2, W4), zbw), hip.EDGE_EMBED_BWD_IMAGE_BYTES // U, parts))
+    if fused_edge():
+        for b in range(num_blocks - 1):
+            pre = f"score_model.trunk.edge_transition_{b}"
+            W1, W2, Wf = P[f"{pre}.trunk.0.weight"], P[f"{pre}.trunk.2.weight"], P[f"{pre}.final_layer.weight"]
+            if not (W1.stride(-1) == W2.stride(-1) == Wf.stride(-1) == 1 and W1.stride(0) == W2.stride(0) == Wf.stride(0)):
+                continue
+            ld, nxt = W1.stride(0), w40(b + 1)
+            zb = nxt if opts.zb_from_edge else None
+            parts = [(hip.WI_EDGE_MLP_FWD, (W1, W2, Wf), ld, 0)] + ([(hip.WI_ZB, (zb,), 0, 120)] if zb is not None else [])
+            specs.append((ops._image_key("em_fwd", (W1, W2, Wf), zb), hip.EDGE_MLP_IMAGE_BYTES // U, parts))
+            zbw = nxt if opts.fused_ln_bwd else None
+            lead = 4 if zbw is not None else 0
+            parts = ([(hip.WI_ZBW, (zbw,), 0, 0)] if zbw is not None else []) + [(hip.WI_EDGE_MLP_BWD, (W1, W2, Wf), ld, lead)]
+            specs.append((ops._image_key("em_bwd", (W1, W2, Wf), zbw), hip.EDGE_MLP_IMAGE_BYTES // U, parts))
+    return specs
+
+
 def forward(P, feats, num_blocks, dconf=(0.1, 0.1, 20.0, 0.1, 1.5, 1000), tfmr_bool_mask=False, save=True, cache=None,
             sc_ca_out=None):
     if save:
         cache = None
-    planes = ops.weight_planes(P) if save else None
+    planes = ops.weight_images(P, _image_specs(P, num_blocks) if opts.weight_images else ()) if save else None
     if not save:
         ops.set_weight_planes(None)
     f = _prep_feats(feats)
@@ -564,7 +603,11 @@
             dx1 = empty((R, CS), dev)
             nw.ln_skip_bwd(P, G, b, st["ln"], du0, dx1, dinit)
         ds = zeros((R, CS), dev)
-        defer = b > 0 and fused_edge() and opts.fused_ln_bwd and sv["stages"][b - 1]["et"] is not None
+        if b > 0:
+            defer = fused_edge() and opts.fused_ln_bwd and sv["stages"][b - 1]["et"] is not None
+        else:
+            W40 = st["ipa"]["W40"]
+            defer = nw.embed_bwd_fused(G, sv["embed"]) and W40.is_contiguous() and W40.data_ptr() % 16 == 0
         dz_acc = dz_in is not None
         if dz_in is None and not defer:
             dz_in = empty((Pn, CZ), dev)
@@ -578,7 +621,7 @@
         notify(b)
     ops.add_view(mv(dnode), mv(dinit), R, CS)
     with rng("embed.bwd"):
-        nw.embed_bwd(P, G, sv["embed"], dnode, dz)
+        nw.embed_bwd(P, G, sv["embed"], dnode, dz, dzb_first=pend)
     ops.flush_dw()
     notify("embed")
     ops.join_grad_stream()
```

New measurement: 179,200. No clear change (-0.9%).
